# xuhaocuhk/TilinGNN

Measured on AMD Instinct MI355X. Metric: scored tile-nodes/sec (GNN forward), higher is better.
Workload: dtype f32; 1 GPU; TilinGNN.forward on a seeded banded super-graph: 100000 nodes / 1000000 adjacency edges / 1250000 collision edges per GPU, tile_count 2, T=13 edge types, width 32, depth 20, train-mode BatchNorm, graph prep included; n_nodes=100000, n_adj_edges=1000000, n_col_edges=1250000, parallelism=single GPU

## Files before the change

### include/tgnn.h

```cpp
#ifndef TGNN_H
#define TGNN_H

#include <stddef.h>
#include <stdint.h>

#ifdef __cplusplus
extern "C" {
#endif

#define TGNN_VERSION 100

#define TGNN_OK 0
#define TGNN_ERR_INVALID_ARG (-1)
#define TGNN_ERR_WORKSPACE (-2)
#define TGNN_ERR_LAUNCH (-3)
#define TGNN_ERR_UNSUPPORTED (-4)
#define TGNN_ERR_BAD_GRAPH (-5)
#define TGNN_ERR_UNVERIFIED (-7)
#define TGNN_ERR_STALE_RESULT (-6)

#define TGNN_ACT_NONE 0
#define TGNN_ACT_LEAKY_RELU 1
#define TGNN_ACT_SIGMOID 2

#define TGNN_BN_STAT_ROWS 4
#define TGNN_BN_MAX_PARTIALS 512

typedef void *tgnn_stream_t;

int tgnn_version(void);
const char *tgnn_last_error(void);


size_t tgnn_csr_workspace_bytes(int64_t n_nodes, int64_t n_edges);
int tgnn_csr_build(const int64_t *edge_index, int64_t n_edges, int64_t n_nodes, int64_t n_src_nodes,
                   int drop_self_loops, int32_t *rowptr, int32_t *col_src, int32_t *col_eid, int32_t *err_flag,
                   void *ws, size_t ws_bytes, tgnn_stream_t stream);

size_t tgnn_edge_dedup_workspace_bytes(int64_t n_edges, int32_t fe);
int tgnn_edge_type_dedup(const float *edge_attr, int64_t n_edges, int32_t fe, int32_t *edge_type,
                         int32_t *type_rep_edge, int32_t *n_types, void *ws, size_t ws_bytes,
                         tgnn_stream_t stream);

int tgnn_gather_i32(const int32_t *src, int64_t n_src, const int32_t *idx, int64_t n, int32_t *out,
                    tgnn_stream_t stream);


int tgnn_edge_weight_table(const float *edge_attr, const int32_t *type_rep_edge, int32_t n_types, int32_t fe,
                           const float *w1, const float *b1, const float *w2, const float *b2,
                           const float *w3, const float *b3, int32_t c, float *wtab, tgnn_stream_t stream);

int tgnn_nnconv_mean_fwd(const float *h, int64_t ldh, const int32_t *rowptr, const int32_t *col_src,
                         const int32_t *col_type, const float *wtab, int32_t n_types, const float *root,
                         const float *bias, int64_t n_nodes, int32_t c, int32_t act, float *out,
                         double *bn_partial, int32_t *n_partials_host, tgnn_stream_t stream);

int64_t tgnn_nnconv_cols_max_columns(int64_t n_nodes, int64_t n_edges);
size_t tgnn_nnconv_cols_workspace_bytes(int64_t n_nodes);
int tgnn_nnconv_cols_build(const int32_t *rowptr, const int32_t *col_src, const int32_t *col_type,
                           int64_t n_nodes, int32_t n_types, int32_t *tile_col_ptr, int32_t *col_meta,
                           int32_t *col_slot_src, void *ws, size_t ws_bytes, tgnn_stream_t stream);
int32_t tgnn_nnconv_cols_max_types(void);
size_t tgnn_nnconv_weight_image_floats(int32_t n_types);
int tgnn_nnconv_mean_cols_fwd(const float *h, int64_t ldh, const int32_t *tile_col_ptr, const int32_t *col_meta,
                              const int32_t *col_src, const float *wtab, int32_t n_types, const float *root,
                              const float *bias, int64_t n_nodes, int32_t c, int32_t act, float *out,
                              float *wimg_scratch, double *bn_partial, int32_t *n_partials_host,
                              tgnn_stream_t stream);
int tgnn_nnconv_mean_cols_f16_fwd(const float *h, int64_t ldh, int64_t n_src_rows, const int32_t *tile_col_ptr,
                                  const int32_t *col_meta, const int32_t *col_src, const float *wtab, int32_t n_types,
                                  const float *root, const float *bias, int64_t n_nodes, int32_t max_in_degree, int32_t act,
                                  float *out, float *wimg_scratch, uint32_t *bounds_scratch, double *bn_partial,
                                  int32_t *n_partials_host, tgnn_stream_t stream);

int64_t tgnn_nnconv_eg_max_groups(int64_t n_nodes, int64_t n_edges, int32_t n_types);
int tgnn_nnconv_eg_build(const int32_t *rowptr, const int32_t *col_src, const int32_t *col_type, int64_t n_nodes,
                         int32_t n_types, int32_t *tile_grp_ptr, int32_t *grp, void *ws, size_t ws_bytes, tgnn_stream_t stream);
int tgnn_nnconv_mean_eg_fwd(const float *h, int64_t ldh, int64_t n_src_rows, const int32_t *tile_grp_ptr,
                            const int32_t *grp, const float *wtab, int32_t n_types,
                            const float *root, const float *bias, int64_t n_nodes, int32_t act, float *out,
                            float *wimg_scratch, uint32_t *bounds_scratch, double *bn_partial, int32_t *n_partials_host,
                            tgnn_stream_t stream);

int32_t tgnn_nnconv64_eg_max_types(void);
size_t tgnn_nnconv64_eg_image_floats(int32_t n_types);
int tgnn_nnconv64_mean_eg_fwd(const float *h, int64_t ldh, int64_t n_src_rows, const int32_t *tile_grp_ptr,
                              const int32_t *grp, const float *wtab, int32_t n_types,
                              const float *root, const float *bias, int64_t n_nodes, int32_t act, float *out,
                              float *wimg_scratch, uint32_t *bounds_scratch, double *bn_partial, int32_t *n_partials_host,
                              tgnn_stream_t stream);

int tgnn_ubench_row_gather(int32_t shape, const float *table, int64_t n_rows, float *sink, int32_t iters, int32_t reps,
                           double *rows_per_s_out, tgnn_stream_t stream);

#define TGNN_MID_BATCH_WORDS 36
#define TGNN_MID_TILE_BATCHES 24
int64_t tgnn_mid_entries_words(int64_t n_nodes);
int tgnn_mid_entries_build(const int32_t *tile_col_ptr, const int32_t *col_meta, const int32_t *col_src, int64_t n_nodes,
                           const int32_t *cols_built_dev, int32_t *tile_nb, uint32_t *ent, int32_t *result, tgnn_stream_t stream);
void tgnn_forward_path_counts(int64_t *out3);
void tgnn_set_mid_layout_limit(int64_t n_nodes);
int64_t tgnn_get_mid_layout_limit(void);
int64_t tgnn_mid_layout_max_nodes(void);

int tgnn_gin_fwd(const float *a, int64_t lda, const float *in_stat, const int32_t *rowptr,
                 const int32_t *col_src, const float *eps, const float *w1, const float *b1,
                 const float *w2, const float *b2, const float *w3, const float *b3, int64_t n_nodes,
                 int32_t c, int32_t act, float *out, float *z_scratch, double *bn_partial,
                 int32_t *n_partials_host, tgnn_stream_t stream);
int tgnn_gin32_fwd(const float *a, int64_t lda, const float *in_stat, const int32_t *rowptr, const int32_t *col_src,
                   const float *eps, const float *w1, const float *b1, const float *w2, const float *b2, const float *w3,
                   const float *b3, int64_t n_nodes, int32_t c, int32_t act, int32_t variant, float *out, float *z_scratch,
                   double *bn_partial, int32_t *n_partials_host, tgnn_stream_t stream);
int tgnn_gin64_fwd(const float *a, int64_t lda, const float *in_stat, const int32_t *rowptr, const int32_t *col_src,
                   const float *eps, const float *w1, const float *b1, const float *w2, const float *b2, const float *w3,
                   const float *b3, int64_t n_nodes, int32_t act, float *out, float *z_scratch, double *bn_partial,
                   int32_t *n_partials_host, tgnn_stream_t stream);

int tgnn_dense_act_fwd(const float *a, int64_t lda, int64_t a_kblock_stride, const float *in_stat,
                       const float *w, const float *b, int64_t n_rows, int32_t in_dim, int32_t out_dim,
                       int32_t act, float *out, int64_t ldo, double *bn_partial, int32_t *n_partials_host,
                       tgnn_stream_t stream);
int tgnn_dense_act_slots_fwd(const float *a, int32_t slot_width, int64_t slot_stride, const float *in_stat,
                             const float *w, const float *b, int64_t n_rows, int32_t in_dim, int32_t out_dim,
                             int32_t act, float *out, int64_t ldo, double *bn_partial, int32_t *n_partials_host,
                             tgnn_stream_t stream);
int tgnn_dense_act_slots_f16_fwd(const float *a, int32_t slot_width, int64_t slot_stride, const float *w, const float *b,
                                 int64_t n_rows, int32_t in_dim, int32_t out_dim, int32_t act, float *out, int64_t ldo,
                                 uint32_t *bounds_scratch, void *wimg_scratch, double *bn_partial, int32_t *n_partials_host,
                                 tgnn_stream_t stream);

int tgnn_bn_finalize(int32_t mode, const double *partials, int32_t n_partials, double *sums, int32_t f,
                     int64_t n_rows_total, const float *gamma, const float *beta, float eps, float momentum,
                     float *running_mean, float *running_var, int64_t *num_batches_tracked, float *stat,
                     tgnn_stream_t stream);

int tgnn_bn_apply(const float *v, int64_t ldv, const float *stat, int64_t n_rows, int32_t f, float *out,
                  int64_t ldo, tgnn_stream_t stream);

int tgnn_merge_fwd(const float *a1, const float *stat1, const float *a2, const float *stat2,
                   const float *resid, int64_t n_nodes, int32_t c, float *out, float *h2_out,
                   tgnn_stream_t stream);

typedef struct tgnn_model_dims {
    int32_t node_features_dim;
    int32_t adj_edge_features_dim;
    int32_t network_width;
    int32_t network_depth;
    int32_t output_dim;
} tgnn_model_dims;

int32_t tgnn_param_count(const tgnn_model_dims *dims);
int tgnn_param_name(const tgnn_model_dims *dims, int32_t index, char *buf, size_t buf_len);

typedef struct tgnn_graph {
    int64_t n_nodes;
    int64_t n_adj_edges;
    int64_t n_col_edges;
    int32_t n_types;
    const int32_t *adj_rowptr;
    const int32_t *adj_src;
    const int32_t *adj_type;
    const int32_t *type_rep_edge;
    const int32_t *col_rowptr;
    const int32_t *col_src;
    const int32_t *nn_tile_col_ptr;
    const int32_t *nn_col_meta;
    const int32_t *nn_col_src;
    int32_t nn_max_in_degree;
    const int32_t *nn_mid_tile_nb;
    const uint32_t *nn_mid_ent;
    const int32_t *nn_tile_grp_ptr;
    const int32_t *nn_grp;
    const int32_t *nn_mid_verdict;
} tgnn_graph;

size_t tgnn_forward_workspace_bytes(const tgnn_model_dims *dims, int64_t n_nodes, int32_t n_types);

enum { TGNN_WS_MID = 0, TGNN_WS_A1, TGNN_WS_F1, TGNN_WS_F2, TGNN_WS_F3, TGNN_WS_BOUNDS, TGNN_WS_BOUNDS64, TGNN_WS_MAP_ENTRIES };
int tgnn_forward_workspace_map(const tgnn_model_dims *dims, int64_t n_nodes, int64_t n_rows, int32_t n_types, int64_t *byte_offsets,
                               int32_t n);

int tgnn_forward(const tgnn_model_dims *dims, const void *const *params_host, const float *x,
                 const float *adj_edge_attr, const tgnn_graph *graph, int32_t update_running,
                 int32_t use_running_stats, float *probs, void *ws, size_t ws_bytes,
                 tgnn_stream_t stream, tgnn_stream_t stream2);

int tgnn_forward_begin(const tgnn_model_dims *dims, const void *const *params_host, const float *x, int64_t n_nodes,
                       int32_t update_running, void *ws, size_t ws_bytes, tgnn_stream_t stream, tgnn_stream_t stream2);
int tgnn_forward_resume(const tgnn_model_dims *dims, const void *const *params_host, const float *x, const float *adj_edge_attr,
                        const tgnn_graph *graph, int32_t update_running, float *probs, void *ws, size_t ws_bytes,
                        tgnn_stream_t stream, tgnn_stream_t stream2);
int tgnn_forward_small_prepass(const tgnn_model_dims *dims, const void *const *params_host, const float *adj_edge_attr,
                               const int32_t *type_rep_edge, const int32_t *n_types_dev, int64_t n_nodes, void *ws, size_t ws_bytes,
                               tgnn_stream_t stream);

int tgnn_forward_begin_weights(const tgnn_model_dims *dims, const void *const *params_host, const float *adj_edge_attr,
                               const int32_t *type_rep_edge, const int32_t *n_types_dev, int64_t n_nodes, void *ws, size_t ws_bytes,
                               tgnn_stream_t stream);

typedef struct tgnn_train_save {
    float *init_a[2];
    float *init_stat[2];
    float *a1, *a2;
    float *u;
    float *stat1, *stat2;
    float *fin_a[4];
    float *fin_stat[4];
    float *skip;
    float *wtab;
} tgnn_train_save;
int tgnn_forward_train(const tgnn_model_dims *dims, const void *const *params_host, const float *x,
                       const float *adj_edge_attr, const tgnn_graph *graph, const tgnn_train_save *keep, float *probs,
                       void *ws, size_t ws_bytes, tgnn_stream_t stream, tgnn_stream_t stream2);

typedef struct tgnn_train_graph {
    const int32_t *adjT_rowptr, *adjT_src, *adjT_type;
    const int32_t *colT_rowptr, *colT_src;
    const float *deg, *inv_deg;
} tgnn_train_graph;
size_t tgnn_backward_workspace_bytes(const tgnn_model_dims *dims, int64_t n_nodes, int32_t n_types);
int tgnn_backward(const tgnn_model_dims *dims, const void *const *params_host, void *const *grads_host, const float *x,
                  const float *adj_edge_attr, const tgnn_graph *graph, const tgnn_train_graph *tgraph,
                  const tgnn_train_save *keep, const float *probs, const float *dprobs, void *ws, size_t ws_bytes,
                  tgnn_stream_t stream);
typedef struct tgnn_train_groups {
    const int32_t *fwd_tile_grp_ptr, *fwd_grp;
    const int32_t *bwd_tile_grp_ptr, *bwd_grp;
    const int32_t *type_major;
    int64_t n_list;
    int32_t max_in_degree, max_out_degree;
} tgnn_train_groups;
int tgnn_backward_groups(const tgnn_model_dims *dims, const void *const *params_host, void *const *grads_host, const float *x,
                         const float *adj_edge_attr, const tgnn_graph *graph, const tgnn_train_graph *tgraph,
                         const tgnn_train_groups *groups, const tgnn_train_save *keep, const float *probs, const float *dprobs,
                         void *ws, size_t ws_bytes, tgnn_stream_t stream);

typedef struct tgnn_shard {
    int64_t n_own, n_rows, n_total;
    const int32_t *send_idx;
    int64_t n_send;
    double *sum_buf;
    float *send_buf;
    float *recv_buf;
    int (*allreduce_f64)(void *ctx, double *buf, int64_t count, tgnn_stream_t stream);
    int (*alltoall_rows)(void *ctx, const float *send, float *recv, int32_t row_floats, int32_t extra_rows,
                         tgnn_stream_t stream);
    void *ctx;
    int32_t world, rank;
    const int32_t *send_idx_fused;
    const int32_t *recv_idx_fused;
    tgnn_stream_t side_stream;
    void *rccl_comm, *rccl_comm_side;
    const int64_t *send_counts, *recv_counts;
    const int32_t *send_row_ptr, *send_row_slot;
} tgnn_shard;

int32_t tgnn_rccl_available(void);
size_t tgnn_rccl_unique_id_bytes(void);
int tgnn_rccl_unique_id(void *id_out);
int tgnn_rccl_comm_create(const void *unique_id, int32_t rank, int32_t world, void **comm_out);
int tgnn_rccl_comm_destroy(void *comm);
void tgnn_rccl_counters(int64_t *out2);
size_t tgnn_forward_sharded_workspace_bytes(const tgnn_model_dims *dims, int64_t n_own, int64_t n_rows,
                                            int32_t n_types);
int tgnn_forward_sharded(const tgnn_model_dims *dims, const void *const *params_host, const float *x,
                         const float *adj_edge_attr, const tgnn_graph *graph, const tgnn_shard *shard,
                         int32_t update_running, float *probs, void *ws, size_t ws_bytes, tgnn_stream_t stream);

void tgnn_set_small_layout_limit(int64_t n_nodes);
int tgnn_spin_error_poll(tgnn_stream_t stream, uint32_t *code_out);
uint64_t tgnn_set_spin_budget_us(uint64_t us);
void tgnn_persist_fallback(int64_t n_forwards);
uint32_t tgnn_spin_error_peek(void);
int64_t tgnn_get_small_layout_limit(void);

int32_t tgnn_set_split_precision(int32_t mode);
int32_t tgnn_set_gin_fused(int32_t mode);
int32_t tgnn_set_gin_mlp_f16(int32_t on);
int32_t tgnn_set_mid_tail(int32_t on);
int32_t tgnn_set_nnconv_eg(int32_t on);
int32_t tgnn_set_nnconv64_eg(int32_t on);
int32_t tgnn_set_gin64_mfma(int32_t on);
int32_t tgnn_set_dense_rows_mode(int32_t mode);
int32_t tgnn_set_lean_head(int32_t bits);

int64_t tgnn_graph_prep_small_max_nodes(void);
int64_t tgnn_graph_prep_small_max_edges(void);
size_t tgnn_graph_prep_small_tmp_ints(int64_t n_nodes, int64_t n_adj_edges, int64_t n_col_edges);
int tgnn_graph_prep_small(const int64_t *adj_edge_index, int64_t n_adj_edges, const float *adj_edge_attr, int32_t fe,
                          const int64_t *col_edge_index, int64_t n_col_edges, int64_t n_nodes, int32_t *adj_rowptr,
                          int32_t *adj_src, int32_t *adj_eid, int32_t *adj_type, int32_t *edge_type, int32_t *type_rep_edge,
// ... 312 lines not shown
```

### tilingnn_amd/_lib.py

```python
from __future__ import annotations

import ctypes as C
import os

_HERE = os.path.dirname(os.path.abspath(__file__))
LIB_PATH = os.environ.get("TGNN_LIB_PATH") or os.path.join(_HERE, "libtgnn.so")

ACT_NONE, ACT_LEAKY_RELU, ACT_SIGMOID = 0, 1, 2
BN_MAX_PARTIALS = 512
BN_STAT_ROWS = 4


class TgnnError(RuntimeError):
    code = 0


class ModelDims(C.Structure):
    _fields_ = [("node_features_dim", C.c_int32), ("adj_edge_features_dim", C.c_int32),
                ("network_width", C.c_int32), ("network_depth", C.c_int32), ("output_dim", C.c_int32)]


class Graph(C.Structure):
    _fields_ = [("n_nodes", C.c_int64), ("n_adj_edges", C.c_int64), ("n_col_edges", C.c_int64),
                ("n_types", C.c_int32),
                ("adj_rowptr", C.c_void_p), ("adj_src", C.c_void_p), ("adj_type", C.c_void_p),
                ("type_rep_edge", C.c_void_p), ("col_rowptr", C.c_void_p), ("col_src", C.c_void_p),
                ("nn_tile_col_ptr", C.c_void_p), ("nn_col_meta", C.c_void_p), ("nn_col_src", C.c_void_p),
                ("nn_max_in_degree", C.c_int32),
                ("nn_mid_tile_nb", C.c_void_p), ("nn_mid_ent", C.c_void_p),
                ("nn_tile_grp_ptr", C.c_void_p), ("nn_grp", C.c_void_p), ("nn_mid_verdict", C.c_void_p)]


class SmallPrepLayout(C.Structure):
    _fields_ = [("adj_edge_index", C.c_void_p), ("adj_edge_attr", C.c_void_p), ("col_edge_index", C.c_void_p),
                ("n_adj_edges", C.c_int64), ("n_col_edges", C.c_int64), ("n_nodes", C.c_int64),
                ("adj_rowptr", C.c_void_p), ("adj_src", C.c_void_p), ("adj_eid", C.c_void_p), ("adj_type", C.c_void_p),
                ("edge_type", C.c_void_p), ("type_rep_edge", C.c_void_p),
                ("col_rowptr", C.c_void_p), ("col_src", C.c_void_p), ("col_eid", C.c_void_p),
                ("tile_col_ptr", C.c_void_p), ("col_meta", C.c_void_p), ("col_slot_src", C.c_void_p),
                ("tmp", C.c_void_p), ("fe", C.c_int32), ("reserved_", C.c_int32)]


class TrainSave(C.Structure):
    _fields_ = [("init_a", C.c_void_p * 2), ("init_stat", C.c_void_p * 2), ("a1", C.c_void_p), ("a2", C.c_void_p),
                ("u", C.c_void_p), ("stat1", C.c_void_p), ("stat2", C.c_void_p), ("fin_a", C.c_void_p * 4),
                ("fin_stat", C.c_void_p * 4), ("skip", C.c_void_p), ("wtab", C.c_void_p)]


class TrainGraphDesc(C.Structure):
    _fields_ = [("adjT_rowptr", C.c_void_p), ("adjT_src", C.c_void_p), ("adjT_type", C.c_void_p),
                ("colT_rowptr", C.c_void_p), ("colT_src", C.c_void_p), ("deg", C.c_void_p), ("inv_deg", C.c_void_p)]


class TrainGroupsDesc(C.Structure):
    _fields_ = [("fwd_tile_grp_ptr", C.c_void_p), ("fwd_grp", C.c_void_p), ("bwd_tile_grp_ptr", C.c_void_p), ("bwd_grp", C.c_void_p),
                ("type_major", C.c_void_p), ("n_list", C.c_int64), ("max_in_degree", C.c_int32), ("max_out_degree", C.c_int32)]


ALLREDUCE_CB = C.CFUNCTYPE(C.c_int, C.c_void_p, C.c_void_p, C.c_int64, C.c_void_p)
ALLTOALL_CB = C.CFUNCTYPE(C.c_int, C.c_void_p, C.c_void_p, C.c_void_p, C.c_int32, C.c_int32, C.c_void_p)


class ShardDesc(C.Structure):
    _fields_ = [("n_own", C.c_int64), ("n_rows", C.c_int64), ("n_total", C.c_int64),
                ("send_idx", C.c_void_p), ("n_send", C.c_int64),
                ("sum_buf", C.c_void_p), ("send_buf", C.c_void_p), ("recv_buf", C.c_void_p),
                ("allreduce_f64", ALLREDUCE_CB), ("alltoall_rows", ALLTOALL_CB), ("ctx", C.c_void_p),
                ("world", C.c_int32), ("rank", C.c_int32), ("send_idx_fused", C.c_void_p), ("recv_idx_fused", C.c_void_p),
                ("side_stream", C.c_void_p), ("rccl_comm", C.c_void_p), ("rccl_comm_side", C.c_void_p),
                ("send_counts", C.c_void_p), ("recv_counts", C.c_void_p),
                ("send_row_ptr", C.c_void_p), ("send_row_slot", C.c_void_p)]


def _load() -> C.CDLL:
    if not os.path.exists(LIB_PATH):
        raise ImportError(
            f"{LIB_PATH} is missing: the HIP extension has not been built. Build it with\n"
            f"    python -c 'import __graft_entry__ as g; g.build()'    (or: make -C tilingnn_amd/csrc)\n"
            "tilingnn_amd has no CPU fallback by design.")
    import torch
    lib = C.CDLL(LIB_PATH)
    p, i32, i64, f32, sz = C.c_void_p, C.c_int32, C.c_int64, C.c_float, C.c_size_t
    pi32 = C.POINTER(C.c_int32)
    sigs = {
        "tgnn_version": (C.c_int, []),
        "tgnn_last_error": (C.c_char_p, []),
        "tgnn_csr_workspace_bytes": (sz, [i64, i64]),
        "tgnn_csr_build": (C.c_int, [p, i64, i64, i64, C.c_int, p, p, p, p, p, sz, p]),
        "tgnn_edge_dedup_workspace_bytes": (sz, [i64, i32]),
        "tgnn_edge_type_dedup": (C.c_int, [p, i64, i32, p, p, p, p, sz, p]),
        "tgnn_gather_i32": (C.c_int, [p, i64, p, i64, p, p]),
        "tgnn_edge_weight_table": (C.c_int, [p, p, i32, i32, p, p, p, p, p, p, i32, p, p]),
        "tgnn_nnconv_mean_fwd": (C.c_int, [p, i64, p, p, p, p, i32, p, p, i64, i32, i32, p, p, pi32, p]),
        "tgnn_nnconv_cols_max_columns": (i64, [i64, i64]),
        "tgnn_nnconv_cols_workspace_bytes": (sz, [i64]),
        "tgnn_nnconv_cols_build": (C.c_int, [p, p, p, i64, i32, p, p, p, p, sz, p]),
        "tgnn_nnconv_cols_max_types": (i32, []),
        "tgnn_nnconv_weight_image_floats": (sz, [i32]),
        "tgnn_nnconv_mean_cols_fwd": (C.c_int, [p, i64, p, p, p, p, i32, p, p, i64, i32, i32, p, p, p, pi32, p]),
        "tgnn_nnconv_mean_cols_f16_fwd": (C.c_int, [p, i64, i64, p, p, p, p, i32, p, p, i64, i32, i32, p, p, p, p, pi32, p]),
        "tgnn_nnconv_eg_max_groups": (i64, [i64, i64, i32]),
        "tgnn_nnconv_eg_build": (C.c_int, [p, p, p, i64, i32, p, p, p, sz, p]),
        "tgnn_nnconv_mean_eg_fwd": (C.c_int, [p, i64, i64, p, p, p, i32, p, p, i64, i32, p, p, p, p, pi32, p]),
        "tgnn_nnconv64_eg_max_types": (i32, []),
        "tgnn_nnconv64_eg_image_floats": (sz, [i32]),
        "tgnn_nnconv64_mean_eg_fwd": (C.c_int, [p, i64, i64, p, p, p, i32, p, p, i64, i32, p, p, p, p, pi32, p]),
        "tgnn_ubench_row_gather": (C.c_int, [i32, p, i64, p, i32, i32, C.POINTER(C.c_double), p]),
        "tgnn_mid_entries_words": (i64, [i64]),
        "tgnn_mid_entries_build": (C.c_int, [p, p, p, i64, p, p, p, p, p]),
        "tgnn_forward_path_counts": (None, [p]),
        "tgnn_set_mid_layout_limit": (None, [i64]),
        "tgnn_get_mid_layout_limit": (i64, []),
        "tgnn_mid_layout_max_nodes": (i64, []),
        "tgnn_spin_error_poll": (C.c_int, [p, C.POINTER(C.c_uint32)]),
        "tgnn_set_spin_budget_us": (C.c_uint64, [C.c_uint64]),
        "tgnn_persist_fallback": (None, [i64]),
        "tgnn_spin_error_peek": (C.c_uint32, []),
        "tgnn_gin_fwd": (C.c_int, [p, i64, p, p, p, p, p, p, p, p, p, p, i64, i32, i32, p, p, p, pi32, p]),
        "tgnn_gin32_fwd": (C.c_int, [p, i64, p, p, p, p, p, p, p, p, p, p, i64, i32, i32, i32, p, p, p, pi32, p]),
        "tgnn_gin64_fwd": (C.c_int, [p, i64, p, p, p, p, p, p, p, p, p, p, i64, i32, p, p, p, pi32, p]),
        "tgnn_dense_act_fwd": (C.c_int, [p, i64, i64, p, p, p, i64, i32, i32, i32, p, i64, p, pi32, p]),
        "tgnn_dense_act_slots_fwd": (C.c_int, [p, i32, i64, p, p, p, i64, i32, i32, i32, p, i64, p, pi32, p]),
        "tgnn_dense_act_slots_f16_fwd": (C.c_int, [p, i32, i64, p, p, i64, i32, i32, i32, p, i64, p, p, p, pi32, p]),
        "tgnn_bn_finalize": (C.c_int, [i32, p, i32, p, i32, i64, p, p, f32, f32, p, p, p, p, p]),
        "tgnn_bn_apply": (C.c_int, [p, i64, p, i64, i32, p, i64, p]),
        "tgnn_merge_fwd": (C.c_int, [p, p, p, p, p, i64, i32, p, p, p]),
        "tgnn_param_count": (i32, [C.POINTER(ModelDims)]),
        "tgnn_param_name": (C.c_int, [C.POINTER(ModelDims), i32, C.c_char_p, sz]),
        "tgnn_forward_workspace_bytes": (sz, [C.POINTER(ModelDims), i64, i32]),
        "tgnn_forward_workspace_map": (C.c_int, [C.POINTER(ModelDims), i64, i64, i32, C.POINTER(C.c_int64), i32]),
        "tgnn_forward": (C.c_int, [C.POINTER(ModelDims), C.POINTER(C.c_void_p), p, p, C.POINTER(Graph), i32, i32,
                                   p, p, sz, p, p]),
        "tgnn_forward_begin": (C.c_int, [C.POINTER(ModelDims), C.POINTER(C.c_void_p), p, i64, i32, p, sz, p, p]),
        "tgnn_forward_resume": (C.c_int, [C.POINTER(ModelDims), C.POINTER(C.c_void_p), p, p, C.POINTER(Graph), i32, p, p, sz, p, p]),
        "tgnn_forward_begin_weights": (C.c_int, [C.POINTER(ModelDims), C.POINTER(C.c_void_p), p, p, p, i64, p, sz, p]),
        "tgnn_forward_small_prepass": (C.c_int, [C.POINTER(ModelDims), C.POINTER(C.c_void_p), p, p, p, i64, p, sz, p]),
        "tgnn_forward_sharded_workspace_bytes": (sz, [C.POINTER(ModelDims), i64, i64, i32]),
        "tgnn_forward_sharded": (C.c_int, [C.POINTER(ModelDims), C.POINTER(C.c_void_p), p, p, C.POINTER(Graph),
                                           C.POINTER(ShardDesc), i32, p, p, sz, p]),
        "tgnn_sublayout_workspace_bytes": (sz, [i64, i64, i64]),
        "tgnn_sublayout_compact": (C.c_int, [p, i64, p, i32, p, i64, p, i32, p, i64, p, p, p, p, p, p, p, p, sz, p]),
        "tgnn_shard_alive_rows": (C.c_int, [p, p, i64, i64, p, i64, p, i64, p, p, p]),
        "tgnn_tiles_in_region": (C.c_int, [p, p, p, p, p, i64, p, p, p, p, i64, i32, p, p, p]),
        "tgnn_region_edge_counts": (C.c_int, [p, i64, i64, p, i64, p, i64, p, p, p]),
        "tgnn_union_area_workspace_bytes": (sz, [i64, i64]),
        "tgnn_union_area": (C.c_int, [p, p, i64, p, p, p, i64, C.c_double, p, p, p, sz, p]),
        "tgnn_union_topology_workspace_bytes": (sz, [i64, i64]),
        "tgnn_union_topology": (C.c_int, [p, p, i64, p, p, p, p, p, i64, C.c_double, C.c_double, C.c_double, p, p, p, sz, p]),
        "tgnn_union_hole_delta_workspace_bytes": (sz, [i64, i64]),
        "tgnn_union_hole_delta": (C.c_int, [p, p, i64, p, p, p, p, p, i64, C.c_double, C.c_double, C.c_double, p, p, p, p, sz, p]),
        "tgnn_union_contour_workspace_bytes": (sz, [i64, i64, i64]),
        "tgnn_union_contour": (C.c_int, [p, p, i64, p, p, p, p, p, i64, C.c_double, i64, i64, p, p, p, p, p, p, p, p, sz, p]),
        "tgnn_batch_union": (C.c_int, [p] * 10 + [i32, i32, i32, p, p, i32, p, p, p, p, p]),
        "tgnn_greedy_round_workspace_bytes": (sz, [i64]),
        "tgnn_greedy_round": (C.c_int, [p, i64, p, i64, p, i64, i32, C.c_uint64, p, p, p, p, p, p, sz, p]),
        "tgnn_greedy_finish_max_nodes": (i64, []),
        "tgnn_greedy_finish": (C.c_int, [p, i64, p, i64, i32, i32, C.c_uint64, p, p, p, p, p, p, p]),
        "tgnn_sublayout_compact_many_workspace_bytes": (sz, [i32, i64, i64, i64]),
        "tgnn_sublayout_compact_many": (C.c_int, [i32, p, p, p, p, i64, i64, i64, p, p, i32, p, p, i32, p, p, p, p, p, p, p, p, p, sz, p]),
        "tgnn_greedy_round_many_workspace_bytes": (sz, [i32, i64]),
        "tgnn_greedy_round_many": (C.c_int, [i32, p, p, i64, p, p, i64, i64, p, p, p, i32, p, p, p, p, p, p, p, sz, p]),
        "tgnn_greedy_finish_many": (C.c_int, [i32, p, p, p, i64, i64, p, p, p, i32, i32, p, p, p, p, p, p, p, p]),
        "tgnn_solution_score_sums_many_workspace_bytes": (sz, [i32]),
        "tgnn_solution_score_sums_many": (C.c_int, [i32, p, p, p, i64, i64, p, p, i64, p, p, p, i64, p, p, sz, p]),
        "tgnn_unsupervised_loss_many_workspace_bytes": (sz, [i32, i32]),
        "tgnn_unsupervised_loss_many": (C.c_int, [i32, p, p, p, p, i64, i64, i64, p, p, i64, i32, p, i64, p, p, i64, p, f32, f32, f32,
                                                  p, p, p, p, sz, p]),
        "tgnn_unsupervised_loss_workspace_bytes": (sz, [i32]),
        "tgnn_unsupervised_loss": (C.c_int, [p, i64, i32, p, i64, i64, p, i64, p, i64, p, i64, f32, f32, f32, p, p, p, sz, p]),
        "tgnn_solution_score_sums": (C.c_int, [p, p, i64, p, i64, p, i64, p, i64, p, p, sz, p]),
        "tgnn_graph_prep_small_max_nodes": (i64, []),
        "tgnn_graph_prep_small_max_edges": (i64, []),
        "tgnn_graph_prep_small_tmp_ints": (sz, [i64, i64, i64]),
        "tgnn_graph_prep_small": (C.c_int, [p, i64, p, i32, p, i64, i64] + [p] * 16 + [p]),
        "tgnn_graph_prep_workspace_bytes": (sz, [i64, i64, i64, i32]),
        "tgnn_graph_prep": (C.c_int, [p, i64, p, i32, p, i64, i64, i64] + [p] * 17 + [sz, p, p, p]),
        "tgnn_graph_prep_wait": (C.c_int, [p]),
        "tgnn_graph_prep_small_many": (C.c_int, [C.POINTER(SmallPrepLayout), i32, p, p, p]),
        "tgnn_graph_prep_small_many_wait": (C.c_int, [p]),
        "tgnn_graph_prep_small_many_plan": (C.c_int, [p, p, p, i32, i32, p, p]),
        "tgnn_graph_prep_small_many_counts": (None, [p]),
        "tgnn_set_nnconv_eg": (i32, [i32]),
        "tgnn_set_nnconv64_eg": (i32, [i32]),
        "tgnn_set_gin64_mfma": (i32, [i32]),
        "tgnn_set_dense_rows_mode": (i32, [i32]),
        "tgnn_set_lean_head": (i32, [i32]),
        "tgnn_set_prep_words_poll": (i32, [i32]),
        "tgnn_set_small_layout_limit": (None, [i64]),
        "tgnn_get_small_layout_limit": (i64, []),
        "tgnn_set_split_precision": (i32, [i32]),
        "tgnn_set_gin_fused": (i32, [i32]),
        "tgnn_set_gin_mlp_f16": (i32, [i32]),
        "tgnn_set_mid_tail": (i32, [i32]),
        "tgnn_rccl_available": (i32, []),
        "tgnn_rccl_unique_id_bytes": (sz, []),
        "tgnn_rccl_unique_id": (C.c_int, [p]),
        "tgnn_rccl_comm_create": (C.c_int, [p, i32, i32, C.POINTER(C.c_void_p)]),
        "tgnn_rccl_comm_destroy": (C.c_int, [p]),
        "tgnn_rccl_counters": (None, [p]),
        "tgnn_forward_profiled": (C.c_int, [C.POINTER(ModelDims), C.POINTER(C.c_void_p), p, p, C.POINTER(Graph), i32,
                                            i32, p, p, sz, p, C.POINTER(C.c_float), pi32]),
        "tgnn_forward_many": (C.c_int, [C.POINTER(ModelDims), C.POINTER(C.c_void_p), i32, p, p, p, i32, i32, p, p, p, p, i32, p]),
        "tgnn_forward_union": (C.c_int, [C.POINTER(ModelDims), C.POINTER(C.c_void_p), i32, p, p, p, i32, p, p, p, p, p, i32, p]),
        "tgnn_forward_union_plan": (C.c_int, [p, i32, i32, p]),
        "tgnn_forward_union_counts": (None, [p]),
        "tgnn_forward_stamped": (C.c_int, [C.POINTER(ModelDims), C.POINTER(C.c_void_p), p, p, C.POINTER(Graph), i32, p, p, sz, p, p,
                                           C.POINTER(C.c_float)]),
        "tgnn_forward_profiled_two_stream": (C.c_int, [C.POINTER(ModelDims), C.POINTER(C.c_void_p), p, p, C.POINTER(Graph), i32,
                                                       p, p, sz, p, p, C.POINTER(C.c_float), pi32]),
        "tgnn_transpose": (C.c_int, [p, i32, i32, p, p]),
        "tgnn_swap_leading": (C.c_int, [p, i32, i32, i32, p, i32, p]),
        "tgnn_backward_workspace_bytes": (sz, [C.POINTER(ModelDims), i64, i32]),
        "tgnn_backward": (C.c_int, [C.POINTER(ModelDims), C.POINTER(C.c_void_p), C.POINTER(C.c_void_p), p, p,
                                    C.POINTER(Graph), C.POINTER(TrainGraphDesc), C.POINTER(TrainSave), p, p, p, sz, p]),
        "tgnn_backward_groups": (C.c_int, [C.POINTER(ModelDims), C.POINTER(C.c_void_p), C.POINTER(C.c_void_p), p, p,
                                           C.POINTER(Graph), C.POINTER(TrainGraphDesc), C.POINTER(TrainGroupsDesc),
                                           C.POINTER(TrainSave), p, p, p, sz, p]),
        "tgnn_nnconv_bwd_eg_ok": (i32, [i32, i64, i32, i32, i32, i32, i32]),
        "tgnn_nnconv_bwd_eg_workspace_bytes": (sz, [i64, i64, i32, i32]),
        "tgnn_nnconv_bwd_eg_list_ints": (sz, [i64]),
        "tgnn_nnconv_bwd_eg_dw_blocks": (i32, [i64]),
        "tgnn_nnconv_bwd_eg_build": (C.c_int, [p, p, i64, i32, p, p]),
        "tgnn_nnconv_bwd_eg": (C.c_int, [p, i64, p, p, p, p, p, p, p, i64, p, p, i64, i32, i32, i32, i32, p, p, p, sz, p]),
        "tgnn_set_nnconv_bwd_eg": (i32, [i32]),
        "tgnn_forward_train": (C.c_int, [C.POINTER(ModelDims), C.POINTER(C.c_void_p), p, p, C.POINTER(Graph),
                                         C.POINTER(TrainSave), p, p, sz, p, p]),
        "tgnn_gin_aggregate": (C.c_int, [p, i64, p, p, p, p, i64, i32, p, p]),
        "tgnn_sigmoid_bwd": (C.c_int, [p, i64, p, i64, i64, i32, p, i64, p]),
        "tgnn_add_into": (C.c_int, [p, i64, i64, i32, p, i64, p]),
        "tgnn_reduce_workspace_bytes": (sz, [i32]),
        "tgnn_colsum": (C.c_int, [p, i64, i64, i32, p, p, sz, p]),
        "tgnn_bn_bwd_reduce": (C.c_int, [p, i64, p, i64, p, i64, i32, f32, p, p, p, p, sz, p]),
        "tgnn_bn_bwd_apply": (C.c_int, [p, i64, p, i64, p, p, i64, i32, i32, p, i64, p, p, i64, p]),
        "tgnn_merge_bwd_reduce": (C.c_int, [p, i64, p, p, p, p, p, i64, i32, f32, f32, p, p, p, i64, p, p, p, p, p, p,
                                            p, sz, p]),
        "tgnn_wgrad_workspace_bytes": (sz, [i64, i32, i32]),
        "tgnn_wgrad": (C.c_int, [p, i64, p, i64, i64, i64, i32, i32, p, p, p, sz, p]),
        "tgnn_wgrad_slots": (C.c_int, [p, i64, p, i32, i64, i64, i32, i32, p, p, p, sz, p]),
        "tgnn_sigmoid_mlp_bwd_workspace_bytes": (sz, [i64, i32, i32, i32, i32]),
        "tgnn_sigmoid_mlp_bwd": (C.c_int, [p, i64, i32, i32, i32, i32, p, p, p, p, p, p, p, i64, p, p, p, p, p, p, p, p, sz,
                                           p]),
        "tgnn_sigmoid_mlp_bwd_fused_form": (i32, [i64, i32, i32, i32, i32, i32]),
        "tgnn_sigmoid_mlp_bwd_fused_workspace_bytes": (sz, [i64, i32, i32, i32, i32]),
        "tgnn_sigmoid_mlp_bwd_fused": (C.c_int, [p, i64, i32, i32, i32, i32, p, p, p, p, p, p, p, i64, p, p, p, p, p, p, p, p,
                                                 sz, p]),
        "tgnn_set_mlp_bwd_fused": (i32, [i32]),
        "tgnn_sigmoid_mlp_bwd_tall64_ok": (i32, [i64, i32, i32, i32, i32]),
        "tgnn_sigmoid_mlp_bwd_tall64_workspace_bytes": (sz, [i64, i32, i32, i32, i32]),
        "tgnn_sigmoid_mlp_bwd_tall64": (C.c_int, [p, i64, i32, i32, i32, i32, p, p, p, p, p, p, p, i64, p, p, p, p, p, p, p, p,
                                                  sz, p]),
        "tgnn_set_mlp_bwd_tall64": (i32, [i32]),
        "tgnn_nnconv_type_sum": (C.c_int, [p, i64, p, i64, p, p, p, p, i64, i32, i32, p, p]),
        "tgnn_csr_degree": (C.c_int, [p, i64, p, p, p]),
        "tgnn_unsupervised_loss_bwd": (C.c_int, [p, i64, p, i64, i64, p, i64, p, i64, p, i64, f32, f32, f32, p, p, p, i64,
                                                 p, sz, p]),
        "tgnn_f32_to_bf16": (C.c_int, [p, i64, p, p]),
        "tgnn_nnconv64_image_elems": (sz, [i32]),
        "tgnn_nnconv64_bf16_fwd": (C.c_int, [p, i64, p, p, p, p, i32, p, p, i64, i32, p, p, p, pi32, p]),
        "tgnn_nnconv64_bf16_eg_fwd": (C.c_int, [p, i64, p, p, p, i32, p, p, i64, i32, p, p, p, pi32, p]),
        "tgnn_gin64_bf16_fwd": (C.c_int, [p, p, p, p, p, p, p, p, p, p, p, i64, i32, p, p, p, pi32, p]),
        "tgnn_collconv64_bf16_fwd": (C.c_int, [p, p, p, p, p, p, p, p, p, p, p, p, p, p, p, i64, p, p, p, p, p, p]),
        "tgnn_merge_bf16_fwd": (C.c_int, [p, p, p, p, p, i64, i32, p, p]),
        "tgnn_dense_bf16_slots_fwd": (C.c_int, [p, i64, i32, p, p, i64, i32, i32, p, p, p, pi32, p]),
        "tgnn_forward_bf16_workspace_bytes": (sz, [C.POINTER(ModelDims), i64, i32]),
        "tgnn_forward_bf16": (C.c_int, [C.POINTER(ModelDims), C.POINTER(C.c_void_p), p, p, C.POINTER(Graph), i32, p, p, sz, p, p]),
        "tgnn_forward_bf16_begin": (C.c_int, [C.POINTER(ModelDims), C.POINTER(C.c_void_p), p, i64, i32, p, sz, p]),
        "tgnn_forward_bf16_drop": (C.c_int, [i32]),
        "tgnn_adam_chunk_elems": (i64, []),
        "tgnn_adam_chunk_count": (i64, [p, i32]),
        "tgnn_adam_table_bytes": (sz, [i32, i64]),
        "tgnn_adam_table_build": (C.c_int, [p, p, p, p, i32, i64, p, sz, C.POINTER(C.c_int64)]),
        "tgnn_adam_step": (C.c_int, [p, p, i32, i64, p, p, p, i64] + [C.c_double] * 6 + [p]),
        "tgnn_rows_gather": (C.c_int, [p, i64, p, i64, i32, p, i64, p]),
        "tgnn_rows_scatter": (C.c_int, [p, p, i64, i32, p, i64, p]),
    }
    for name, (res, args) in sigs.items():
        fn = getattr(lib, name)
        fn.restype, fn.argtypes = res, args
    for name, (res, args) in {"tgnn_debug_spin_fault": (None, [i32]), "tgnn_debug_set_csr_bucket_cap": (i32, [i32]),
                              "tgnn_debug_set_block_caps": (None, [i32, i32])}.items():
        try:
            fn = getattr(lib, name)
        except AttributeError:
            continue
        fn.restype, fn.argtypes = res, args
    return lib


DEBUG_LIB_PATH = os.path.join(_HERE, "libtgnn_debug.so")


def has_debug_hooks() -> bool:
    return hasattr(lib, "tgnn_debug_spin_fault")


lib = _load()
EXPORTED_SYMBOLS = (
    "tgnn_version", "tgnn_last_error", "tgnn_csr_workspace_bytes", "tgnn_csr_build",
    "tgnn_edge_dedup_workspace_bytes", "tgnn_edge_type_dedup", "tgnn_gather_i32", "tgnn_edge_weight_table",
    "tgnn_nnconv_mean_fwd", "tgnn_nnconv_cols_max_columns", "tgnn_nnconv_cols_workspace_bytes",
    "tgnn_nnconv_cols_build", "tgnn_nnconv_cols_max_types", "tgnn_nnconv_weight_image_floats", "tgnn_nnconv_mean_cols_fwd", "tgnn_nnconv_mean_cols_f16_fwd", "tgnn_nnconv_eg_max_groups", "tgnn_nnconv_eg_build", "tgnn_nnconv_mean_eg_fwd",
    "tgnn_nnconv64_eg_max_types", "tgnn_nnconv64_eg_image_floats", "tgnn_nnconv64_mean_eg_fwd", "tgnn_set_nnconv64_eg",
    "tgnn_gin64_fwd", "tgnn_set_gin64_mfma", "tgnn_gin32_fwd",
    "tgnn_ubench_row_gather", "tgnn_mid_entries_words", "tgnn_mid_entries_build", "tgnn_forward_path_counts", "tgnn_set_mid_layout_limit", "tgnn_get_mid_layout_limit", "tgnn_mid_layout_max_nodes",
    "tgnn_spin_error_poll", "tgnn_set_spin_budget_us", "tgnn_persist_fallback", "tgnn_spin_error_peek", "tgnn_gin_fwd", "tgnn_dense_act_fwd", "tgnn_dense_act_slots_fwd", "tgnn_dense_act_slots_f16_fwd", "tgnn_bn_finalize", "tgnn_bn_apply",
    "tgnn_merge_fwd", "tgnn_param_count", "tgnn_param_name", "tgnn_forward_workspace_bytes", "tgnn_forward_workspace_map", "tgnn_forward", "tgnn_forward_begin", "tgnn_forward_resume",
    "tgnn_forward_profiled", "tgnn_forward_profiled_two_stream", "tgnn_forward_stamped", "tgnn_forward_many", "tgnn_forward_union", "tgnn_forward_union_plan", "tgnn_forward_union_counts", "tgnn_graph_prep_small_max_nodes", "tgnn_graph_prep_small_max_edges", "tgnn_graph_prep_small_tmp_ints",
    "tgnn_graph_prep_small", "tgnn_graph_prep_workspace_bytes", "tgnn_graph_prep", "tgnn_graph_prep_wait", "tgnn_graph_prep_small_many", "tgnn_graph_prep_small_many_wait", "tgnn_graph_prep_small_many_plan", "tgnn_graph_prep_small_many_counts", "tgnn_set_small_layout_limit", "tgnn_get_small_layout_limit", "tgnn_set_split_precision", "tgnn_set_gin_fused", "tgnn_set_gin_mlp_f16", "tgnn_set_mid_tail", "tgnn_set_nnconv_eg", "tgnn_set_dense_rows_mode", "tgnn_set_lean_head", "tgnn_set_prep_words_poll", "tgnn_forward_begin_weights", "tgnn_forward_bf16_begin", "tgnn_forward_bf16_drop", "tgnn_forward_small_prepass", "tgnn_rccl_available", "tgnn_rccl_unique_id_bytes", "tgnn_rccl_unique_id", "tgnn_rccl_comm_create", "tgnn_rccl_comm_destroy", "tgnn_rccl_counters", "tgnn_forward_train", "tgnn_backward_workspace_bytes", "tgnn_backward", "tgnn_forward_sharded_workspace_bytes", "tgnn_forward_sharded",
    "tgnn_rows_gather", "tgnn_rows_scatter", "tgnn_unsupervised_loss_workspace_bytes", "tgnn_unsupervised_loss", "tgnn_solution_score_sums",
    "tgnn_sublayout_workspace_bytes", "tgnn_sublayout_compact", "tgnn_greedy_round_workspace_bytes", "tgnn_greedy_round", "tgnn_greedy_finish_max_nodes", "tgnn_greedy_finish", "tgnn_shard_alive_rows",
    "tgnn_sublayout_compact_many_workspace_bytes", "tgnn_sublayout_compact_many", "tgnn_greedy_round_many_workspace_bytes", "tgnn_greedy_round_many",
    "tgnn_greedy_finish_many", "tgnn_solution_score_sums_many_workspace_bytes", "tgnn_solution_score_sums_many",
    "tgnn_unsupervised_loss_many_workspace_bytes", "tgnn_unsupervised_loss_many",
    "tgnn_tiles_in_region", "tgnn_region_edge_counts", "tgnn_union_area_workspace_bytes", "tgnn_union_area", "tgnn_batch_union",
    "tgnn_union_topology_workspace_bytes", "tgnn_union_topology", "tgnn_union_contour_workspace_bytes", "tgnn_union_contour",
    "tgnn_union_hole_delta_workspace_bytes", "tgnn_union_hole_delta",
    "tgnn_transpose", "tgnn_swap_leading", "tgnn_gin_aggregate", "tgnn_sigmoid_bwd", "tgnn_add_into", "tgnn_reduce_workspace_bytes", "tgnn_colsum",
    "tgnn_bn_bwd_reduce", "tgnn_bn_bwd_apply", "tgnn_merge_bwd_reduce", "tgnn_wgrad_workspace_bytes", "tgnn_wgrad", "tgnn_wgrad_slots",
    "tgnn_sigmoid_mlp_bwd_workspace_bytes", "tgnn_sigmoid_mlp_bwd",
    "tgnn_sigmoid_mlp_bwd_fused_form", "tgnn_sigmoid_mlp_bwd_fused_workspace_bytes", "tgnn_sigmoid_mlp_bwd_fused", "tgnn_set_mlp_bwd_fused",
    "tgnn_sigmoid_mlp_bwd_tall64_ok", "tgnn_sigmoid_mlp_bwd_tall64_workspace_bytes", "tgnn_sigmoid_mlp_bwd_tall64", "tgnn_set_mlp_bwd_tall64",
    "tgnn_backward_groups", "tgnn_nnconv_bwd_eg_ok", "tgnn_nnconv_bwd_eg_workspace_bytes", "tgnn_nnconv_bwd_eg_list_ints",
    "tgnn_nnconv_bwd_eg_dw_blocks", "tgnn_nnconv_bwd_eg_build", "tgnn_nnconv_bwd_eg", "tgnn_set_nnconv_bwd_eg",
    "tgnn_nnconv_type_sum", "tgnn_csr_degree", "tgnn_unsupervised_loss_bwd",
    "tgnn_f32_to_bf16", "tgnn_nnconv64_image_elems", "tgnn_nnconv64_bf16_fwd", "tgnn_nnconv64_bf16_eg_fwd", "tgnn_gin64_bf16_fwd", "tgnn_collconv64_bf16_fwd", "tgnn_merge_bf16_fwd",
    "tgnn_dense_bf16_slots_fwd", "tgnn_forward_bf16_workspace_bytes", "tgnn_forward_bf16",
    "tgnn_adam_chunk_elems", "tgnn_adam_chunk_count", "tgnn_adam_table_bytes", "tgnn_adam_table_build", "tgnn_adam_step")


WS_MAP_PIECES = ("mid", "a1", "f1", "f2", "f3", "bounds", "bounds64")


def forward_workspace_map(dims, n_nodes, n_rows=None, n_types=0):
    out = (C.c_int64 * len(WS_MAP_PIECES))()
    check(lib.tgnn_forward_workspace_map(C.byref(dims), n_nodes, n_nodes if n_rows is None else n_rows, n_types, out, len(WS_MAP_PIECES)))
    return {name: int(v) for name, v in zip(WS_MAP_PIECES, out)}


def forward_path_counts():
    out = (C.c_int64 * 3)()
    lib.tgnn_forward_path_counts(out)
    return tuple(int(v) for v in out)


def forward_union_counts():
    out = (C.c_int64 * 2)()
    lib.tgnn_forward_union_counts(out)
    return tuple(int(v) for v in out)


def forward_union_plan(n_nodes, capacity_blocks):
    k = len(n_nodes)
    sizes = (C.c_int64 * max(k, 1))(*[int(v) for v in n_nodes])
    out = (C.c_int32 * max(k, 1))()
    n_groups = int(lib.tgnn_forward_union_plan(sizes, k, int(capacity_blocks), out))
    if n_groups < 0:
        raise ValueError("tgnn_forward_union_plan: invalid arguments")
    return [int(out[i]) for i in range(k)], n_groups


def graph_prep_small_many_counts():
    out = (C.c_int64 * 2)()
    lib.tgnn_graph_prep_small_many_counts(out)
    return tuple(int(v) for v in out)


def graph_prep_small_many_plan(n_adj_edges, n_col_edges, n_nodes, capacity_blocks):
    k = len(n_nodes)
    if not (len(n_adj_edges) == len(n_col_edges) == k):
        raise ValueError("tgnn_graph_prep_small_many_plan: one count of each kind per layout")
    arr = lambda vs: (C.c_int64 * max(k, 1))(*[int(v) for v in vs])
    blocks, groups = (C.c_int32 * max(k, 1))(), (C.c_int32 * max(k, 1))()
    n_groups = int(lib.tgnn_graph_prep_small_many_plan(arr(n_adj_edges), arr(n_col_edges), arr(n_nodes), k, int(capacity_blocks), blocks, groups))
    if n_groups < 0:
        raise ValueError("tgnn_graph_prep_small_many_plan: invalid arguments")
    return [int(blocks[i]) for i in range(k)], [int(groups[i]) for i in range(k)], n_groups


def check(rc: int) -> None:
    if rc != 0:
        msg = lib.tgnn_last_error()
        err = TgnnError(f"libtgnn error {rc}: {msg.decode() if msg else '?'}")
        err.code = int(rc)
        raise err


def ptr(t) -> C.c_void_p:
    return C.c_void_p(0) if t is None else C.c_void_p(t.data_ptr())


import threading

_pinned = threading.local()


def current_stream(device) -> C.c_void_p:
    import torch
    hit = getattr(_pinned, "value", None)
    if hit is not None:
        return hit[1]
    return C.c_void_p(torch.cuda.current_stream(device).cuda_stream)


class pinned_stream:

    def __init__(self, device):
        self.device = device

    def __enter__(self):
        import torch
        self.prev = getattr(_pinned, "value", None)
        dev = torch.device(self.device)
        _pinned.value = (dev.index, C.c_void_p(torch.cuda.current_stream(dev).cuda_stream))

    def __exit__(self, *exc):
        _pinned.value = self.prev


_side_streams = {}
_stream_lock = threading.Lock()
_stream_retry_at = {}
_stream_sets = {}


def _run_side_by_side(a, b, dev, cycles=400_000, reps=3) -> bool:
    import torch

    def span(with_b: bool) -> float:
        best = float("inf")
        for _ in range(reps):
            torch.cuda.synchronize(dev)
            e0, ea, eb = (torch.cuda.Event(enable_timing=True) for _ in range(3))
            e0.record(a)
            if with_b:
                b.wait_event(e0)
            with torch.cuda.stream(a):
                torch.cuda._sleep(cycles)
            ea.record(a)
            if with_b:
                with torch.cuda.stream(b):
                    torch.cuda._sleep(cycles)
                eb.record(b)
            torch.cuda.synchronize(dev)
            t = e0.elapsed_time(ea)
            if with_b:
                t = max(t, e0.elapsed_time(eb))
            best = min(best, t)
        return best
    span(False)
    with torch.cuda.stream(b):
        torch.cuda._sleep(1000)
    return span(True) < 1.5 * span(False)


# ... 75 lines not shown
```

### tilingnn_amd/csrc/bn_merge.hip

```cpp
#include "tgnn_common.h"

namespace tgnn {

__global__ __launch_bounds__(1024) void bn_finalize_kernel(BnJobs jobs, int mode, int f, int slices, int64_t n_total, float eps,
                                                           float momentum) {
    __shared__ double red[1024];
    __shared__ double tot[64];
    const BnJob jb = jobs.job[blockIdx.x / slices];
    const int slice = blockIdx.x % slices, f0 = slice * 32, fw = f - f0 < 32 ? f - f0 : 32;
    const int tid = threadIdx.x, two_f = 2 * f;
    float pre_gamma = 1.f, pre_beta = 0.f, pre_rm = 0.f, pre_rv = 1.f;
    if (tid < fw && mode != 1) {
        pre_gamma = jb.gamma[f0 + tid];
        pre_beta = jb.beta[f0 + tid];
        if (jb.running_mean) {
            pre_rm = jb.running_mean[f0 + tid];
            pre_rv = jb.running_var[f0 + tid];
        }
    }
    if (mode == 3) {
        if (tid < fw) {
            const double mean = (double)pre_rm;
            const double var = (double)pre_rv;
            const float mh = (float)mean;
            jb.stat[f0 + tid] = mh;
            jb.stat[f + f0 + tid] = (float)(mean - (double)mh);
            jb.stat[2 * f + f0 + tid] = (float)((double)pre_gamma / sqrt(var + (double)eps));
            jb.stat[3 * f + f0 + tid] = pre_beta;
        }
        return;
    }
    const int j = tid & 63, g = tid >> 6;
    const bool live = (j & 31) < fw;
    const int col = (j >> 5) * f + f0 + (j & 31);
    if (mode == 2) {
        if (tid < 64) tot[tid] = live ? jb.sums[col] : 0.0;
    } else {
        constexpr int groups = 16;
        double acc = 0.0;
        if (live) {
            const double *src = jb.partials + col;
            int p = g;
            for (; p + 31 * groups < jb.n_partials; p += 32 * groups) {
                double v[32];
#pragma unroll
                for (int u = 0; u < 32; ++u) v[u] = src[(int64_t)(p + u * groups) * two_f];
#pragma unroll
                for (int u = 0; u < 32; ++u) acc += v[u];
            }
            for (; p + 7 * groups < jb.n_partials; p += 8 * groups) {
                double v[8];
#pragma unroll
                for (int u = 0; u < 8; ++u) v[u] = src[(int64_t)(p + u * groups) * two_f];
#pragma unroll
                for (int u = 0; u < 8; ++u) acc += v[u];
            }
            for (; p < jb.n_partials; p += groups) acc += src[(int64_t)p * two_f];
        }
        red[tid] = acc;
        __syncthreads();
        if (tid < 64) {
            double t = 0.0;
            for (int gg = 0; gg < groups; ++gg) t += red[gg * 64 + tid];
            tot[tid] = t;
            if (mode == 1 && live) jb.sums[col] = t;
        }
        if (mode == 1) return;
    }
    __syncthreads();
    if (tid < fw) {
        const double inv_n = 1.0 / (double)n_total;
        const double mean = tot[tid] * inv_n;
        double var = tot[32 + tid] * inv_n - mean * mean;
        if (var < 0.0) var = 0.0;
        const float mh = (float)mean;
        jb.stat[f0 + tid] = mh;
        jb.stat[f + f0 + tid] = (float)(mean - (double)mh);
        jb.stat[2 * f + f0 + tid] = (float)((double)pre_gamma / sqrt(var + (double)eps));
        jb.stat[3 * f + f0 + tid] = pre_beta;
        if (jb.running_mean) {
            const double unbiased = n_total > 1 ? var * ((double)n_total / (double)(n_total - 1)) : var;
            jb.running_mean[f0 + tid] = (float)((1.0 - (double)momentum) * (double)pre_rm + (double)momentum * mean);
            jb.running_var[f0 + tid] = (float)((1.0 - (double)momentum) * (double)pre_rv + (double)momentum * unbiased);
        }
    }
    if (tid == 0 && slice == 0 && jb.num_batches_tracked) *jb.num_batches_tracked += 1;
}

__global__ void bn_apply_kernel(const float *__restrict__ v, int64_t ldv, const float *__restrict__ stat, int64_t n,
                                int f, float *__restrict__ out, int64_t ldo, unsigned *__restrict__ absmax_out) {
    const int64_t total = n * f;
    float am = 0.f;
    if (f == 32 && ldv == 32 && ldo == 32 && (((uintptr_t)v | (uintptr_t)out | (uintptr_t)stat) & 15) == 0) {
        const int q = threadIdx.x & 7;
        const float4 mh = reinterpret_cast<const float4 *>(stat)[q], ml = reinterpret_cast<const float4 *>(stat + 32)[q];
        const float4 gi = reinterpret_cast<const float4 *>(stat + 64)[q], be = reinterpret_cast<const float4 *>(stat + 96)[q];
        for (int64_t i = (int64_t)blockIdx.x * blockDim.x + threadIdx.x; i < total / 4; i += (int64_t)gridDim.x * blockDim.x) {
            const float4 x = reinterpret_cast<const float4 *>(v)[i];
            float4 o;
            o.x = bn_apply1(x.x, mh.x, ml.x, gi.x, be.x);
            o.y = bn_apply1(x.y, mh.y, ml.y, gi.y, be.y);
            o.z = bn_apply1(x.z, mh.z, ml.z, gi.z, be.z);
            o.w = bn_apply1(x.w, mh.w, ml.w, gi.w, be.w);
            reinterpret_cast<float4 *>(out)[i] = o;
            am = absmax4(am, o);
        }
        absmax_flush(am, absmax_out);
        return;
    }
    for (int64_t i = (int64_t)blockIdx.x * blockDim.x + threadIdx.x; i < total; i += (int64_t)gridDim.x * blockDim.x) {
        const int64_t r = i / f;
        const int c = (int)(i - r * f);
        const float o = bn_apply1(v[r * ldv + c], stat[c], stat[f + c], stat[2 * f + c], stat[3 * f + c]);
        out[r * ldo + c] = o;
        am = fmaxf(am, fabsf(o));
    }
    absmax_flush(am, absmax_out);
}

__global__ __launch_bounds__(256) void merge_kernel(const float *__restrict__ a1, const float *__restrict__ st1,
                                                    const float *__restrict__ a2, const float *__restrict__ st2,
                                                    const float *__restrict__ resid, int64_t n4, int c,
                                                    float *__restrict__ out, float *__restrict__ h2_out,
                                                    unsigned *__restrict__ absmax_out) {
    float am = 0.f;
    for (int64_t i = (int64_t)blockIdx.x * blockDim.x + threadIdx.x; i < n4; i += (int64_t)gridDim.x * blockDim.x) {
        const int col = (int)((i * 4) % c);
        const float4 x1 = reinterpret_cast<const float4 *>(a1)[i];
        const float4 x2 = reinterpret_cast<const float4 *>(a2)[i];
        const float4 m1h = *reinterpret_cast<const float4 *>(st1 + col), m1l = *reinterpret_cast<const float4 *>(st1 + c + col);
        const float4 g1 = *reinterpret_cast<const float4 *>(st1 + 2 * c + col), b1 = *reinterpret_cast<const float4 *>(st1 + 3 * c + col);
        const float4 m2h = *reinterpret_cast<const float4 *>(st2 + col), m2l = *reinterpret_cast<const float4 *>(st2 + c + col);
        const float4 g2 = *reinterpret_cast<const float4 *>(st2 + 2 * c + col), b2 = *reinterpret_cast<const float4 *>(st2 + 3 * c + col);
        float4 y2, o;
        y2.x = bn_apply1(x2.x, m2h.x, m2l.x, g2.x, b2.x);
        y2.y = bn_apply1(x2.y, m2h.y, m2l.y, g2.y, b2.y);
        y2.z = bn_apply1(x2.z, m2h.z, m2l.z, g2.z, b2.z);
        y2.w = bn_apply1(x2.w, m2h.w, m2l.w, g2.w, b2.w);
        o.x = bn_apply1(x1.x, m1h.x, m1l.x, g1.x, b1.x) * y2.x;
        o.y = bn_apply1(x1.y, m1h.y, m1l.y, g1.y, b1.y) * y2.y;
        o.z = bn_apply1(x1.z, m1h.z, m1l.z, g1.z, b1.z) * y2.z;
        o.w = bn_apply1(x1.w, m1h.w, m1l.w, g1.w, b1.w) * y2.w;
        if (resid) {
            const float4 r = reinterpret_cast<const float4 *>(resid)[i];
            o.x += r.x; o.y += r.y; o.z += r.z; o.w += r.w;
        }
        reinterpret_cast<float4 *>(out)[i] = o;
        am = absmax4(am, o);
        if (h2_out) reinterpret_cast<float4 *>(h2_out)[i] = y2;
    }
    absmax_flush(am, absmax_out);
}

__global__ __launch_bounds__(256) void merge_bn1_kernel(const float *__restrict__ a1, BnJob j1, int64_t n_total, float eps,
                                                        float momentum, const float *__restrict__ a2,
                                                        const float *__restrict__ st2, const float *__restrict__ resid,
                                                        int64_t n4, float *__restrict__ out, unsigned *__restrict__ absmax_out) {
    constexpr int c = 32, two_f = 64, groups = 16;
    __shared__ double red[groups * two_f];
    __shared__ double tot[two_f];
    __shared__ __attribute__((aligned(16))) float st1[4 * c];
    const int tid = threadIdx.x;
    float pre_gamma = 1.f, pre_beta = 0.f, pre_rm = 0.f, pre_rv = 1.f;
    if (tid < c) {
        pre_gamma = j1.gamma[tid];
        pre_beta = j1.beta[tid];
        if (blockIdx.x == 0 && j1.running_mean) {
            pre_rm = j1.running_mean[tid];
            pre_rv = j1.running_var[tid];
        }
    }
    {
        const int j = tid & 63, g0 = (tid >> 6) * 4;
        const double *src = j1.partials + j;
#pragma unroll
        for (int u = 0; u < 4; ++u) {
            const int g = g0 + u;
            double acc = 0.0;
            int p = g;
            for (; p + 31 * groups < j1.n_partials; p += 32 * groups) {
                double v[32];
#pragma unroll
                for (int q = 0; q < 32; ++q) v[q] = src[(int64_t)(p + q * groups) * two_f];
#pragma unroll
                for (int q = 0; q < 32; ++q) acc += v[q];
            }
            for (; p + 7 * groups < j1.n_partials; p += 8 * groups) {
                double v[8];
#pragma unroll
                for (int q = 0; q < 8; ++q) v[q] = src[(int64_t)(p + q * groups) * two_f];
#pragma unroll
                for (int q = 0; q < 8; ++q) acc += v[q];
            }
            for (; p < j1.n_partials; p += groups) acc += src[(int64_t)p * two_f];
            red[g * two_f + j] = acc;
        }
    }
    __syncthreads();
    if (tid < two_f) {
        double t = 0.0;
        for (int gg = 0; gg < groups; ++gg) t += red[gg * two_f + tid];
        tot[tid] = t;
    }
    __syncthreads();
    if (tid < c) {
        const double inv_n = 1.0 / (double)n_total;
        const double mean = tot[tid] * inv_n;
        double var = tot[c + tid] * inv_n - mean * mean;
        if (var < 0.0) var = 0.0;
        const float mh = (float)mean;
        st1[tid] = mh;
        st1[c + tid] = (float)(mean - (double)mh);
        st1[2 * c + tid] = (float)((double)pre_gamma / sqrt(var + (double)eps));
        st1[3 * c + tid] = pre_beta;
        if (blockIdx.x == 0) {
            if (j1.stat) {
                j1.stat[tid] = st1[tid]; j1.stat[c + tid] = st1[c + tid];
                j1.stat[2 * c + tid] = st1[2 * c + tid]; j1.stat[3 * c + tid] = st1[3 * c + tid];
            }
            if (j1.running_mean) {
                const double unbiased = n_total > 1 ? var * ((double)n_total / (double)(n_total - 1)) : var;
                j1.running_mean[tid] = (float)((1.0 - (double)momentum) * (double)pre_rm + (double)momentum * mean);
                j1.running_var[tid] = (float)((1.0 - (double)momentum) * (double)pre_rv + (double)momentum * unbiased);
            }
            if (tid == 0 && j1.num_batches_tracked) *j1.num_batches_tracked += 1;
        }
    }
    __syncthreads();
    float am = 0.f;
    for (int64_t i = (int64_t)blockIdx.x * blockDim.x + tid; i < n4; i += (int64_t)gridDim.x * blockDim.x) {
        const int col = (int)((i * 4) % c);
        const float4 x1 = reinterpret_cast<const float4 *>(a1)[i];
        const float4 x2 = reinterpret_cast<const float4 *>(a2)[i];
        const float4 m1h = *reinterpret_cast<const float4 *>(st1 + col), m1l = *reinterpret_cast<const float4 *>(st1 + c + col);
        const float4 g1 = *reinterpret_cast<const float4 *>(st1 + 2 * c + col), b1 = *reinterpret_cast<const float4 *>(st1 + 3 * c + col);
        const float4 m2h = *reinterpret_cast<const float4 *>(st2 + col), m2l = *reinterpret_cast<const float4 *>(st2 + c + col);
        const float4 g2 = *reinterpret_cast<const float4 *>(st2 + 2 * c + col), b2 = *reinterpret_cast<const float4 *>(st2 + 3 * c + col);
        float4 o;
        o.x = bn_apply1(x1.x, m1h.x, m1l.x, g1.x, b1.x) * bn_apply1(x2.x, m2h.x, m2l.x, g2.x, b2.x);
        o.y = bn_apply1(x1.y, m1h.y, m1l.y, g1.y, b1.y) * bn_apply1(x2.y, m2h.y, m2l.y, g2.y, b2.y);
        o.z = bn_apply1(x1.z, m1h.z, m1l.z, g1.z, b1.z) * bn_apply1(x2.z, m2h.z, m2l.z, g2.z, b2.z);
        o.w = bn_apply1(x1.w, m1h.w, m1l.w, g1.w, b1.w) * bn_apply1(x2.w, m2h.w, m2l.w, g2.w, b2.w);
        if (resid) {
            const float4 r = reinterpret_cast<const float4 *>(resid)[i];
            o.x += r.x; o.y += r.y; o.z += r.z; o.w += r.w;
        }
        reinterpret_cast<float4 *>(out)[i] = o;
        am = absmax4(am, o);
    }
    absmax_flush(am, absmax_out);
}

__global__ __launch_bounds__(1024) void merge_bn1_wide_kernel(const float *__restrict__ a1, BnJob j1, int64_t n_total, float eps,
                                                              float momentum, const float *__restrict__ a2,
                                                              const float *__restrict__ st2, const float *__restrict__ resid,
                                                              int64_t n4, float *__restrict__ out, unsigned *__restrict__ absmax_out) {
    constexpr int c = 32, two_f = 64, groups = 16;
    __shared__ double red[groups * two_f];
    __shared__ double tot[two_f];
    __shared__ __attribute__((aligned(16))) float st1[4 * c];
    __shared__ __attribute__((aligned(16))) float st2s[4 * c];
    const int tid = threadIdx.x;
    float pre_gamma = 1.f, pre_beta = 0.f, pre_rm = 0.f, pre_rv = 1.f;
    if (tid < c) {
        pre_gamma = j1.gamma[tid];
        pre_beta = j1.beta[tid];
        if (blockIdx.x == 0 && j1.running_mean) {
            pre_rm = j1.running_mean[tid];
            pre_rv = j1.running_var[tid];
        }
    }
    if (tid >= 1024 - 4 * c) st2s[tid - (1024 - 4 * c)] = st2[tid - (1024 - 4 * c)];
    constexpr int kPf = 3;
    const int64_t i_first = (int64_t)blockIdx.x * blockDim.x + tid, i_step = (int64_t)gridDim.x * blockDim.x;
    float4 px1[kPf], px2[kPf], pr[kPf];
    {
        using u32x2_ = __attribute__((ext_vector_type(2))) unsigned int;
        const int j = tid % two_f, g = tid / two_f;
        const __amdgpu_buffer_rsrc_t prs = __builtin_amdgcn_make_buffer_rsrc(
            const_cast<double *>(j1.partials), 0, (int)((uint32_t)j1.n_partials * (uint32_t)two_f * 8u), 0x00020000);
        static_assert(TGNN_BN_MAX_PARTIALS <= 32 * groups, "32 rows per thread cover every partial row");
        u32x2_ v[32];
#pragma unroll
        for (int q = 0; q < 32; ++q)
            v[q] = __builtin_amdgcn_raw_buffer_load_b64(prs, ((uint32_t)(g + q * groups) * (uint32_t)two_f + (uint32_t)j) * 8u, 0, 0);
#pragma unroll
        for (int k = 0; k < kPf; ++k) {
            const int64_t i = i_first + k * i_step;
            const int64_t ii = i < n4 ? i : n4 - 1;
            px1[k] = reinterpret_cast<const float4 *>(a1)[ii];
            px2[k] = reinterpret_cast<const float4 *>(a2)[ii];
            pr[k] = resid ? reinterpret_cast<const float4 *>(resid)[ii] : float4{0.f, 0.f, 0.f, 0.f};
        }
        double acc = 0.0;
#pragma unroll
        for (int q = 0; q < 32; ++q) acc += __builtin_bit_cast(double, v[q]);
        red[tid] = acc;
    }
    __syncthreads();
    if (tid < two_f) {
        double t = 0.0;
        for (int gg = 0; gg < groups; ++gg) t += red[gg * two_f + tid];
        tot[tid] = t;
    }
    __syncthreads();
    if (tid < c) {
        const double inv_n = 1.0 / (double)n_total;
        const double mean = tot[tid] * inv_n;
        double var = tot[c + tid] * inv_n - mean * mean;
        if (var < 0.0) var = 0.0;
        const float mh = (float)mean;
        st1[tid] = mh;
        st1[c + tid] = (float)(mean - (double)mh);
        st1[2 * c + tid] = (float)((double)pre_gamma / sqrt(var + (double)eps));
        st1[3 * c + tid] = pre_beta;
        if (blockIdx.x == 0) {
            if (j1.stat) {
                j1.stat[tid] = st1[tid]; j1.stat[c + tid] = st1[c + tid];
                j1.stat[2 * c + tid] = st1[2 * c + tid]; j1.stat[3 * c + tid] = st1[3 * c + tid];
            }
            if (j1.running_mean) {
                const double unbiased = n_total > 1 ? var * ((double)n_total / (double)(n_total - 1)) : var;
                j1.running_mean[tid] = (float)((1.0 - (double)momentum) * (double)pre_rm + (double)momentum * mean);
                j1.running_var[tid] = (float)((1.0 - (double)momentum) * (double)pre_rv + (double)momentum * unbiased);
            }
            if (tid == 0 && j1.num_batches_tracked) *j1.num_batches_tracked += 1;
        }
    }
    __syncthreads();
    const int col = (tid * 4) % c;
    const float4 m1h = *reinterpret_cast<const float4 *>(st1 + col), m1l = *reinterpret_cast<const float4 *>(st1 + c + col);
    const float4 g1 = *reinterpret_cast<const float4 *>(st1 + 2 * c + col), b1 = *reinterpret_cast<const float4 *>(st1 + 3 * c + col);
    const float4 m2h = *reinterpret_cast<const float4 *>(st2s + col), m2l = *reinterpret_cast<const float4 *>(st2s + c + col);
    const float4 g2 = *reinterpret_cast<const float4 *>(st2s + 2 * c + col), b2 = *reinterpret_cast<const float4 *>(st2s + 3 * c + col);
    float am = 0.f;
    auto item = [&](const float4 &x1, const float4 &x2, const float4 &r, int64_t i) {
#pragma clang fp contract(off)
        float4 o;
        o.x = bn_apply1(x1.x, m1h.x, m1l.x, g1.x, b1.x) * bn_apply1(x2.x, m2h.x, m2l.x, g2.x, b2.x);
        o.y = bn_apply1(x1.y, m1h.y, m1l.y, g1.y, b1.y) * bn_apply1(x2.y, m2h.y, m2l.y, g2.y, b2.y);
        o.z = bn_apply1(x1.z, m1h.z, m1l.z, g1.z, b1.z) * bn_apply1(x2.z, m2h.z, m2l.z, g2.z, b2.z);
        o.w = bn_apply1(x1.w, m1h.w, m1l.w, g1.w, b1.w) * bn_apply1(x2.w, m2h.w, m2l.w, g2.w, b2.w);
        if (resid) { o.x += r.x; o.y += r.y; o.z += r.z; o.w += r.w; }
        reinterpret_cast<float4 *>(out)[i] = o;
        am = absmax4(am, o);
    };
#pragma unroll
    for (int k = 0; k < kPf; ++k) {
        const int64_t i = i_first + k * i_step;
        if (i < n4) item(px1[k], px2[k], pr[k], i);
    }
    for (int64_t i = i_first + kPf * i_step; i < n4; i += i_step) {
        const float4 x1 = reinterpret_cast<const float4 *>(a1)[i];
        const float4 x2 = reinterpret_cast<const float4 *>(a2)[i];
        const float4 r = resid ? reinterpret_cast<const float4 *>(resid)[i] : float4{0.f, 0.f, 0.f, 0.f};
        item(x1, x2, r, i);
    }
    absmax_flush(am, absmax_out);
}

__global__ void rows_gather_kernel(const float *__restrict__ src, int64_t ld, const int *__restrict__ idx, int64_t n_idx,
                                   int c, float *__restrict__ out, int64_t ld_out) {
    const int64_t total = n_idx * c;
    for (int64_t i = (int64_t)blockIdx.x * blockDim.x + threadIdx.x; i < total; i += (int64_t)gridDim.x * blockDim.x) {
        const int64_t r = i / c;
        const int k = (int)(i - r * c);
        out[r * ld_out + k] = src[(int64_t)idx[r] * ld + k];
    }
}

__global__ void rows_scatter_kernel(const float *__restrict__ in, const int *__restrict__ idx, int64_t n_idx, int c,
                                    float *__restrict__ dst, int64_t ld) {
    const int64_t total = n_idx * c;
    for (int64_t i = (int64_t)blockIdx.x * blockDim.x + threadIdx.x; i < total; i += (int64_t)gridDim.x * blockDim.x) {
        const int64_t r = i / c;
        const int k = (int)(i - r * c);
        dst[(int64_t)idx[r] * ld + k] = in[i];
    }
}

static inline unsigned ew_grid(int64_t n, int cap = 256 * 8) {
    int64_t g = (n + 255) / 256;
    if (g < 1) g = 1;
    if (g > cap) g = cap;
    return (unsigned)g;
}

__global__ void shard_pack_kernel(const float *__restrict__ a1, const float *__restrict__ a2, const int *__restrict__ idx,
                                  int64_t n_rows, const float *__restrict__ sums_as_float, float *__restrict__ out) {
    const int64_t total = n_rows * 64;
    for (int64_t i = (int64_t)blockIdx.x * blockDim.x + threadIdx.x; i < total; i += (int64_t)gridDim.x * blockDim.x) {
        const int64_t r = i >> 6;
        const int k = (int)(i & 63), id = idx[r];
        float v;
        if (id >= 0) v = k < 32 ? a1[(int64_t)id * 32 + k] : a2[(int64_t)id * 32 + (k - 32)];
        else v = sums_as_float[(-1 - id) * 64 + k];
        out[i] = v;
    }
}
__global__ void shard_unpack_kernel(const float *__restrict__ in, const int *__restrict__ idx, int64_t n_rows,
                                    int64_t n_own, float *__restrict__ a1, float *__restrict__ a2,
                                    float *__restrict__ peer_sums_as_float) {
    const int64_t total = n_rows * 64;
    for (int64_t i = (int64_t)blockIdx.x * blockDim.x + threadIdx.x; i < total; i += (int64_t)gridDim.x * blockDim.x) {
        const int64_t r = i >> 6;
        const int k = (int)(i & 63), id = idx[r];
        const float v = in[i];
        if (id >= 0) {
            if (k < 32) a1[(n_own + id) * 32 + k] = v;
            else a2[(n_own + id) * 32 + (k - 32)] = v;
        } else {
            peer_sums_as_float[(int64_t)(-1 - id) * 64 + k] = v;
        }
    }
}
__global__ void shard_sum_peers_kernel(const double *__restrict__ peer_sums, const double *__restrict__ own, int world,
                                       int rank, double *__restrict__ total) {
    const int j = threadIdx.x;
    double t = 0.0;
    for (int p = 0; p < world; ++p) t += p == rank ? own[j] : peer_sums[(int64_t)p * 128 + j];
    total[j] = t;
}

__device__ __forceinline__ void bn_sums_from_partials_1024(const BnJob &jb, int two_f, double *red, double *tot) {
    const int tid = threadIdx.x;
    const int groups = 1024 / two_f;
    const int j = tid % two_f, g = tid / two_f;
    double acc = 0.0;
    if (g < groups) {
        const double *src = jb.partials + j;
        int p = g;
        for (; p + 31 * groups < jb.n_partials; p += 32 * groups) {
            double v[32];
#pragma unroll
            for (int u = 0; u < 32; ++u) v[u] = src[(int64_t)(p + u * groups) * two_f];
#pragma unroll
            for (int u = 0; u < 32; ++u) acc += v[u];
        }
        for (; p + 7 * groups < jb.n_partials; p += 8 * groups) {
            double v[8];
#pragma unroll
            for (int u = 0; u < 8; ++u) v[u] = src[(int64_t)(p + u * groups) * two_f];
#pragma unroll
            for (int u = 0; u < 8; ++u) acc += v[u];
        }
        for (; p < jb.n_partials; p += groups) acc += src[(int64_t)p * two_f];
    }
    red[tid] = acc;
    __syncthreads();
    if (tid < two_f) {
        double t = 0.0;
        for (int gg = 0; gg < groups; ++gg) t += red[gg * two_f + tid];
        tot[tid] = t;
    }
    __syncthreads();
}

__global__ __launch_bounds__(1024) void shard_pack_sums_kernel(const float *__restrict__ a1, const float *__restrict__ a2,
                                                               const int *__restrict__ idx, int64_t n_rows, BnJobs jobs,
                                                               float *__restrict__ out) {
    const int tid = threadIdx.x;
    if (blockIdx.x == 0) {
        __shared__ double red[1024];
        __shared__ double tot[128];
        bn_sums_from_partials_1024(jobs.job[0], 64, red, tot);
        bn_sums_from_partials_1024(jobs.job[1], 64, red, tot + 64);
        if (tid < 128) jobs.job[tid >> 6].sums[tid & 63] = tot[tid];
        const float *tf = reinterpret_cast<const float *>(tot);
        for (int64_t r = tid >> 6; r < n_rows; r += 16) {
            const int id = idx[r];
            if (id < 0) out[r * 64 + (tid & 63)] = tf[(-1 - id) * 64 + (tid & 63)];
        }
        return;
    }
    const int64_t total = n_rows * 64;
    for (int64_t i = (int64_t)(blockIdx.x - 1) * 1024 + tid; i < total; i += (int64_t)(gridDim.x - 1) * 1024) {
        const int64_t r = i >> 6;
        const int k = (int)(i & 63), id = idx[r];
        if (id >= 0) out[i] = k < 32 ? a1[(int64_t)id * 32 + k] : a2[(int64_t)id * 32 + (k - 32)];
    }
}

__global__ __launch_bounds__(1024) void shard_unpack_finalize_kernel(const float *__restrict__ in, const int *__restrict__ idx,
                                                                     int64_t n_rows, int64_t n_own, float *__restrict__ a1,
                                                                     float *__restrict__ a2, BnJobs jobs, int world, int rank,
                                                                     int64_t n_total, float eps, float momentum) {
    const int tid = threadIdx.x;
    if (blockIdx.x == 0) {
        __shared__ int pos[4 * 64];
        __shared__ double tot[128];
        for (int64_t r = tid; r < n_rows; r += 1024) {
            const int id = idx[r];
            if (id < 0 && -1 - id < 4 * 64) pos[-1 - id] = (int)r;
        }
        __syncthreads();
        if (tid < 128) {
            const int k = tid >> 5, jj = tid & 31;
            const double *own = jobs.job[0].sums;
            double t = 0.0;
            for (int p = 0; p < world; ++p)
                t += p == rank ? own[tid] : reinterpret_cast<const double *>(in + (int64_t)pos[4 * p + k] * 64)[jj];
            tot[tid] = t;
        }
        __syncthreads();
        bn_record_from_sums(jobs.job[0], tot, 32, n_total, eps, momentum);
        bn_record_from_sums(jobs.job[1], tot + 64, 32, n_total, eps, momentum);
        return;
    }
    const int64_t total = n_rows * 64;
// ... 53 lines not shown
        return;
    }
    const int64_t total = n_rows * 32;
    for (int64_t i = (int64_t)(blockIdx.x - 1) * 1024 + tid; i < total; i += (int64_t)(gridDim.x - 1) * 1024) {
        const int id = idx[i >> 5];
        if (id >= 0) a[(n_own + id) * 32 + (i & 31)] = in[i];
    }
}

__global__ __launch_bounds__(256) void shard_unpack1_merge_kernel(const float *__restrict__ in, const int *__restrict__ idx,
                                                                  int64_t n_in, int64_t n_own, const float *__restrict__ a1, BnJob job,
                                                                  int world, int rank, int64_t n_total, float eps, float momentum,
                                                                  const float *__restrict__ a2, const float *__restrict__ st2,
                                                                  const float *__restrict__ resid, int64_t n_rows,
                                                                  float *__restrict__ out, unsigned *__restrict__ absmax_out) {
    constexpr int c = 32;
    __shared__ int pos[4 * 64];
    __shared__ int hend[64];
    __shared__ double tot[64];
    __shared__ __attribute__((aligned(16))) float st1[4 * c];
    const int tid = threadIdx.x;
    for (int64_t r = tid; r < n_in; r += 256) {
        const int id = idx[r];
        if (id < 0 && -1 - id < 4 * 64) pos[-1 - id] = (int)r;
    }
    float pre_gamma = 1.f, pre_beta = 0.f, pre_rm = 0.f, pre_rv = 1.f;
    if (tid < c) {
        pre_gamma = job.gamma[tid];
        pre_beta = job.beta[tid];
        if (blockIdx.x == 0 && job.running_mean) {
            pre_rm = job.running_mean[tid];
            pre_rv = job.running_var[tid];
        }
    }
    __syncthreads();
    if (tid < 64) {
        const int k = tid >> 4, jj = tid & 15;
        double t = 0.0;
        for (int p = 0; p < world; ++p)
            t += p == rank ? job.sums[tid] : reinterpret_cast<const double *>(in + (int64_t)pos[4 * p + k] * 32)[jj];
        tot[tid] = t;
        if (tid < world) hend[tid] = pos[4 * tid] - 4 * tid;
    }
    __syncthreads();
    if (tid < c) {
        const double inv_n = 1.0 / (double)n_total;
        const double mean = tot[tid] * inv_n;
        double var = tot[c + tid] * inv_n - mean * mean;
        if (var < 0.0) var = 0.0;
        const float mh = (float)mean;
        st1[tid] = mh;
        st1[c + tid] = (float)(mean - (double)mh);
        st1[2 * c + tid] = (float)((double)pre_gamma / sqrt(var + (double)eps));
        st1[3 * c + tid] = pre_beta;
        if (blockIdx.x == 0) {
            job.stat[tid] = st1[tid]; job.stat[c + tid] = st1[c + tid];
            job.stat[2 * c + tid] = st1[2 * c + tid]; job.stat[3 * c + tid] = st1[3 * c + tid];
            if (job.running_mean) {
                const double unbiased = n_total > 1 ? var * ((double)n_total / (double)(n_total - 1)) : var;
                job.running_mean[tid] = (float)((1.0 - (double)momentum) * (double)pre_rm + (double)momentum * mean);
                job.running_var[tid] = (float)((1.0 - (double)momentum) * (double)pre_rv + (double)momentum * unbiased);
            }
            if (tid == 0 && job.num_batches_tracked) *job.num_batches_tracked += 1;
        }
    }
    __syncthreads();
    float am = 0.f;
    const int64_t n4 = n_rows * c / 4;
    for (int64_t i = (int64_t)blockIdx.x * blockDim.x + tid; i < n4; i += (int64_t)gridDim.x * blockDim.x) {
        const int col = (int)((i * 4) % c);
        const int64_t row = i >> 3;
        float4 x1;
        if (row < n_own) {
            x1 = reinterpret_cast<const float4 *>(a1)[i];
        } else {
            const int h = (int)(row - n_own);
            int p = 0;
            while (p + 1 < world && h >= hend[p]) ++p;
            x1 = reinterpret_cast<const float4 *>(in)[((int64_t)h + 4 * p) * 8 + (i & 7)];
        }
        const float4 x2 = reinterpret_cast<const float4 *>(a2)[i];
        const float4 m1h = *reinterpret_cast<const float4 *>(st1 + col), m1l = *reinterpret_cast<const float4 *>(st1 + c + col);
        const float4 g1 = *reinterpret_cast<const float4 *>(st1 + 2 * c + col), b1 = *reinterpret_cast<const float4 *>(st1 + 3 * c + col);
        const float4 m2h = *reinterpret_cast<const float4 *>(st2 + col), m2l = *reinterpret_cast<const float4 *>(st2 + c + col);
        const float4 g2 = *reinterpret_cast<const float4 *>(st2 + 2 * c + col), b2 = *reinterpret_cast<const float4 *>(st2 + 3 * c + col);
        float4 y2, o;
        y2.x = bn_apply1(x2.x, m2h.x, m2l.x, g2.x, b2.x);
        y2.y = bn_apply1(x2.y, m2h.y, m2l.y, g2.y, b2.y);
        y2.z = bn_apply1(x2.z, m2h.z, m2l.z, g2.z, b2.z);
        y2.w = bn_apply1(x2.w, m2h.w, m2l.w, g2.w, b2.w);
        o.x = bn_apply1(x1.x, m1h.x, m1l.x, g1.x, b1.x) * y2.x;
        o.y = bn_apply1(x1.y, m1h.y, m1l.y, g1.y, b1.y) * y2.y;
        o.z = bn_apply1(x1.z, m1h.z, m1l.z, g1.z, b1.z) * y2.z;
        o.w = bn_apply1(x1.w, m1h.w, m1l.w, g1.w, b1.w) * y2.w;
        if (resid) {
            const float4 r = reinterpret_cast<const float4 *>(resid)[i];
            o.x += r.x; o.y += r.y; o.z += r.z; o.w += r.w;
        }
        reinterpret_cast<float4 *>(out)[i] = o;
        am = absmax4(am, o);
    }
    absmax_flush(am, absmax_out);
}

static inline unsigned shard_copy_blocks(int64_t n_rows) {
    int64_t b = (n_rows * 64 + 1023) / 1024;
    if (b < 1) b = 1;
    if (b > 1024) b = 1024;
    return (unsigned)b;
}
void launch_shard_pack_sums(const float *a1, const float *a2, const int *idx, int64_t n_rows, const BnJobs &jobs, float *out,
                            hipStream_t s) {
    shard_pack_sums_kernel<<<1 + shard_copy_blocks(n_rows), 1024, 0, s>>>(a1, a2, idx, n_rows, jobs, out);
}
void launch_shard_unpack_finalize(const float *in, const int *idx, int64_t n_rows, int64_t n_own, float *a1, float *a2,
                                  const BnJobs &jobs, int world, int rank, int64_t n_total, float eps, float momentum,
                                  hipStream_t s) {
    shard_unpack_finalize_kernel<<<1 + shard_copy_blocks(n_rows), 1024, 0, s>>>(in, idx, n_rows, n_own, a1, a2, jobs, world,
                                                                                rank, n_total, eps, momentum);
}

void launch_shard_pack1(const float *a, const int *idx, int64_t n_rows, const BnJob &job, float *out, hipStream_t s) {
    shard_pack1_kernel<<<1 + shard_copy_blocks((n_rows + 1) / 2), 1024, 0, s>>>(a, idx, n_rows, job, out);
}
void launch_shard_unpack1(const float *in, const int *idx, int64_t n_rows, int64_t n_own, float *a, const BnJob &job, int world,
                          int rank, int64_t n_total, float eps, float momentum, hipStream_t s) {
    shard_unpack1_kernel<<<1 + shard_copy_blocks((n_rows + 1) / 2), 1024, 0, s>>>(in, idx, n_rows, n_own, a, job, world, rank,
                                                                                 n_total, eps, momentum);
}

void launch_shard_unpack1_merge(const float *in, const int *idx, int64_t n_in, int64_t n_own, const float *a1, const BnJob &job,
                                int world, int rank, int64_t n_total, float eps, float momentum, const float *a2, const float *stat2,
                                const float *resid, int64_t n_rows, float *out, unsigned *absmax_out, hipStream_t s) {
    const int64_t n4 = n_rows * 32 / 4;
    shard_unpack1_merge_kernel<<<ew_grid(n4, 512), 256, 0, s>>>(in, idx, n_in, n_own, a1, job, world, rank, n_total, eps, momentum, a2,
                                                               stat2, resid, n_rows, out, absmax_out);
}

void launch_shard_pack(const float *a1, const float *a2, const int *idx, int64_t n_rows, const double *sums, float *out,
                       hipStream_t s) {
    if (n_rows > 0)
        shard_pack_kernel<<<ew_grid(n_rows * 64), 256, 0, s>>>(a1, a2, idx, n_rows, reinterpret_cast<const float *>(sums), out);
}
void launch_shard_unpack(const float *in, const int *idx, int64_t n_rows, int64_t n_own, float *a1, float *a2,
                         double *peer_sums, hipStream_t s) {
    if (n_rows > 0)
        shard_unpack_kernel<<<ew_grid(n_rows * 64), 256, 0, s>>>(in, idx, n_rows, n_own, a1, a2,
                                                                 reinterpret_cast<float *>(peer_sums));
}
void launch_shard_sum_peers(const double *peer_sums, const double *own, int world, int rank, double *total, hipStream_t s) {
    shard_sum_peers_kernel<<<1, 128, 0, s>>>(peer_sums, own, world, rank, total);
}

void launch_merge_bn1(const float *a1, const BnJob &j1, int64_t n_total, float eps, float momentum, const float *a2,
                      const float *stat2, const float *resid, int64_t n_nodes, float *out, hipStream_t s, unsigned *absmax_out) {
    const int64_t n4 = n_nodes * 32 / 4;
    if (j1.n_partials > 128) {
        int64_t blocks = (n4 + 1023) / 1024;
        if (blocks > 256) blocks = 256;
        merge_bn1_wide_kernel<<<(unsigned)blocks, 1024, 0, s>>>(a1, j1, n_total, eps, momentum, a2, stat2, resid, n4, out, absmax_out);
        return;
    }
    int64_t blocks = (n4 + 255) / 256;
    if (blocks > 256) blocks = 256;
    merge_bn1_kernel<<<(unsigned)blocks, 256, 0, s>>>(a1, j1, n_total, eps, momentum, a2, stat2, resid, n4, out, absmax_out);
}

__global__ void absmax_kernel(const float *__restrict__ h, int64_t n4, unsigned *__restrict__ out_bits) {
    float m = 0.f;
    for (int64_t i = (int64_t)blockIdx.x * blockDim.x + threadIdx.x; i < n4; i += (int64_t)gridDim.x * blockDim.x) {
        const float4 v = reinterpret_cast<const float4 *>(h)[i];
        m = fmaxf(fmaxf(m, fmaxf(fabsf(v.x), fabsf(v.y))), fmaxf(fabsf(v.z), fabsf(v.w)));
    }
    absmax_flush(m, out_bits);
}
void launch_absmax(const float *h, int64_t n_floats, unsigned *max_bits, hipStream_t s) {
    const int64_t n4 = n_floats / 4;
    if (n4 <= 0) return;
    int64_t g = (n4 + 255) / 256;
    if (g > 512) g = 512;
    absmax_kernel<<<(unsigned)g, 256, 0, s>>>(h, n4, max_bits);
}

void launch_merge(const float *a1, const float *stat1, const float *a2, const float *stat2, const float *resid, int64_t n_nodes,
                  int c, float *out, float *h2_out, unsigned *absmax_out, hipStream_t s) {
    const int64_t n4 = n_nodes * c / 4;
    merge_kernel<<<ew_grid(n4, absmax_out ? 512 : 256 * 8), 256, 0, s>>>(a1, stat1, a2, stat2, resid, n4, c, out, h2_out, absmax_out);
}
void launch_bn_apply(const float *v, int64_t ldv, const float *stat, int64_t n_rows, int f, float *out, int64_t ldo,
                     unsigned *absmax_out, hipStream_t s) {
    bn_apply_kernel<<<ew_grid(n_rows * f, absmax_out ? 512 : 256 * 8), 256, 0, s>>>(v, ldv, stat, n_rows, f, out, ldo, absmax_out);
}

void launch_bn_finalize(const BnJobs &jobs, int n_jobs, int mode, int f, int64_t n_total, float eps, float momentum,
                        hipStream_t s) {
    const int slices = (f + 31) / 32;
    bn_finalize_kernel<<<n_jobs * slices, 1024, 0, s>>>(jobs, mode, f, slices, n_total, eps, momentum);
}

}

using namespace tgnn;

extern "C" int tgnn_bn_finalize(int32_t mode, const double *partials, int32_t n_partials, double *sums, int32_t f,
                                int64_t n_rows_total, const float *gamma, const float *beta, float eps, float momentum,
                                float *running_mean, float *running_var, int64_t *num_batches_tracked, float *stat,
                                tgnn_stream_t stream) {
    DeviceGuard guard__(stream);
    TGNN_CHECK_ARG(mode >= 0 && mode <= 3, "mode");
    TGNN_CHECK_ARG(f >= 1 && f <= 256, "feature count must be in [1,256]");
    TGNN_CHECK_ARG(mode == 3 || n_rows_total >= 1, "n_rows_total");
    TGNN_CHECK_ARG(mode == 1 || (gamma && beta && stat), "null pointer");
    TGNN_CHECK_ARG(!(mode == 0 || mode == 1) || (partials && n_partials >= 1 && n_partials <= TGNN_BN_MAX_PARTIALS), "partials");
    TGNN_CHECK_ARG(!(mode == 1 || mode == 2) || sums, "sums");
    TGNN_CHECK_ARG(mode != 3 || (running_mean && running_var), "running stats");
    TGNN_CHECK_ARG((running_mean == nullptr) == (running_var == nullptr), "running stats come in pairs");
    BnJobs jobs{};
    jobs.job[0] = BnJob{partials, n_partials, sums, gamma, beta, running_mean, running_var, num_batches_tracked, stat};
    const int slices = (f + 31) / 32;
    bn_finalize_kernel<<<slices, 1024, 0, static_cast<hipStream_t>(stream)>>>(jobs, mode, f, slices, n_rows_total, eps, momentum);
    TGNN_CHECK_LAUNCH();
    return TGNN_OK;
}

extern "C" int tgnn_bn_apply(const float *v, int64_t ldv, const float *stat, int64_t n_rows, int32_t f, float *out,
                             int64_t ldo, tgnn_stream_t stream) {
    DeviceGuard guard__(stream);
    if (n_rows <= 0) return TGNN_OK;
    TGNN_CHECK_ARG(v && stat && out && f >= 1 && ldv >= f && ldo >= f, "arguments");
    launch_bn_apply(v, ldv, stat, n_rows, f, out, ldo, nullptr, static_cast<hipStream_t>(stream));
    TGNN_CHECK_LAUNCH();
    return TGNN_OK;
}

extern "C" int tgnn_merge_fwd(const float *a1, const float *stat1, const float *a2, const float *stat2,
                              const float *resid, int64_t n_nodes, int32_t c, float *out, float *h2_out,
                              tgnn_stream_t stream) {
    DeviceGuard guard__(stream);
    if (n_nodes <= 0) return TGNN_OK;
    TGNN_CHECK_ARG(a1 && stat1 && a2 && stat2 && out, "null pointer");
    TGNN_CHECK_ARG(c >= 4 && c % 4 == 0, "width must be a multiple of 4");
    TGNN_CHECK_ARG(((uintptr_t)a1 | (uintptr_t)a2 | (uintptr_t)out | (uintptr_t)resid | (uintptr_t)h2_out |
                    (uintptr_t)stat1 | (uintptr_t)stat2) % 16 == 0, "pointers must be 16-byte aligned");
    launch_merge(a1, stat1, a2, stat2, resid, n_nodes, c, out, h2_out, nullptr, static_cast<hipStream_t>(stream));
    TGNN_CHECK_LAUNCH();
    return TGNN_OK;
}

extern "C" int tgnn_rows_gather(const float *src, int64_t ld_src, const int32_t *idx, int64_t n_idx, int32_t c,
                                float *out, int64_t ld_out, tgnn_stream_t stream) {
    DeviceGuard guard__(stream);
    if (n_idx <= 0) return TGNN_OK;
    TGNN_CHECK_ARG(src && idx && out && c >= 1 && ld_src >= c && ld_out >= c, "arguments");
    rows_gather_kernel<<<ew_grid(n_idx * c), 256, 0, static_cast<hipStream_t>(stream)>>>(src, ld_src, idx, n_idx, c, out,
                                                                                         ld_out);
    TGNN_CHECK_LAUNCH();
    return TGNN_OK;
}

extern "C" int tgnn_rows_scatter(const float *in, const int32_t *idx, int64_t n_idx, int32_t c, float *dst,
                                 int64_t ld_dst, tgnn_stream_t stream) {
    DeviceGuard guard__(stream);
    if (n_idx <= 0) return TGNN_OK;
    TGNN_CHECK_ARG(in && idx && dst && c >= 1 && ld_dst >= c, "arguments");
    rows_scatter_kernel<<<ew_grid(n_idx * c), 256, 0, static_cast<hipStream_t>(stream)>>>(in, idx, n_idx, c, dst, ld_dst);
    TGNN_CHECK_LAUNCH();
    return TGNN_OK;
}
```

### tilingnn_amd/csrc/gin.hip

```cpp
#include <stdlib.h>

#include "forward_persist.h"
#include "gin32_plan.h"

namespace tgnn {


template <int C>
__global__ __launch_bounds__(256) void gin_aggregate_kernel(
    const float *__restrict__ a, int64_t lda, const float *__restrict__ in_stat, const int *__restrict__ rowptr,
    const int *__restrict__ col_src, const float *__restrict__ eps_p, int64_t n, float *__restrict__ z) {
    constexpr int LPR = C / 4, RPB = 256 / LPR;
#ifdef TGNN_ABL_EMPTYGIN
    if (n > 0) return;
#endif
    const int tid = threadIdx.x, g = tid / LPR, q = tid % LPR;
    const int xcd = blockIdx.x & 7, chunk = blockIdx.x >> 3;
    const int64_t r_beg = n * xcd / 8, r_end = n * (xcd + 1) / 8;
    const int64_t v = r_beg + (int64_t)chunk * RPB + g;
    if (v >= r_end) return;
    const float one_eps = 1.0f + eps_p[0];
    float4 mhi = make_float4(0, 0, 0, 0), mlo = mhi, gv = make_float4(1, 1, 1, 1), bv = mhi;
    if (in_stat) {
        mhi = reinterpret_cast<const float4 *>(in_stat)[q];
        mlo = reinterpret_cast<const float4 *>(in_stat + C)[q];
        gv = reinterpret_cast<const float4 *>(in_stat + 2 * C)[q];
        bv = reinterpret_cast<const float4 *>(in_stat + 3 * C)[q];
    }
    const int beg = rowptr[v], end = rowptr[v + 1];
    const float4 self = *reinterpret_cast<const float4 *>(a + v * lda + 4 * q);
    float4 acc = make_float4(0, 0, 0, 0);
    int e = beg;
    for (; e + 4 <= end; e += 4) {
        const int s0 = col_src[e], s1 = col_src[e + 1], s2 = col_src[e + 2], s3 = col_src[e + 3];
        const float4 x0 = *reinterpret_cast<const float4 *>(a + (int64_t)s0 * lda + 4 * q);
        const float4 x1 = *reinterpret_cast<const float4 *>(a + (int64_t)s1 * lda + 4 * q);
        const float4 x2 = *reinterpret_cast<const float4 *>(a + (int64_t)s2 * lda + 4 * q);
        const float4 x3 = *reinterpret_cast<const float4 *>(a + (int64_t)s3 * lda + 4 * q);
#define TGNN_ACC(X)                          \
    acc.x += ((X).x - mhi.x) - mlo.x;        \
    acc.y += ((X).y - mhi.y) - mlo.y;        \
    acc.z += ((X).z - mhi.z) - mlo.z;        \
    acc.w += ((X).w - mhi.w) - mlo.w;
        TGNN_ACC(x0) TGNN_ACC(x1) TGNN_ACC(x2) TGNN_ACC(x3)
    }
    for (; e < end; ++e) {
        const float4 x0 = *reinterpret_cast<const float4 *>(a + (int64_t)col_src[e] * lda + 4 * q);
        TGNN_ACC(x0)
    }
#undef TGNN_ACC
    const float kb = one_eps + (float)(end - beg);
    float4 o;
    o.x = fmaf(gv.x, fmaf(one_eps, (self.x - mhi.x) - mlo.x, acc.x), kb * bv.x);
    o.y = fmaf(gv.y, fmaf(one_eps, (self.y - mhi.y) - mlo.y, acc.y), kb * bv.y);
    o.z = fmaf(gv.z, fmaf(one_eps, (self.z - mhi.z) - mlo.z, acc.z), kb * bv.z);
    o.w = fmaf(gv.w, fmaf(one_eps, (self.w - mhi.w) - mlo.w, acc.w), kb * bv.w);
    *reinterpret_cast<float4 *>(z + v * C + 4 * q) = o;
}

constexpr int kMlpWaves = 8, kMlpThreads = kMlpWaves * 64;
static_assert(kGin32BlockRows == kGin32TileRows * kMlpWaves && kGin32MaxPartials == TGNN_BN_MAX_PARTIALS &&
              kGin32ActLeakyRelu == TGNN_ACT_LEAKY_RELU, "gin32_plan.h restates these");
constexpr int kGinGroupRow0 = TGNN_BN_MAX_PARTIALS - 16;
using bf16x8 = __attribute__((ext_vector_type(8))) __bf16;
using f32x4 = __attribute__((ext_vector_type(4))) float;

__device__ __forceinline__ int gin_kf(int q, int e) { return e < 4 ? 4 * q + e : 16 + 4 * q + (e - 4); }

__device__ __forceinline__ void gin_split3(const float (&x)[8], bf16x8 &hi, bf16x8 &mid, bf16x8 &lo) {
    split3_trunc(x, hi, mid, lo);
}

__device__ __forceinline__ f32x4 gin_mma6(const bf16x8 *wpl, int plane_stride, const bf16x8 (&x)[3], f32x4 acc) {
    const bf16x8 w0 = wpl[0], w1 = wpl[plane_stride], w2 = wpl[2 * plane_stride];
    acc = __builtin_amdgcn_mfma_f32_16x16x32_bf16(w2, x[0], acc, 0, 0, 0);
    acc = __builtin_amdgcn_mfma_f32_16x16x32_bf16(w0, x[2], acc, 0, 0, 0);
    acc = __builtin_amdgcn_mfma_f32_16x16x32_bf16(w1, x[1], acc, 0, 0, 0);
    acc = __builtin_amdgcn_mfma_f32_16x16x32_bf16(w1, x[0], acc, 0, 0, 0);
    acc = __builtin_amdgcn_mfma_f32_16x16x32_bf16(w0, x[1], acc, 0, 0, 0);
    acc = __builtin_amdgcn_mfma_f32_16x16x32_bf16(w0, x[0], acc, 0, 0, 0);
    return acc;
}

__global__ __launch_bounds__(kMlpThreads, 2) void gin32_mlp_kernel(
    const float *__restrict__ z, const float *__restrict__ w1, const float *__restrict__ b1,
    const float *__restrict__ w2, const float *__restrict__ b2, const float *__restrict__ w3,
    const float *__restrict__ b3, int64_t n, int act, float *__restrict__ out, double *__restrict__ bn_partial, GinFin fin) {
    __shared__ bf16x8 W1s[3 * 2 * 64];
    __shared__ bf16x8 W2s[3 * 4 * 64];
    __shared__ bf16x8 W3s[3 * 2 * 2 * 64];
    __shared__ __attribute__((aligned(16))) float Bs[128];
    __shared__ double red[kMlpWaves * 64];
    const int tid = threadIdx.x, lane = tid & 63, wave = tid >> 6;
    const int fn = lane & 15, fq = lane >> 4;
#ifdef TGNN_ABL_EMPTYGIN
    if (n > 0) return;
#endif

    const Gin32Tiles share = gin32_wave_share(n, (int)gridDim.x, (int)blockIdx.x, wave);
    const int64_t t0 = share.t0, t1 = share.t1;

    auto load_z = [&](int64_t tile, float4 (&zin)[2]) {
        int64_t zr = tile * 16 + fn;
        zr = zr < n ? zr : n - 1;
        const float4 *pz = reinterpret_cast<const float4 *>(z + zr * 32 + 8 * fq);
        zin[0] = pz[0];
        zin[1] = pz[1];
    };
    float4 zin[2];
    load_z(t0 < t1 ? t0 : 0, zin);

#ifndef TGNN_ABL_GINNOPRO
    for (int i = tid; i < 2 * 64; i += kMlpThreads) {
        const int mb = i >> 6, ii = (i >> 2) & 15, q = i & 3;
        float x[8];
#pragma unroll
        for (int e = 0; e < 8; ++e) x[e] = w1[(16 * mb + ii) * 32 + 8 * q + e];
        gin_split3(x, W1s[(0 * 2 + mb) * 64 + ii * 4 + q], W1s[(1 * 2 + mb) * 64 + ii * 4 + q], W1s[(2 * 2 + mb) * 64 + ii * 4 + q]);
    }
    for (int i = tid; i < 4 * 64; i += kMlpThreads) {
        const int mb = i >> 6, ii = (i >> 2) & 15, q = i & 3;
        float x[8];
#pragma unroll
        for (int e = 0; e < 8; ++e) x[e] = w2[(16 * mb + ii) * 32 + gin_kf(q, e)];
        gin_split3(x, W2s[(0 * 4 + mb) * 64 + ii * 4 + q], W2s[(1 * 4 + mb) * 64 + ii * 4 + q], W2s[(2 * 4 + mb) * 64 + ii * 4 + q]);
    }
    for (int i = tid; i < 4 * 64; i += kMlpThreads) {
        const int mb = i >> 7, ks = (i >> 6) & 1, ii = (i >> 2) & 15, q = i & 3;
        float x[8];
#pragma unroll
        for (int e = 0; e < 8; ++e) x[e] = w3[(16 * mb + ii) * 64 + 32 * ks + gin_kf(q, e)];
        const int o = (mb * 2 + ks) * 64 + ii * 4 + q;
        gin_split3(x, W3s[0 * 256 + o], W3s[1 * 256 + o], W3s[2 * 256 + o]);
    }
#endif
    if (tid < 32) Bs[tid] = b1[tid];
    else if (tid < 96) Bs[tid] = b2[tid - 32];
    else if (tid < 128) Bs[tid] = b3[tid - 96];
    __syncthreads();

    auto bias4 = [&](int base, int mb) {
        const float4 t = *reinterpret_cast<const float4 *>(Bs + base + 16 * mb + 4 * fq);
        return f32x4{t.x, t.y, t.z, t.w};
    };
    const bf16x8 *w1p = W1s + fn * 4 + fq, *w2p = W2s + fn * 4 + fq, *w3p = W3s + fn * 4 + fq;
    double cs[8] = {0, 0, 0, 0, 0, 0, 0, 0}, cq[8] = {0, 0, 0, 0, 0, 0, 0, 0};

    for (int64_t tile = t0; tile < t1; ++tile) {
        bf16x8 xb[3];
        {
            const float x[8] = {zin[0].x, zin[0].y, zin[0].z, zin[0].w, zin[1].x, zin[1].y, zin[1].z, zin[1].w};
            gin_split3(x, xb[0], xb[1], xb[2]);
        }
        load_z(tile + 1 < t1 ? tile + 1 : tile, zin);
        f32x4 h1a = gin_mma6(w1p + 0 * 64, 2 * 64, xb, bias4(0, 0));
        f32x4 h1b = gin_mma6(w1p + 1 * 64, 2 * 64, xb, bias4(0, 1));
        {
            const float x[8] = {sigmoidf_(h1a[0]), sigmoidf_(h1a[1]), sigmoidf_(h1a[2]), sigmoidf_(h1a[3]),
                                sigmoidf_(h1b[0]), sigmoidf_(h1b[1]), sigmoidf_(h1b[2]), sigmoidf_(h1b[3])};
            gin_split3(x, xb[0], xb[1], xb[2]);
        }
        f32x4 h2[4];
#pragma unroll
        for (int mb = 0; mb < 4; ++mb) h2[mb] = gin_mma6(w2p + mb * 64, 4 * 64, xb, bias4(32, mb));
        f32x4 o0 = bias4(96, 0), o1 = bias4(96, 1);
#pragma unroll
        for (int ks = 0; ks < 2; ++ks) {
            const float x[8] = {sigmoidf_(h2[2 * ks][0]), sigmoidf_(h2[2 * ks][1]), sigmoidf_(h2[2 * ks][2]), sigmoidf_(h2[2 * ks][3]),
                                sigmoidf_(h2[2 * ks + 1][0]), sigmoidf_(h2[2 * ks + 1][1]), sigmoidf_(h2[2 * ks + 1][2]), sigmoidf_(h2[2 * ks + 1][3])};
            gin_split3(x, xb[0], xb[1], xb[2]);
            o0 = gin_mma6(w3p + (0 * 2 + ks) * 64, 256, xb, o0);
            o1 = gin_mma6(w3p + (1 * 2 + ks) * 64, 256, xb, o1);
        }
        float4 r0, r1;
        auto sig_out = [](float v) { return sigmoid_out_f32(v); };
        r0.x = sig_out(o0[0]); r0.y = sig_out(o0[1]); r0.z = sig_out(o0[2]); r0.w = sig_out(o0[3]);
        r1.x = sig_out(o1[0]); r1.y = sig_out(o1[1]); r1.z = sig_out(o1[2]); r1.w = sig_out(o1[3]);
        if (act == TGNN_ACT_LEAKY_RELU) {
            r0.x = leakyf_(r0.x); r0.y = leakyf_(r0.y); r0.z = leakyf_(r0.z); r0.w = leakyf_(r0.w);
            r1.x = leakyf_(r1.x); r1.y = leakyf_(r1.y); r1.z = leakyf_(r1.z); r1.w = leakyf_(r1.w);
        }
        const int64_t row = tile * 16 + fn;
        if (row < n) {
            *reinterpret_cast<float4 *>(out + row * 32 + 4 * fq) = r0;
            *reinterpret_cast<float4 *>(out + row * 32 + 16 + 4 * fq) = r1;
            const float v[8] = {r0.x, r0.y, r0.z, r0.w, r1.x, r1.y, r1.z, r1.w};
#pragma unroll
            for (int e = 0; e < 8; ++e) {
                cs[e] += (double)v[e];
                cq[e] += (double)v[e] * (double)v[e];
            }
        }
    }
    if (bn_partial) {
#pragma unroll
        for (int e = 0; e < 8; ++e)
#pragma unroll
            for (int d = 1; d <= 8; d <<= 1) {
                cs[e] += __shfl_xor(cs[e], d, 64);
                cq[e] += __shfl_xor(cq[e], d, 64);
            }
        if (fn == 0) {
#pragma unroll
            for (int e = 0; e < 8; ++e) {
                const int feat = (e < 4 ? 0 : 16) + 4 * fq + (e & 3);
                red[wave * 64 + feat] = cs[e];
                red[wave * 64 + 32 + feat] = cq[e];
            }
        }
        __syncthreads();
        using u32x2 = __attribute__((ext_vector_type(2))) unsigned int;
        const __amdgpu_buffer_rsrc_t prs = __builtin_amdgcn_make_buffer_rsrc(bn_partial, 0, (int)0x80000000u, 0x00020000);
        constexpr int kSc1 = 16;
        if (tid < 64) {
            double tot = 0.0;
            for (int w = 0; w < kMlpWaves; ++w) tot += red[w * 64 + tid];
            if (fin.counter)
                __builtin_amdgcn_raw_buffer_store_b64(__builtin_bit_cast(u32x2, tot), prs, ((uint32_t)blockIdx.x * 64u + (uint32_t)tid) * 8u, 0, kSc1);
            else
                bn_partial[(int64_t)blockIdx.x * 64 + tid] = tot;
        }
        if (fin.counter) {
            __shared__ unsigned ticket;
            __shared__ double ftot[64];
            const int g = (int)(blockIdx.x & 15u), np = (int)gridDim.x;
            asm volatile("s_waitcnt vmcnt(0)" ::: "memory");
            __syncthreads();
            if (tid == 0) ticket = __hip_atomic_fetch_add(fin.counter + 1 + g, 1u, __ATOMIC_RELAXED, __HIP_MEMORY_SCOPE_AGENT);
            __syncthreads();
            const unsigned group_size = (unsigned)((np - g + 15) / 16);
#ifdef TGNN_ABL_NOFOLDWORK
            if (ticket == group_size - 1 && tid == 0) __hip_atomic_store(fin.counter + 1 + g, 0u, __ATOMIC_RELAXED, __HIP_MEMORY_SCOPE_AGENT);
            if (false) {
#else
            if (ticket == group_size - 1) {
#endif
                if (tid < 64) {
                    double acc = 0.0;
                    for (int u0 = 0; g + u0 * 16 < np; u0 += 16) {
                        u32x2 v[16];
#pragma unroll
                        for (int u = 0; u < 16; ++u) {
                            const int pp = g + (u0 + u) * 16;
                            v[u] = __builtin_amdgcn_raw_buffer_load_b64(prs, pp < np ? ((uint32_t)pp * 64u + (uint32_t)tid) * 8u : 0x80000000u, 0, kSc1);
                        }
#pragma unroll
                        for (int u = 0; u < 16; ++u)
                            if (g + (u0 + u) * 16 < np) acc += __builtin_bit_cast(double, v[u]);
                    }
                    __builtin_amdgcn_raw_buffer_store_b64(__builtin_bit_cast(u32x2, acc), prs, ((uint32_t)(kGinGroupRow0 + g) * 64u + (uint32_t)tid) * 8u, 0, kSc1);
                }
                asm volatile("s_waitcnt vmcnt(0)" ::: "memory");
// ... 273 lines not shown
    if (tid >= 384 && tid < 384 + 8 * kFusedRing) flags[tid - 384] = 0;
    for (int i = tid; i < 4 * kMidTileFloats; i += kFusedThreads) tiles[i] = 0.f;
    __syncthreads();

    const int team = wave & 3, role = wave >> 2;
    const Gin32Tiles share = gin32_slot_share(n, (int)gridDim.x, (int)blockIdx.x, team);
    const int64_t t0 = share.t0, t1 = share.t1;
    const GinGraph G{rowptr, col_src, n};
    float *ring = rings + team * kFusedRing * kMidTileFloats;
    volatile int *ready = flags + 2 * kFusedRing * team, *taken = ready + kFusedRing;
    double bn = 0.0;
    if (role > 0) {
        for (int64_t i = role - 1; t0 + i < t1; i += kFusedGatherPerPair) {
            const int s = (int)(i % kFusedRing);
            while (i >= kFusedRing && taken[s] < (int)(i - kFusedRing) + 1) __builtin_amdgcn_s_sleep(1);
            gin_tile_gather<0>(G, t0 + i, in_stat != nullptr, a, spl, st2, ring + s * kMidTileFloats, lane);
            asm volatile("s_waitcnt lgkmcnt(0)" ::: "memory");
            __builtin_amdgcn_wave_barrier();
            if (lane == 0) ready[s] = (int)i + 1;
        }
    } else {
        float *tbuf = tiles + team * kMidTileFloats;
        for (int64_t i = 0; t0 + i < t1; ++i) {
            const int s = (int)(i % kFusedRing);
            while (ready[s] < (int)i + 1) __builtin_amdgcn_s_sleep(1);
            __builtin_amdgcn_fence(__ATOMIC_ACQUIRE, "workgroup");
            gin_tile_mlp<0>(G, t0 + i, out, gw, spl, ring + s * kMidTileFloats, tbuf, lane, bn, taken + s, (int)i + 1);
        }
    }

    if (bn_partial) {
        if (role == 0) red[team * 64 + lane] = bn;
        __syncthreads();
        using u32x2_ = __attribute__((ext_vector_type(2))) unsigned int;
        const __amdgpu_buffer_rsrc_t prs = __builtin_amdgcn_make_buffer_rsrc(bn_partial, 0, (int)0x80000000u, 0x00020000);
        if (tid < 64) {
            double tot = 0.0;
            for (int w = 0; w < 4; ++w) tot += red[w * 64 + tid];
            if (fin.counter)
                __builtin_amdgcn_raw_buffer_store_b64(__builtin_bit_cast(u32x2_, tot), prs, ((uint32_t)blockIdx.x * 64u + (uint32_t)tid) * 8u, 0, kCpSc1);
            else
                bn_partial[(int64_t)blockIdx.x * 64 + tid] = tot;
        }
        if (fin.counter) {
            __shared__ unsigned ticket;
            asm volatile("s_waitcnt vmcnt(0)" ::: "memory");
            __syncthreads();
            if (tid == 0) ticket = __hip_atomic_fetch_add(fin.counter, 1u, __ATOMIC_RELAXED, __HIP_MEMORY_SCOPE_AGENT);
            __syncthreads();
            if (ticket == gridDim.x - 1) {
                const int j = tid & 63, h = tid >> 6;
                if (tid < 512) {
#pragma unroll
                    for (int half = 0; half < 2; ++half) {
                        const int g = h + 8 * half;
                        double acc = 0.0;
                        const int np = (int)gridDim.x;
                        for (int p = g; p < np; p += 8 * 16) {
                            u32x2_ v[8];
#pragma unroll
                            for (int u = 0; u < 8; ++u) {
                                const int pp = p + u * 16;
                                v[u] = __builtin_amdgcn_raw_buffer_load_b64(prs, pp < np ? ((uint32_t)pp * 64u + (uint32_t)j) * 8u : 0x80000000u, 0, kCpSc1);
                            }
#pragma unroll
                            for (int u = 0; u < 8; ++u)
                                if (p + u * 16 < np) acc += __builtin_bit_cast(double, v[u]);
                        }
                        fred[g * 64 + j] = acc;
                    }
                }
                __syncthreads();
                if (tid < 64) {
                    double t = 0.0;
                    for (int gg = 0; gg < 16; ++gg) t += fred[gg * 64 + tid];
                    ftot[tid] = t;
                }
                __syncthreads();
                bn_record_from_sums(fin.job, ftot, 32, fin.n_total, fin.eps, fin.momentum);
                if (tid == 0) __hip_atomic_store(fin.counter, 0u, __ATOMIC_RELAXED, __HIP_MEMORY_SCOPE_AGENT);
            }
        }
    }
}

__global__ __launch_bounds__(256) void gin_generic_kernel(
    const float *__restrict__ a, int64_t lda, const float *__restrict__ in_stat, const int *__restrict__ rowptr,
    const int *__restrict__ col_src, const float *__restrict__ eps_p, const float *__restrict__ w1,
    const float *__restrict__ b1, const float *__restrict__ w2, const float *__restrict__ b2,
    const float *__restrict__ w3, const float *__restrict__ b3, int64_t n, int c, int act, float *__restrict__ out,
    double *__restrict__ bn_partial, float *__restrict__ z_keep) {
    __shared__ float zs[4][256];
    __shared__ float h1s[4][32];
    __shared__ float h2s[4][64];
    __shared__ double red[4][512];
    const int lane = threadIdx.x & 63, wave = threadIdx.x >> 6;
    const float one_eps = 1.0f + eps_p[0];
    for (int k = lane; k < 2 * c; k += 64) red[wave][k] = 0.0;
    for (int64_t v = (int64_t)blockIdx.x * 4 + wave; v < n; v += (int64_t)gridDim.x * 4) {
        const int beg = rowptr[v], end = rowptr[v + 1];
        for (int k = lane; k < c; k += 64) {
            float mh = 0.f, ml = 0.f, gg = 1.f, bb = 0.f;
            if (in_stat) { mh = in_stat[k]; ml = in_stat[c + k]; gg = in_stat[2 * c + k]; bb = in_stat[3 * c + k]; }
            float acc = 0.f;
            for (int e = beg; e < end; ++e) acc += (a[(int64_t)col_src[e] * lda + k] - mh) - ml;
            const float self = (a[v * lda + k] - mh) - ml;
            zs[wave][k] = fmaf(gg, fmaf(one_eps, self, acc), (one_eps + (float)(end - beg)) * bb);
            if (z_keep) z_keep[v * c + k] = zs[wave][k];
        }
        __builtin_amdgcn_wave_barrier();
        if (lane < 32) {
            float acc = b1[lane];
            for (int i = 0; i < c; ++i) acc = fmaf(zs[wave][i], w1[lane * c + i], acc);
            h1s[wave][lane] = sigmoidf_(acc);
        }
        __builtin_amdgcn_wave_barrier();
        {
            float acc = b2[lane];
            for (int i = 0; i < 32; ++i) acc = fmaf(h1s[wave][i], w2[lane * 32 + i], acc);
            h2s[wave][lane] = sigmoidf_(acc);
        }
        __builtin_amdgcn_wave_barrier();
        for (int o = lane; o < c; o += 64) {
            float acc = b3[o];
            for (int i = 0; i < 64; ++i) acc = fmaf(h2s[wave][i], w3[o * 64 + i], acc);
            acc = sigmoidf_(acc);
            if (act == TGNN_ACT_LEAKY_RELU) acc = leakyf_(acc);
            out[v * c + o] = acc;
            red[wave][o] += (double)acc;
            red[wave][c + o] += (double)acc * (double)acc;
        }
        __builtin_amdgcn_wave_barrier();
    }
    __syncthreads();
    if (bn_partial)
        for (int k = threadIdx.x; k < 2 * c; k += 256)
            bn_partial[(int64_t)blockIdx.x * 2 * c + k] = red[0][k] + red[1][k] + red[2][k] + red[3][k];
}

}

using namespace tgnn;
namespace tgnn { std::atomic<int> g_debug_block_cap[2]; static std::atomic<int> g_gin_fused{1}; std::atomic<int> g_gin_mlp16{0}; }
extern "C" int32_t tgnn_set_gin_mlp_f16(int32_t on) { return tgnn::g_gin_mlp16.exchange(on ? 1 : 0); }
extern "C" int32_t tgnn_set_gin_fused(int32_t mode) { return tgnn::g_gin_fused.exchange(mode < 0 ? 0 : (mode > 2 ? 2 : mode)); }
#ifdef TGNN_DEBUG
extern "C" void tgnn_debug_set_block_caps(int32_t nnconv_blocks, int32_t gin_mlp_blocks) {
    g_debug_block_cap[0].store(nnconv_blocks);
    g_debug_block_cap[1].store(gin_mlp_blocks);
}
#endif

namespace tgnn {
static int gin32_grid(int64_t n_nodes) {
    constexpr int reserve = 32;
    int cap = cus_minus(reserve);
    if (const int dbg = g_debug_block_cap[1].load(); dbg > 0) cap = dbg < device_cus() ? dbg : device_cus();
    return gin32_blocks(n_nodes, cap);
}

static void launch_gin32_aggregate(const float *a, int64_t lda, const float *in_stat, const int32_t *rowptr, const int32_t *col_src,
                                   const float *eps, int64_t n_nodes, float *z, hipStream_t s) {
    const int64_t rows_per_xcd = (n_nodes + 7) / 8;
    const unsigned agg_blocks = (unsigned)(8 * ((rows_per_xcd + 31) / 32));
    gin_aggregate_kernel<32><<<agg_blocks, 256, 0, s>>>(a, lda, in_stat, rowptr, col_src, eps, n_nodes, z);
}

static int launch_gin32_mlp_variant(Gin32Variant variant, const float *z, const float *w1, const float *b1, const float *w2, const float *b2,
                                    const float *w3, const float *b3, int64_t n_nodes, int32_t act, float *out, double *bn_partial,
                                    int32_t *n_partials_host, hipStream_t s, const GinFin *fin) {
    const int blocks = gin32_grid(n_nodes);
    GinFin f{};
    if (variant == kGin32F16) {
        if (fin && bn_partial) f = *fin;
        gin32_mlp16_kernel<<<blocks, kMlp16Threads, 0, s>>>(z, w1, b1, w2, b2, w3, b3, n_nodes, out, bn_partial, f);
    } else {
        if (fin && bn_partial) {
            f = *fin;
            f.job.partials = bn_partial;
            f.job.n_partials = blocks;
        }
        gin32_mlp_kernel<<<blocks, kMlpThreads, 0, s>>>(z, w1, b1, w2, b2, w3, b3, n_nodes, act, out, bn_partial, f);
    }
    if (n_partials_host) *n_partials_host = blocks;
    TGNN_CHECK_LAUNCH();
    return TGNN_OK;
}

static int launch_gin32_variant(Gin32Variant variant, const float *a, int64_t lda, const float *in_stat, const int32_t *rowptr,
                                const int32_t *col_src, const float *eps, const float *w1, const float *b1, const float *w2, const float *b2,
                                const float *w3, const float *b3, int64_t n_nodes, int32_t act, float *out, float *z_scratch,
                                double *bn_partial, int32_t *n_partials_host, const GinFin *fin, hipStream_t s) {
    if (variant == kGin32Fused) {
        const int blocks = gin32_grid(n_nodes);
        GinFin f{};
        if (fin && bn_partial) f = *fin;
        f.job.partials = bn_partial;
        f.job.n_partials = blocks;
        static LdsOptIn site;
        TGNN_CHECK_HIP(opt_in_dynamic_lds(gin32_fused_kernel, (int)kFusedLdsBytes, site));
        gin32_fused_kernel<<<blocks, kFusedThreads, kFusedLdsBytes, s>>>(a, in_stat, rowptr, col_src, eps, w1, b1, w2, b2, w3, b3, n_nodes, out, bn_partial, f);
        if (n_partials_host) *n_partials_host = blocks;
        TGNN_CHECK_LAUNCH();
        return TGNN_OK;
    }
    launch_gin32_aggregate(a, lda, in_stat, rowptr, col_src, eps, n_nodes, z_scratch, s);
    return launch_gin32_mlp_variant(variant, z_scratch, w1, b1, w2, b2, w3, b3, n_nodes, act, out, bn_partial, n_partials_host, s, fin);
}

int gin32_fwd_folded(const float *a, int64_t lda, const float *in_stat, const int32_t *rowptr, const int32_t *col_src, const float *eps,
                     const float *w1, const float *b1, const float *w2, const float *b2, const float *w3, const float *b3,
                     int64_t n_nodes, int32_t act, float *out, float *z_scratch, double *bn_partial, int32_t *n_partials_host,
                     const GinFin &fin, hipStream_t s, bool need_z) {
    if (!(n_nodes >= 1 && lda % 4 == 0 && ((uintptr_t)a % 16) == 0 && ((uintptr_t)out % 16) == 0 && z_scratch &&
          ((uintptr_t)z_scratch % 16) == 0 && bn_partial))
        return TGNN_ERR_UNSUPPORTED;
    const Gin32Variant variant = gin32_variant(need_z, lda, act, n_nodes, g_gin_fused.load(std::memory_order_relaxed),
                                               g_gin_mlp16.load(std::memory_order_relaxed));
    return launch_gin32_variant(variant, a, lda, in_stat, rowptr, col_src, eps, w1, b1, w2, b2, w3, b3, n_nodes, act, out, z_scratch, bn_partial,
                                n_partials_host, &fin, s);
}
}

extern "C" int tgnn_gin32_fwd(const float *a, int64_t lda, const float *in_stat, const int32_t *rowptr, const int32_t *col_src,
                              const float *eps, const float *w1, const float *b1, const float *w2, const float *b2, const float *w3,
                              const float *b3, int64_t n_nodes, int32_t c, int32_t act, int32_t variant, float *out, float *z_scratch,
                              double *bn_partial, int32_t *n_partials_host, tgnn_stream_t stream) {
    DeviceGuard guard__(stream);
    TGNN_CHECK_ARG(n_nodes >= 0 && c >= 1, "shape");
    TGNN_CHECK_ARG(act == TGNN_ACT_NONE || act == TGNN_ACT_LEAKY_RELU, "activation");
    TGNN_CHECK_ARG(variant == kGin32Bf16x3 || variant == kGin32F16 || variant == kGin32Fused, "variant");
    if (c != 32) {
        set_error("tgnn_gin32_fwd: width 32 only (c = %d)", (int)c);
        return TGNN_ERR_UNSUPPORTED;
    }
    if (n_nodes == 0) {
        if (n_partials_host) *n_partials_host = 0;
        return TGNN_OK;
    }
    TGNN_CHECK_ARG(a && rowptr && eps && w1 && b1 && w2 && b2 && w3 && b3 && out && (z_scratch || variant == kGin32Fused), "null pointer");
    TGNN_CHECK_ARG(lda >= 32, "lda");
    if (lda % 4 != 0 || ((uintptr_t)a % 16) != 0 || ((uintptr_t)out % 16) != 0 || (variant != kGin32Fused && ((uintptr_t)z_scratch % 16) != 0)) {
        set_error("tgnn_gin32_fwd: lda a multiple of 4, a / out / z_scratch 16-byte aligned (lda %lld)", (long long)lda);
        return TGNN_ERR_UNSUPPORTED;
    }
    if (!gin32_rows_addressable(n_nodes)) {
        set_error("tgnn_gin32_fwd: %lld rows of 128 bytes are past 2 GB", (long long)n_nodes);
        return TGNN_ERR_UNSUPPORTED;
    }
    if (variant != kGin32Bf16x3 && act != TGNN_ACT_LEAKY_RELU) {
        set_error("tgnn_gin32_fwd: variant %d runs with LeakyReLU only", (int)variant);
        return TGNN_ERR_UNSUPPORTED;
    }
    if (variant != kGin32Bf16x3 && lda != 32) {
        set_error("tgnn_gin32_fwd: variant %d reads packed rows only (lda %lld, not 32)", (int)variant, (long long)lda);
        return TGNN_ERR_UNSUPPORTED;
    }
    return launch_gin32_variant(static_cast<Gin32Variant>(variant), a, lda, in_stat, rowptr, col_src, eps, w1, b1, w2, b2, w3, b3, n_nodes, act,
                                out, z_scratch, bn_partial, n_partials_host, nullptr, static_cast<hipStream_t>(stream));
}

extern "C" int tgnn_gin_fwd(const float *a, int64_t lda, const float *in_stat, const int32_t *rowptr,
                            const int32_t *col_src, const float *eps, const float *w1, const float *b1,
                            const float *w2, const float *b2, const float *w3, const float *b3, int64_t n_nodes,
                            int32_t c, int32_t act, float *out, float *z_scratch, double *bn_partial,
                            int32_t *n_partials_host, tgnn_stream_t stream) {
    DeviceGuard guard__(stream);
    TGNN_CHECK_ARG(n_nodes >= 0 && c >= 1 && c <= 256, "shape");
    TGNN_CHECK_ARG(act == TGNN_ACT_NONE || act == TGNN_ACT_LEAKY_RELU, "activation");
    if (n_nodes == 0) {
        if (n_partials_host) *n_partials_host = 0;
        return TGNN_OK;
    }
    TGNN_CHECK_ARG(a && rowptr && eps && w1 && b1 && w2 && b2 && w3 && b3 && out, "null pointer");
    TGNN_CHECK_ARG(lda >= c, "lda");
    hipStream_t s = static_cast<hipStream_t>(stream);
    int blocks;
    if (c == 32 && lda % 4 == 0 && ((uintptr_t)a % 16) == 0 && ((uintptr_t)out % 16) == 0 && z_scratch &&
        ((uintptr_t)z_scratch % 16) == 0) {
        launch_gin32_aggregate(a, lda, in_stat, rowptr, col_src, eps, n_nodes, z_scratch, s);
        blocks = gin32_blocks(n_nodes, cus_minus(32));
        gin32_mlp_kernel<<<blocks, kMlpThreads, 0, s>>>(z_scratch, w1, b1, w2, b2, w3, b3, n_nodes, act, out,
                                                        bn_partial, GinFin{});
    } else {
        blocks = producer_blocks(n_nodes, 4);
        gin_generic_kernel<<<blocks, 256, 0, s>>>(a, lda, in_stat, rowptr, col_src, eps, w1, b1, w2, b2, w3, b3,
                                                  n_nodes, c, act, out, bn_partial, nullptr);
    }
    if (n_partials_host) *n_partials_host = blocks;
    TGNN_CHECK_LAUNCH();
    return TGNN_OK;
}

namespace tgnn {
int launch_gin32_mlp(const float *z, const float *w1, const float *b1, const float *w2, const float *b2, const float *w3,
                     const float *b3, int64_t n_nodes, int32_t act, float *out, double *bn_partial, int32_t *n_partials_host,
                     hipStream_t s, const GinFin *fin, bool inference) {
    const Gin32Variant variant = gin32_variant(!inference, 32, act, n_nodes, 0, g_gin_mlp16.load(std::memory_order_relaxed));
    return launch_gin32_mlp_variant(variant, z, w1, b1, w2, b2, w3, b3, n_nodes, act, out, bn_partial, n_partials_host, s, fin);
}
}

extern "C" int tgnn_gin_aggregate(const float *a, int64_t lda, const float *in_stat, const int32_t *rowptr,
                                  const int32_t *col_src, const float *eps, int64_t n_nodes, int32_t c, float *z,
                                  tgnn_stream_t stream) {
    DeviceGuard guard__(stream);
    TGNN_CHECK_ARG(n_nodes >= 0, "shape");
    if (c != 32 && c != 64) {
        set_error("tgnn_gin_aggregate: width 32 or 64 only");
        return TGNN_ERR_UNSUPPORTED;
    }
    if (n_nodes == 0) return TGNN_OK;
    TGNN_CHECK_ARG(a && rowptr && eps && z, "null pointer");
    TGNN_CHECK_ARG(lda >= c && lda % 4 == 0 && ((uintptr_t)a % 16) == 0 && ((uintptr_t)z % 16) == 0, "alignment");
    const int rows_per_block = 256 / (c / 4);
    const int64_t rows_per_xcd = (n_nodes + 7) / 8;
    const unsigned agg_blocks = (unsigned)(8 * ((rows_per_xcd + rows_per_block - 1) / rows_per_block));
    hipStream_t s = static_cast<hipStream_t>(stream);
    if (c == 32)
        gin_aggregate_kernel<32><<<agg_blocks, 256, 0, s>>>(a, lda, in_stat, rowptr, col_src, eps, n_nodes, z);
    else
        gin_aggregate_kernel<64><<<agg_blocks, 256, 0, s>>>(a, lda, in_stat, rowptr, col_src, eps, n_nodes, z);
    TGNN_CHECK_LAUNCH();
    return TGNN_OK;
}

namespace tgnn {
int gin_generic_fwd_keep(const float *a, int64_t lda, const float *in_stat, const int32_t *rowptr, const int32_t *col_src,
                         const float *eps, const float *w1, const float *b1, const float *w2, const float *b2, const float *w3,
                         const float *b3, int64_t n_nodes, int32_t c, int32_t act, float *out, float *z_keep, double *bn_partial,
                         int32_t *n_partials_host, hipStream_t s) {
    TGNN_CHECK_ARG(n_nodes >= 1 && c >= 1 && c <= 256 && lda >= c, "shape");
    TGNN_CHECK_ARG(a && rowptr && eps && w1 && b1 && w2 && b2 && w3 && b3 && out && z_keep, "null pointer");
    const int blocks = producer_blocks(n_nodes, 4);
    gin_generic_kernel<<<blocks, 256, 0, s>>>(a, lda, in_stat, rowptr, col_src, eps, w1, b1, w2, b2, w3, b3, n_nodes, c, act, out,
                                              bn_partial, z_keep);
    if (n_partials_host) *n_partials_host = blocks;
    TGNN_CHECK_LAUNCH();
    return TGNN_OK;
}
}
```

### tilingnn_amd/csrc/nnconv_eg.hip

```cpp
#include <atomic>
#include <type_traits>

#include "tgnn_common.h"
#include "split_pair_f16.h"

namespace tgnn {

using f32x4 = __attribute__((ext_vector_type(4))) float;
using f16x8 = tgnn_f16x8;
using f16x4 = __attribute__((ext_vector_type(4))) _Float16;

constexpr int kEgRootBit = 1 << 8;
constexpr int kEgExtraLog2 = 5;

using u32x4 = __attribute__((ext_vector_type(4))) unsigned;
using u32x2 = __attribute__((ext_vector_type(2))) unsigned;

struct EgShard {
    const int *send_row_ptr, *send_row_slot;
    float *msg;
    const int *msg_idx;
    int64_t n_msg;
    double *sums;
    unsigned *counter;
    double *group_rows;
};

template <int WAVES, int OCC, int ACT, bool SHARD = false, bool SUM = false>
__global__ __launch_bounds__(WAVES * 64, OCC) void nnconv32_eg_kernel(
    const float *__restrict__ h, const int *__restrict__ tile_grp_ptr, const int2 *__restrict__ grp,
    const float *__restrict__ wimg, int n_types, const float *__restrict__ bias, int64_t n,
    int act, float *__restrict__ out, double *__restrict__ bn_partial, const unsigned *__restrict__ h_max,
    const unsigned *__restrict__ root_max, unsigned long long *__restrict__ stamp, EgShard sh = EgShard{}) {
    extern __shared__ __attribute__((aligned(16))) float lds[];
    if (stamp && threadIdx.x == 0) atomicMin(stamp, wall_clock64());
    constexpr int kTy = kWtTypeF16;
    float *wl = lds;
    f16x4 *lut = reinterpret_cast<f16x4 *>(lds + (n_types + 1) * kTy);
    const unsigned hm_bits = *h_max, hm_exp = (hm_bits >> 23) & 0xffu;
#ifdef TGNN_ABL_EGNOUNIT
    const bool unit = hm_exp > 300;
#else
    const bool unit = hm_exp >= 130 && hm_exp <= 136;
#endif
    const float sx = unit ? 1.0f : pow2_scale_for(hm_bits, kEgExtraLog2);
    const float unscale = 1.0f / (sx * nnconv_weight_scale(*root_max) * kEgImageScale);
    const int tid = threadIdx.x, lane = tid & 63, wave = tid >> 6;
    const int fj = lane & 15, fq = lane >> 4;
    constexpr int kThreads = WAVES * 64;
    static_assert(WAVES % 4 == 0, "whole SIMD quads");
    const uint32_t n_tiles = (uint32_t)((n + 15) / 16);
    const uint32_t nblk = gridDim.x;
    uint32_t blk = blockIdx.x;
    if (nblk >= 8 && (nblk & 7) == 0) blk = (blockIdx.x & 7) * (nblk >> 3) + (blockIdx.x >> 3);
    const uint32_t slot = blk * 4 + (wave & 3), n_slots = nblk * 4;
    const uint32_t tq = n_tiles / n_slots, tr = n_tiles % n_slots;
    const uint32_t q0 = tq * slot + tr * slot / n_slots, q1 = tq * (slot + 1) + tr * (slot + 1) / n_slots;
    constexpr uint32_t kSubs = WAVES / 4;
    const uint32_t sub = wave >> 2;
    const int64_t t0 = q0 + (q1 - q0) * sub / kSubs, t1 = q0 + (q1 - q0) * (sub + 1) / kSubs;
    const int cbeg = __builtin_amdgcn_readfirstlane(tile_grp_ptr[t0]);
    const int cend = __builtin_amdgcn_readfirstlane(tile_grp_ptr[t1]);

    const float bias0 = SUM ? 0.f : bias[fj], bias1 = SUM ? 0.f : bias[16 + fj];
    double bs[2] = {0, 0}, bq[2] = {0, 0};

    const __amdgpu_buffer_rsrc_t h_rsrc =
        __builtin_amdgcn_make_buffer_rsrc(const_cast<float *>(h), 0, (int)0x80000000u, 0x00020000);
    const __amdgpu_buffer_rsrc_t own_rsrc =
        SUM ? __builtin_amdgcn_make_buffer_rsrc(const_cast<float *>(bias), 0, (int)0x80000000u, 0x00020000) : h_rsrc;
    const uint32_t fq_bytes = (uint32_t)fq * 32u;
    auto load_four = [&](int p, int &s4, int &m4) {
        const int pc = p < cend ? p : cbeg;
        const int2 v = grp[(int64_t)pc * 16 + lane];
        s4 = v.x;
        m4 = v.y;
    };
    auto unpack = [&](auto steady, int p, int u, int s4, int m4, int &s, int &m, int &meta) {
        s = __shfl(s4, u * 16 + fj, 64);
        m = __shfl(m4, u * 16 + fj, 64);
        meta = __builtin_amdgcn_readlane(m4, u * 16) >> 16;
        if constexpr (!decltype(steady)::value)
            if (p + u >= cend) {
                s = -1;
                m = 0;
                meta = 0;
            }
    };
    int64_t gtile = t0;
    auto own_off_of = [&](int64_t tile) -> uint32_t {
        const int64_t r = tile * 16 + fj;
        return r < n ? (uint32_t)r * 128u + fq_bytes : 0x80000000u;
    };
    uint32_t own_off = own_off_of(gtile);
    auto issue_gather = [&](int s, int meta, float4 (&x)[2]) {
        const bool root = (meta & kEgRootBit) != 0;
#ifdef TGNN_ABL_EGNOGATHER
        const uint32_t off = 0x80000000u + (((uint32_t)s + own_off) & 0);
#else
        const uint32_t off = root ? own_off : ((uint32_t)s << 7) + fq_bytes;
#endif
        if (SUM && root) {
            x[0] = __builtin_bit_cast(float4, __builtin_amdgcn_raw_buffer_load_b128(own_rsrc, off, 0, 0));
            x[1] = __builtin_bit_cast(float4, __builtin_amdgcn_raw_buffer_load_b128(own_rsrc, off + 16u, 0, 0));
        } else {
            x[0] = __builtin_bit_cast(float4, __builtin_amdgcn_raw_buffer_load_b128(h_rsrc, off, 0, 0));
            x[1] = __builtin_bit_cast(float4, __builtin_amdgcn_raw_buffer_load_b128(h_rsrc, off + 16u, 0, 0));
        }
        if (root) {
            ++gtile;
            own_off = own_off_of(gtile);
        }
    };

    f32x4 d0 = {0.f, 0.f, 0.f, 0.f}, d1 = d0;
    int64_t ctile = t0;
    const f32x4 zero4 = {0.f, 0.f, 0.f, 0.f};
    struct Msg {
        u32x2 a0, b0, a1, b1;
        f16x4 sel;
    };
    auto stage1 = [&](int s, int m, int meta, const float4 (&x)[2]) -> Msg {
        const int t = meta & 0xff;
        constexpr int kPl = kWtPlane / 4;
        const f16x8 *wp = reinterpret_cast<const f16x8 *>(wl + t * kTy) + lane;
        const f16x8 h0 = wp[0], h1 = wp[64], l0 = wp[kPl], l1 = wp[kPl + 64];
        f16x4 sel0 = lut[(m >> (4 * fq)) & 15];
#ifndef TGNN_ABL_EGLATE
        asm volatile("" : "+v"(sel0) :: "memory");
#endif
        unsigned xh0, xh1, xh2, xh3, xl0, xl1, xl2, xl3;
#ifdef TGNN_ABL_EGNOSPLIT
        xh0 = __float_as_uint(x[0].x); xl0 = __float_as_uint(x[0].y); xh1 = __float_as_uint(x[0].z); xl1 = __float_as_uint(x[0].w);
        xh2 = __float_as_uint(x[1].x); xl2 = __float_as_uint(x[1].y); xh3 = __float_as_uint(x[1].z); xl3 = __float_as_uint(x[1].w);
        if (false) {
#else
        if (unit) {
#endif
            split_pair_f16(x[0].x, x[0].y, xh0, xl0);
            split_pair_f16(x[0].z, x[0].w, xh1, xl1);
            split_pair_f16(x[1].x, x[1].y, xh2, xl2);
            split_pair_f16(x[1].z, x[1].w, xh3, xl3);
        } else {
            split_pair_f16(x[0].x, x[0].y, sx, xh0, xl0);
            split_pair_f16(x[0].z, x[0].w, sx, xh1, xl1);
            split_pair_f16(x[1].x, x[1].y, sx, xh2, xl2);
            split_pair_f16(x[1].z, x[1].w, sx, xh3, xl3);
        }
        const f16x8 gh = __builtin_bit_cast(f16x8, u32x4{xh0, xh1, xh2, xh3}), gl = __builtin_bit_cast(f16x8, u32x4{xl0, xl1, xl2, xl3});
        f32x4 m0 = __builtin_amdgcn_mfma_f32_16x16x32_f16(gh, l0, zero4, 0, 0, 0);
        f32x4 m1 = __builtin_amdgcn_mfma_f32_16x16x32_f16(gh, l1, zero4, 0, 0, 0);
        m0 = __builtin_amdgcn_mfma_f32_16x16x32_f16(gl, h0, m0, 0, 0, 0);
        m1 = __builtin_amdgcn_mfma_f32_16x16x32_f16(gl, h1, m1, 0, 0, 0);
        m0 = __builtin_amdgcn_mfma_f32_16x16x32_f16(gh, h0, m0, 0, 0, 0);
        m1 = __builtin_amdgcn_mfma_f32_16x16x32_f16(gh, h1, m1, 0, 0, 0);
        unsigned a00, a01, b00, b01, a10, a11, b10, b11;
#ifdef TGNN_ABL_EGNOMSGSPLIT
        a00 = __float_as_uint(m0[0]); b00 = __float_as_uint(m0[1]); a01 = __float_as_uint(m0[2]); b01 = __float_as_uint(m0[3]);
        a10 = __float_as_uint(m1[0]); b10 = __float_as_uint(m1[1]); a11 = __float_as_uint(m1[2]); b11 = __float_as_uint(m1[3]);
#else
        split_pair_f16(m0[0], m0[1], a00, b00);
        split_pair_f16(m0[2], m0[3], a01, b01);
        split_pair_f16(m1[0], m1[1], a10, b10);
        split_pair_f16(m1[2], m1[3], a11, b11);
#endif
        Msg r;
        r.a0 = u32x2{a00, a01}; r.b0 = u32x2{b00, b01}; r.a1 = u32x2{a10, a11}; r.b1 = u32x2{b10, b11};
        r.sel = sel0;
        if (!SUM && (meta & kEgRootBit)) {
            asm volatile("" ::: "memory");
            const _Float16 dg = (_Float16)__int_as_float(s);
            r.sel = r.sel * dg;
        }
        return r;
    };
    auto fold16 = [&](const Msg &g) {
        d0 = __builtin_amdgcn_mfma_f32_16x16x16f16(g.sel, __builtin_bit_cast(f16x4, g.b0), d0, 0, 0, 0);
        d1 = __builtin_amdgcn_mfma_f32_16x16x16f16(g.sel, __builtin_bit_cast(f16x4, g.b1), d1, 0, 0, 0);
        d0 = __builtin_amdgcn_mfma_f32_16x16x16f16(g.sel, __builtin_bit_cast(f16x4, g.a0), d0, 0, 0, 0);
        d1 = __builtin_amdgcn_mfma_f32_16x16x16f16(g.sel, __builtin_bit_cast(f16x4, g.a1), d1, 0, 0, 0);
    };
    auto fold32 = [&](const Msg &g, const Msg &k) {
        using f16x8v = f16x8;
        const f16x4 sg = g.sel, sk = k.sel;
        const f16x8v sel = {sg[0], sg[1], sg[2], sg[3], sk[0], sk[1], sk[2], sk[3]};
        auto cat = [](u32x2 p, u32x2 q) { return __builtin_bit_cast(f16x8v, u32x4{p[0], p[1], q[0], q[1]}); };
        d0 = __builtin_amdgcn_mfma_f32_16x16x32_f16(sel, cat(g.b0, k.b0), d0, 0, 0, 0);
        d1 = __builtin_amdgcn_mfma_f32_16x16x32_f16(sel, cat(g.b1, k.b1), d1, 0, 0, 0);
        d0 = __builtin_amdgcn_mfma_f32_16x16x32_f16(sel, cat(g.a0, k.a0), d0, 0, 0, 0);
        d1 = __builtin_amdgcn_mfma_f32_16x16x32_f16(sel, cat(g.a1, k.a1), d1, 0, 0, 0);
    };
    auto finish_tile = [&](int s) {
        double s0 = 0, s1 = 0, z0 = 0, z1 = 0;
#pragma unroll
        for (int r = 0; r < 4; ++r) {
            const int dg = __shfl(s, 4 * fq + r, 64);
            const bool valid = dg >= 0;
            const float inv = SUM ? unscale : unscale * __builtin_amdgcn_rcpf(__int_as_float(dg));
            float o0 = SUM ? d0[r] * inv : fmaf(d0[r], inv, bias0);
            float o1 = SUM ? d1[r] * inv : fmaf(d1[r], inv, bias1);
            if constexpr (ACT == TGNN_ACT_LEAKY_RELU) {
                o0 = leakyf_(o0);
                o1 = leakyf_(o1);
            }
            const int64_t v = ctile * 16 + 4 * fq + r;
            if (valid) {
                out[v * 32 + fj] = o0;
                out[v * 32 + 16 + fj] = o1;
                if constexpr (SHARD) {
                    const int p0 = sh.send_row_ptr[v], p1 = sh.send_row_ptr[v + 1];
                    for (int pp = p0; pp < p1; ++pp) {
                        float *dst = sh.msg + (int64_t)sh.send_row_slot[pp] * 32;
                        dst[fj] = o0;
// ... 33 lines not shown
    {
        int s4, m4;
        load_four(cbeg, s4, m4);
        load_four(cbeg + 4, s4n, m4n);
#pragma unroll
        for (int u = 0; u < 4; ++u) {
            unpack(std::false_type{}, cbeg, u, s4, m4, xs[u], xm[u], xt[u]);
            issue_gather(xs[u], xt[u], x[u]);
        }
    }
    {
        const int n4 = (n_types + 1) * kTy / 4;
        for (int i = tid; i < n4; i += 4 * kThreads) {
            float4 v[4];
#pragma unroll
            for (int u = 0; u < 4; ++u) {
                const int ii = i + u * kThreads < n4 ? i + u * kThreads : n4 - 1;
                v[u] = reinterpret_cast<const float4 *>(wimg)[ii];
            }
#pragma unroll
            for (int u = 0; u < 4; ++u)
                if (i + u * kThreads < n4) reinterpret_cast<float4 *>(wl)[i + u * kThreads] = v[u];
        }
        if (tid < 16) {
            f16x4 e;
#pragma unroll
            for (int b = 0; b < 4; ++b) e[b] = (tid >> b & 1) ? (_Float16)1.0f : (_Float16)0.0f;
            lut[tid] = e;
        }
    }

    __syncthreads();
    int base = cbeg;
#ifdef TGNN_ABL_EGNOLOOP
    base = cend;
#endif
    for (; base + 8 <= cend; base += 4) {
        int s4c, m4c;
        load_four(base + 8, s4c, m4c);
#pragma unroll
        for (int u = 0; u < 4; u += 2) {
            consume_pair(xs[u], xm[u], xt[u], x[u], xs[u + 1], xm[u + 1], xt[u + 1], x[u + 1]);
#pragma unroll
            for (int v = u; v < u + 2; ++v) {
                unpack(std::true_type{}, base + 4, v, s4n, m4n, xs[v], xm[v], xt[v]);
                issue_gather(xs[v], xt[v], x[v]);
            }
        }
        s4n = s4c;
        m4n = m4c;
    }
    for (; base < cend; base += 4) {
        int s4c, m4c;
        load_four(base + 8, s4c, m4c);
#pragma unroll
        for (int u = 0; u < 4; u += 2) {
            consume_pair(xs[u], xm[u], xt[u], x[u], xs[u + 1], xm[u + 1], xt[u + 1], x[u + 1]);
#pragma unroll
            for (int v = u; v < u + 2; ++v) {
                unpack(std::false_type{}, base + 4, v, s4n, m4n, xs[v], xm[v], xt[v]);
                issue_gather(xs[v], xt[v], x[v]);
            }
        }
        s4n = s4c;
        m4n = m4c;
    }

    if (bn_partial) {
        __syncthreads();
        double *red = reinterpret_cast<double *>(lds);
        double *mine = red + ((int64_t)wave * 64 + lane) * 4;
        mine[0] = bs[0]; mine[1] = bs[1]; mine[2] = bq[0]; mine[3] = bq[1];
        __syncthreads();
        if (tid < 64) {
            const int which = tid >> 5, ch = tid & 31, m2 = ch >> 4, j = ch & 15;
            double acc = 0;
            for (int w = 0; w < WAVES; ++w)
#pragma unroll
                for (int q = 0; q < 4; ++q) acc += red[((int64_t)w * 64 + q * 16 + j) * 4 + which * 2 + m2];
            if constexpr (SHARD) st_partial_sc1(bn_partial, (int64_t)blockIdx.x * 64 + tid, acc);
            else bn_partial[(int64_t)blockIdx.x * 64 + tid] = acc;
        }
        if constexpr (SHARD) {
            using u32x2_ = __attribute__((ext_vector_type(2))) unsigned int;
            constexpr int kSc1 = 16;
            double *ftot = red + WAVES * 64 * 4;
            unsigned *ticket = reinterpret_cast<unsigned *>(ftot + 64);
            const int np = (int)gridDim.x, g = (int)(blockIdx.x & 15u);
            const __amdgpu_buffer_rsrc_t prs = __builtin_amdgcn_make_buffer_rsrc(bn_partial, 0, (int)0x80000000u, 0x00020000);
            const __amdgpu_buffer_rsrc_t grs = __builtin_amdgcn_make_buffer_rsrc(sh.group_rows, 0, (int)0x80000000u, 0x00020000);
            asm volatile("s_waitcnt vmcnt(0)" ::: "memory");
            __syncthreads();
            if (tid == 0) *ticket = __hip_atomic_fetch_add(sh.counter + 1 + g, 1u, __ATOMIC_RELAXED, __HIP_MEMORY_SCOPE_AGENT);
            __syncthreads();
            if (*ticket == (unsigned)((np - g + 15) / 16) - 1u) {
                if (tid < 64) {
                    double acc = 0.0;
                    for (int u0 = 0; g + u0 * 16 < np; u0 += 16) {
                        u32x2_ v[16];
#pragma unroll
                        for (int u = 0; u < 16; ++u) {
                            const int pp = g + (u0 + u) * 16;
                            v[u] = __builtin_amdgcn_raw_buffer_load_b64(prs, pp < np ? ((uint32_t)pp * 64u + (uint32_t)tid) * 8u : 0x80000000u, 0, kSc1);
                        }
#pragma unroll
                        for (int u = 0; u < 16; ++u)
                            if (g + (u0 + u) * 16 < np) acc += __builtin_bit_cast(double, v[u]);
                    }
                    __builtin_amdgcn_raw_buffer_store_b64(__builtin_bit_cast(u32x2_, acc), grs, ((uint32_t)g * 64u + (uint32_t)tid) * 8u, 0, kSc1);
                }
                asm volatile("s_waitcnt vmcnt(0)" ::: "memory");
                __syncthreads();
                if (tid == 0) {
                    __hip_atomic_store(sh.counter + 1 + g, 0u, __ATOMIC_RELAXED, __HIP_MEMORY_SCOPE_AGENT);
                    *ticket = __hip_atomic_fetch_add(sh.counter, 1u, __ATOMIC_RELAXED, __HIP_MEMORY_SCOPE_AGENT);
                }
                __syncthreads();
                const int n_groups = np < 16 ? np : 16;
                if (*ticket == (unsigned)n_groups - 1u) {
                    if (tid < 64) {
                        u32x2_ v[16];
#pragma unroll
                        for (int gg = 0; gg < 16; ++gg)
                            v[gg] = __builtin_amdgcn_raw_buffer_load_b64(grs, gg < n_groups ? ((uint32_t)gg * 64u + (uint32_t)tid) * 8u : 0x80000000u, 0, kSc1);
                        double t = 0.0;
#pragma unroll
                        for (int gg = 0; gg < 16; ++gg)
                            if (gg < n_groups) t += __builtin_bit_cast(double, v[gg]);
                        ftot[tid] = t;
                        sh.sums[tid] = t;
                    }
                    __syncthreads();
                    const float *tf = reinterpret_cast<const float *>(ftot);
                    for (int64_t r = tid >> 5; r < sh.n_msg; r += kThreads / 32) {
                        const int id = sh.msg_idx[r];
                        if (id < 0) sh.msg[r * 32 + (tid & 31)] = tf[(-1 - id) * 32 + (tid & 31)];
                    }
                    if (tid == 0) __hip_atomic_store(sh.counter, 0u, __ATOMIC_RELAXED, __HIP_MEMORY_SCOPE_AGENT);
                }
            }
        }
    }
    if (stamp && tid == 0) atomicMax(stamp + 1, wall_clock64());
}

static size_t eg_lds_bytes(int n_types, int waves) {
    const size_t a = (size_t)(n_types + 1) * kWtTypeF16 * sizeof(float) + 16 * 8;
    const size_t b = (size_t)waves * 64 * 4 * sizeof(double) + 64 * sizeof(double) + 16;
    return a > b ? a : b;
}

constexpr size_t kEgMaxLds = 160 * 1024 - 256;

int launch_nnconv_eg(const float *h, const int32_t *tile_grp_ptr, const int32_t *grp, const float *wimg, int32_t n_types, const float *bias, int64_t n_nodes, int32_t act, float *out,
                     double *bn_partial, int32_t *n_partials_host, hipStream_t s, const unsigned *h_max, const unsigned *root_max,
                     unsigned long long *stamp, const EgShardPack *pack, const float *sum_root_rows) {
#ifdef TGNN_ABL_EGW8
    constexpr int WAVES = 8, kBlocksPerCu = 2;
#else
    constexpr int WAVES = 16, kBlocksPerCu = 1;
#endif
    const bool leaky = act == TGNN_ACT_LEAKY_RELU;
    const bool shard = pack && pack->counter && bn_partial && leaky;
    const bool sum = sum_root_rows != nullptr;
    auto kern = sum     ? nnconv32_eg_kernel<WAVES, 4, TGNN_ACT_NONE, false, true>
                : shard ? nnconv32_eg_kernel<WAVES, 4, TGNN_ACT_LEAKY_RELU, true>
                        : leaky ? nnconv32_eg_kernel<WAVES, 4, TGNN_ACT_LEAKY_RELU> : nnconv32_eg_kernel<WAVES, 4, TGNN_ACT_NONE>;
    static LdsOptIn site[4];
    TGNN_CHECK_HIP(opt_in_dynamic_lds(kern, (int)kEgMaxLds, site[sum ? 3 : shard ? 2 : leaky]));
    if (sum) {
        bias = sum_root_rows;
        bn_partial = nullptr;
    }
    EgShard sh{};
    if (shard) sh = EgShard{pack->send_row_ptr, pack->send_row_slot, pack->msg, pack->msg_idx, pack->n_msg, pack->sums, pack->counter, pack->group_rows};
    const int64_t n_tiles = (n_nodes + 15) / 16;
    constexpr int tiles_per_block = 4;
    int64_t blocks = (n_tiles + tiles_per_block - 1) / tiles_per_block;
    constexpr int reserve = 32;
    int64_t cap = (int64_t)cus_minus(reserve) * kBlocksPerCu;
    if (const int dbg = g_debug_block_cap[0].load(); dbg > 0) cap = dbg < device_cus() ? dbg : device_cus();
    if (blocks > cap) blocks = cap;
    if (blocks >= 8) blocks &= ~7;
    if (blocks < 1) blocks = 1;
    kern<<<(unsigned)blocks, WAVES * 64, eg_lds_bytes(n_types, WAVES), s>>>(h, tile_grp_ptr, reinterpret_cast<const int2 *>(grp), wimg,
                                                                            n_types, bias, n_nodes, act, out, bn_partial, h_max, root_max,
                                                                            stamp, sh);
    if (n_partials_host) *n_partials_host = (int32_t)blocks;
    TGNN_CHECK_LAUNCH();
    return TGNN_OK;
}

}

using namespace tgnn;

extern "C" int tgnn_nnconv_mean_eg_fwd(const float *h, int64_t ldh, int64_t n_src_rows, const int32_t *tile_grp_ptr,
                                       const int32_t *grp, const float *wtab, int32_t n_types,
                                       const float *root, const float *bias, int64_t n_nodes, int32_t act, float *out,
                                       float *wimg_scratch, uint32_t *bounds_scratch, double *bn_partial,
                                       int32_t *n_partials_host, tgnn_stream_t stream) {
    DeviceGuard guard__(stream);
    TGNN_CHECK_ARG(n_nodes >= 1 && n_src_rows >= n_nodes, "shape");
    TGNN_CHECK_ARG(act == TGNN_ACT_NONE || act == TGNN_ACT_LEAKY_RELU, "activation");
    TGNN_CHECK_ARG(h && tile_grp_ptr && grp && root && bias && out && wimg_scratch && bounds_scratch, "null pointer");
    TGNN_CHECK_ARG(n_types == 0 || wtab, "null weight table");
    TGNN_CHECK_ARG(ldh == 32 && ((uintptr_t)h % 16) == 0 && ((uintptr_t)wimg_scratch % 16) == 0 && ((uintptr_t)root % 16) == 0,
                   "alignment / packed rows");
    TGNN_CHECK_ARG(n_src_rows * 128 < ((int64_t)1 << 31), "source rows must lie within 2 GB of h");
    if ((size_t)(n_types + 1) * kWtTypeF16 * sizeof(float) + 16 * 8 > kEgMaxLds) {
        set_error("tgnn_nnconv_mean_eg_fwd: %d edge types do not fit the LDS weight image", n_types);
        return TGNN_ERR_UNSUPPORTED;
    }
    hipStream_t s = static_cast<hipStream_t>(stream);
    launch_forward_scales(bounds_scratch, 2, &root, 1, bounds_scratch + 1, nullptr, 0, nullptr, s);
    launch_absmax(h, n_src_rows * 32, bounds_scratch, s);
    launch_nnconv_weight_image(wtab, &root, n_types, 1, wimg_scratch, s, bounds_scratch + 1, kEgImageScale);
    return launch_nnconv_eg(h, tile_grp_ptr, grp, wimg_scratch, n_types, bias, n_nodes, act, out, bn_partial,
                            n_partials_host, s, bounds_scratch, bounds_scratch + 1, nullptr, nullptr, nullptr);
}
```

### tilingnn_amd/csrc/tgnn_common.h

```cpp
#pragma once
#include <hip/hip_runtime.h>
#include <stdint.h>
#include <stdio.h>

#include <atomic>

#include "../../include/tgnn.h"

namespace tgnn {

constexpr int kWave = 64;
constexpr float kLeakySlope = 0.01f;

void set_error(const char *fmt, ...);

#define TGNN_CHECK_ARG(cond, msg)                                                     \
    do {                                                                              \
        if (!(cond)) {                                                                \
            ::tgnn::set_error("%s: invalid argument: %s (%s)", __func__, msg, #cond); \
            return TGNN_ERR_INVALID_ARG;                                              \
        }                                                                             \
    } while (0)

#define TGNN_CHECK_LAUNCH()                                                                 \
// ... 259 lines not shown
        double acc = 0.0;
        for (int p = g; p < np; p += 8 * 16) {
            u32x2_ v[8];
#pragma unroll
            for (int u = 0; u < 8; ++u) {
                const int pp = p + u * 16;
                v[u] = __builtin_amdgcn_raw_buffer_load_b64(prs, pp < np ? ((uint32_t)pp * (uint32_t)kRow + (uint32_t)j) * 8u : 0x80000000u, 0, 16);
            }
#pragma unroll
            for (int u = 0; u < 8; ++u)
                if (p + u * 16 < np) acc += __builtin_bit_cast(double, v[u]);
        }
        fred[g * kRow + j] = acc;
    }
    __syncthreads();
    for (int j = tid; j < kRow; j += nthr) {
        double t = 0.0;
        for (int gg = 0; gg < 16; ++gg) t += fred[gg * kRow + j];
        ftot[j] = t;
    }
    __syncthreads();
    bn_record_from_sums(fin.job, ftot, F, fin.n_total, fin.eps, fin.momentum);
    if (tid == 0) __hip_atomic_store(fin.counter, 0u, __ATOMIC_RELAXED, __HIP_MEMORY_SCOPE_AGENT);
}
template <int F>
__device__ __forceinline__ void bn_fold_two_level(const GinFin &fin, double *bn_partial, double *group_rows, double *ftot,
                                                  unsigned *ticket) {
    using u32x2_ = __attribute__((ext_vector_type(2))) unsigned int;
    constexpr int kRow = 2 * F, kSc1 = 16;
    const int tid = threadIdx.x, nthr = blockDim.x, np = (int)gridDim.x, g = (int)(blockIdx.x & 15u);
    const __amdgpu_buffer_rsrc_t prs = __builtin_amdgcn_make_buffer_rsrc(bn_partial, 0, (int)0x80000000u, 0x00020000);
    const __amdgpu_buffer_rsrc_t grs = __builtin_amdgcn_make_buffer_rsrc(group_rows, 0, (int)0x80000000u, 0x00020000);
    asm volatile("s_waitcnt vmcnt(0)" ::: "memory");
    __syncthreads();
    if (tid == 0) *ticket = __hip_atomic_fetch_add(fin.counter + 1 + g, 1u, __ATOMIC_RELAXED, __HIP_MEMORY_SCOPE_AGENT);
    __syncthreads();
    if (*ticket != (unsigned)((np - g + 15) / 16) - 1u) return;
    for (int j = tid; j < kRow; j += nthr) {
        double acc = 0.0;
        for (int u0 = 0; g + u0 * 16 < np; u0 += 16) {
            u32x2_ v[16];
#pragma unroll
            for (int u = 0; u < 16; ++u) {
                const int pp = g + (u0 + u) * 16;
                v[u] = __builtin_amdgcn_raw_buffer_load_b64(prs, pp < np ? ((uint32_t)pp * (uint32_t)kRow + (uint32_t)j) * 8u : 0x80000000u, 0, kSc1);
            }
#pragma unroll
            for (int u = 0; u < 16; ++u)
                if (g + (u0 + u) * 16 < np) acc += __builtin_bit_cast(double, v[u]);
        }
        __builtin_amdgcn_raw_buffer_store_b64(__builtin_bit_cast(u32x2_, acc), grs, ((uint32_t)g * (uint32_t)kRow + (uint32_t)j) * 8u, 0, kSc1);
    }
    asm volatile("s_waitcnt vmcnt(0)" ::: "memory");
    __syncthreads();
    if (tid == 0) {
        __hip_atomic_store(fin.counter + 1 + g, 0u, __ATOMIC_RELAXED, __HIP_MEMORY_SCOPE_AGENT);
        *ticket = __hip_atomic_fetch_add(fin.counter, 1u, __ATOMIC_RELAXED, __HIP_MEMORY_SCOPE_AGENT);
    }
    __syncthreads();
    const int n_groups = np < 16 ? np : 16;
    if (*ticket != (unsigned)n_groups - 1u) return;
    for (int j = tid; j < kRow; j += nthr) {
        u32x2_ v[16];
#pragma unroll
        for (int gg = 0; gg < 16; ++gg)
            v[gg] = __builtin_amdgcn_raw_buffer_load_b64(grs, gg < n_groups ? ((uint32_t)gg * (uint32_t)kRow + (uint32_t)j) * 8u : 0x80000000u, 0, kSc1);
        double t = 0.0;
#pragma unroll
        for (int gg = 0; gg < 16; ++gg)
            if (gg < n_groups) t += __builtin_bit_cast(double, v[gg]);
        ftot[j] = t;
    }
    __syncthreads();
    bn_record_from_sums(fin.job, ftot, F, fin.n_total, fin.eps, fin.momentum);
    if (tid == 0) __hip_atomic_store(fin.counter, 0u, __ATOMIC_RELAXED, __HIP_MEMORY_SCOPE_AGENT);
}
void launch_bn_finalize(const BnJobs &jobs, int n_jobs, int mode, int f, int64_t n_total, float eps, float momentum,
                        hipStream_t s);
void launch_merge_bn1(const float *a1, const BnJob &j1, int64_t n_total, float eps, float momentum, const float *a2,
                      const float *stat2, const float *resid, int64_t n_nodes, float *out, hipStream_t s,
                      unsigned *absmax_out = nullptr);
void launch_merge(const float *a1, const float *stat1, const float *a2, const float *stat2, const float *resid, int64_t n_nodes,
                  int c, float *out, float *h2_out, unsigned *absmax_out, hipStream_t s);
void launch_bn_apply(const float *v, int64_t ldv, const float *stat, int64_t n_rows, int f, float *out, int64_t ldo,
                     unsigned *absmax_out, hipStream_t s);
void launch_shard_pack(const float *a1, const float *a2, const int *idx, int64_t n_rows, const double *sums, float *out,
                       hipStream_t s);
void launch_shard_unpack(const float *in, const int *idx, int64_t n_rows, int64_t n_own, float *a1, float *a2,
                         double *peer_sums, hipStream_t s);
void launch_shard_sum_peers(const double *peer_sums, const double *own, int world, int rank, double *total, hipStream_t s);
void launch_shard_pack_sums(const float *a1, const float *a2, const int *idx, int64_t n_rows, const BnJobs &jobs, float *out,
                            hipStream_t s);
int rccl_alltoall_rows(void *comm, const float *send, float *recv, const int64_t *send_counts, const int64_t *recv_counts,
                       int world, int32_t row_floats, int32_t extra_rows, hipStream_t s);
int rccl_allreduce_f64(void *comm, double *buf, int64_t count, hipStream_t s);
void launch_shard_pack1(const float *a, const int *idx, int64_t n_rows, const BnJob &job, float *out, hipStream_t s);
void launch_shard_unpack1(const float *in, const int *idx, int64_t n_rows, int64_t n_own, float *a, const BnJob &job, int world,
                          int rank, int64_t n_total, float eps, float momentum, hipStream_t s);
void launch_shard_unpack1_merge(const float *in, const int *idx, int64_t n_in, int64_t n_own, const float *a1, const BnJob &job,
                                int world, int rank, int64_t n_total, float eps, float momentum, const float *a2, const float *stat2,
                                const float *resid, int64_t n_rows, float *out, unsigned *absmax_out, hipStream_t s);
void launch_shard_unpack_finalize(const float *in, const int *idx, int64_t n_rows, int64_t n_own, float *a1, float *a2,
                                  const BnJobs &jobs, int world, int rank, int64_t n_total, float eps, float momentum,
                                  hipStream_t s);

struct EdgeMlpLayer {
    const float *w1, *b1, *w2, *b2, *w3, *b3;
};
constexpr int kMaxDepth = 64;
struct EdgeMlpLayers {
    EdgeMlpLayer l[kMaxDepth];
};
unsigned edge_weight_table_blocks(int n_types, int fe, int depth, int c, bool image);
void launch_edge_weight_table_batched(const float *edge_attr, const int *type_rep_edge, int n_types, int fe,
                                      const EdgeMlpLayers &layers, int depth, int c, float *wtab, const float *const *roots,
                                      float *wimg_all, hipStream_t s, unsigned *done_ctr = nullptr,
                                      const unsigned *root_max = nullptr, float img_scale = 1.0f, const int *n_types_dev = nullptr,
                                      int max_types_dev = 0);
struct EdgeWeightUnionEntry {
    const float *edge_attr;
    const int *type_rep_edge;
    float *wtab, *wimg;
    int n_types, pad_;
};
void launch_edge_weight_table_union(const EdgeWeightUnionEntry *tab_dev, int n_layouts, int max_types, int fe, const EdgeMlpLayers &layers,
                                    int depth, const float *const *roots, hipStream_t s);
bool edge_weight_table_device_count_ok(int fe, int c);
int init_mlp_fused_blocks(int64_t n);
int launch_init_mlp_fused(const float *x, int64_t ldx, int fx, const float *w0, const float *b0, const float *w1, const float *b1,
                          BnJob job0, BnJob job1, int64_t n, float eps, float momentum, float *out, unsigned *absmax_out,
                          hipStream_t s);
void launch_forward_scales(unsigned *words, int n_zero, const float *const *roots, int depth, unsigned *root_max,
                           const float *dense_w, int64_t dense_n, unsigned *dense_max, hipStream_t s);
void launch_nnconv_weight_image(const float *wtab_all, const float *const *roots, int n_types, int depth,
                                float *wimg_all, hipStream_t s, const unsigned *root_max = nullptr, float img_scale = 1.0f);
constexpr float kEgImageScale = 1.0f / 32768.0f;
int launch_nnconv_cols(const float *h, int64_t ldh, const int32_t *tile_col_ptr, const int32_t *col_meta,
                       const int32_t *col_src, const float *wimg, int32_t n_types, const float *bias,
                       int64_t n_nodes, int32_t act, float *out, double *bn_partial, int32_t *n_partials_host,
                       hipStream_t s, const unsigned *h_max = nullptr, const unsigned *root_max = nullptr,
                       int max_in_degree = 0, unsigned long long *stamp = nullptr);
struct EgShardPack {
    const int *send_row_ptr, *send_row_slot;
    float *msg;
    const int *msg_idx;
    int64_t n_msg;
    double *sums;
    unsigned *counter;
    double *group_rows;
};
int launch_nnconv_eg(const float *h, const int32_t *tile_grp_ptr, const int32_t *grp, const float *wimg, int32_t n_types, const float *bias, int64_t n_nodes, int32_t act, float *out,
                     double *bn_partial, int32_t *n_partials_host, hipStream_t s, const unsigned *h_max, const unsigned *root_max,
                     unsigned long long *stamp = nullptr, const EgShardPack *pack = nullptr, const float *sum_root_rows = nullptr);
void launch_absmax(const float *h, int64_t n_floats, unsigned *max_bits, hipStream_t s);
void launch_dense_bounds(int n_jobs, const float *const *w, const int64_t *w_n, const float *const *gamma, const float *const *beta,
                         const int *f, unsigned *const *w_max, unsigned *const *a_max, int64_t n_total, hipStream_t s);
int dense_act_bounded(const float *a, int64_t lda, int64_t a_kblock_stride, const float *in_stat, const float *w, const float *b,
                      int64_t n_rows, int32_t in_dim, int32_t out_dim, int32_t act, float *out, int64_t ldo, double *bn_partial,
                      int32_t *n_partials_host, const unsigned *a_max, int n_a_max, const unsigned *w_max, hipStream_t s,
                      const void *wimg = nullptr, const GinFin *fold = nullptr, double *fold_group_rows = nullptr, bool *folded = nullptr);
constexpr int64_t kDenseRowsKernelMin = 49152;
size_t dense_f16_image_size(int in_dim, int out_dim);
int dense_f16_image_build(const float *w, int in_dim, int out_dim, const unsigned *w_max, void *wimg, hipStream_t s);
int dense_f16_images_build(int n_jobs, const float *const *w, const int *in_dim, const int *out_dim, const unsigned *const *w_max,
                           void *const *wimg, hipStream_t s);
int dense_act_slots_bounded(const float *a, int32_t slot_width, int64_t slot_stride, const float *w, const float *b,
                            int64_t n_rows, int32_t in_dim, int32_t out_dim, int32_t act, float *out, int64_t ldo,
                            double *bn_partial, int32_t *n_partials_host, const unsigned *a_max, int n_a_max,
                            const unsigned *w_max, hipStream_t s, const void *wimg = nullptr, const GinFin *fold = nullptr,
                            double *fold_group_rows = nullptr, bool *folded = nullptr);
extern std::atomic<int> g_debug_block_cap[2];
int launch_gin32_mlp(const float *z, const float *w1, const float *b1, const float *w2, const float *b2, const float *w3,
                     const float *b3, int64_t n_nodes, int32_t act, float *out, double *bn_partial, int32_t *n_partials_host,
                     hipStream_t s, const GinFin *fin = nullptr, bool inference = false);
int gin32_fwd_folded(const float *a, int64_t lda, const float *in_stat, const int32_t *rowptr, const int32_t *col_src, const float *eps,
                     const float *w1, const float *b1, const float *w2, const float *b2, const float *w3, const float *b3,
                     int64_t n_nodes, int32_t act, float *out, float *z_scratch, double *bn_partial, int32_t *n_partials_host,
                     const GinFin &fin, hipStream_t s, bool need_z = true);
int gin_generic_fwd_keep(const float *a, int64_t lda, const float *in_stat, const int32_t *rowptr, const int32_t *col_src,
                         const float *eps, const float *w1, const float *b1, const float *w2, const float *b2, const float *w3,
                         const float *b3, int64_t n_nodes, int32_t c, int32_t act, float *out, float *z_keep, double *bn_partial,
                         int32_t *n_partials_host, hipStream_t s);
int spin_kernel_chain(hipStream_t s, void (*launch)(void *ctx, hipStream_t s), void *ctx, int cus_needed);
int small_layout_teams(const tgnn_model_dims *d, int64_t n_nodes, int n_types, int max_in_degree);
size_t small_pack_floats(int depth);
void launch_small_pack(const Params &P, int depth, float *pack, unsigned *barrier_ctr, hipStream_t s, bool dense_images = true,
                       void *zero = nullptr, size_t zero_bytes = 0, const unsigned *fin0_f16_max = nullptr,
                       hipStream_t final_images_stream = nullptr);
int launch_forward_small(const tgnn_model_dims *d, const Params &P, const float *x, float *probs, float *mid, float *a2_0,
                         float *a2_1, const float *wimg, float *pack, const tgnn_graph *graph, double *part, double *part_wide,
                         double *runstat, unsigned *ctr, const unsigned *weights_done, unsigned weights_target, int64_t n,
                         int update_running, float eps, float momentum, hipStream_t s);
struct SmallUnionLayout {
    const float *x, *edge_attr;
    const tgnn_graph *graph;
    float *probs, *mid, *a2_0, *a2_1, *wtab, *wimg;
    double *part, *part_wide;
};
int small_union_tiles(const tgnn_model_dims *d, int64_t n_nodes, int n_types, int max_in_degree);
int small_union_capacity();
int small_union_plan(const int *teams, int k, int capacity, int32_t *group_out);
int launch_forward_small_union(const tgnn_model_dims *d, const Params &P, const SmallUnionLayout *L, int k, const int32_t *group,
                               int n_groups, float eps, float momentum, hipStream_t s);
int mid_layout_tiles_per_block(const tgnn_model_dims *d, const tgnn_graph *g, int64_t n_nodes, int *blocks_out);
size_t mid_part_doubles();
int launch_forward_mid(const tgnn_model_dims *d, const Params &P, float *mid, float *a1, float *a2_0, float *a2_1, const float *wimg,
                       const float *pack, const tgnn_graph *graph, double *part, double *runstat, unsigned *ctr, unsigned *bounds,
                       int64_t n, int tiles_per_block, int blocks, int update_running, float eps, float momentum, hipStream_t s,
                       const unsigned *weights_done = nullptr, unsigned weights_target = 0, double *const *tail_zero = nullptr,
                       size_t tail_zero_doubles = 0, const float *x_init = nullptr);
int mid_tail_tiles_per_block(const tgnn_model_dims *d, int64_t n_nodes, int *blocks_out);
bool mid_init_in_kernel();
size_t mid_tail_part_doubles();
const float *small_dense_image(const float *pack, int depth, int k);
int launch_forward_tail(const tgnn_model_dims *d, const Params &P, const float *mid, const float *pack, float *probs, double *part,
                        double *gpart, const unsigned *slot_max, const unsigned *w0_max, int64_t n, int tiles_per_block, int blocks,
                        int update_running, float eps, float momentum, hipStream_t s, const int *verdict = nullptr);
constexpr int kWtPlane = 2 * 64 * 4;
constexpr int kWtType = 3 * kWtPlane;
constexpr int kWtTypeF16 = 2 * kWtPlane;
__device__ __host__ __forceinline__ float nnconv_weight_scale(unsigned root_max_bits) {
    float m;
    __builtin_memcpy(&m, &root_max_bits, 4);
    m = m > 1.0f ? m : 1.0f;
    unsigned b;
    __builtin_memcpy(&b, &m, 4);
    return pow2_scale_for(b, 0);
}
}
```

Measured before the change: 52.85 million nodes/s.

## Reshape merge and GIN MLP blocks to smaller waves for co-residency

The wide BN1 merge kernel drops from 1024 to 512 threads with an occupancy hint, handles two partial-row groups per thread, and batches its streaming loop with prefetch. The GIN MLP gains a four-wave variant, and a shared plan header fixes per-kernel footprints (waves, VGPR caps) and the NNConv tile split so the merge and GIN MLP kernels can share CUs. It also adds footprint query and standalone merge entry points. The goal is better occupancy and overlap between layer kernels, at the cost of more per-thread partial-reduction work and a changed block shape.

```diff
diff --git a/include/tgnn.h b/include/tgnn.h
--- a/include/tgnn.h
+++ b/include/tgnn.h
@@ -74,6 +74,8 @@
                                   int32_t *n_partials_host, tgnn_stream_t stream);
 
 int64_t tgnn_nnconv_eg_max_groups(int64_t n_nodes, int64_t n_edges, int32_t n_types);
+int tgnn_kernel_footprint(int32_t kernel, int32_t n_types, int32_t *out);
+int32_t tgnn_set_gin_mlp_half_blocks(int32_t mode);
 int tgnn_nnconv_eg_build(const int32_t *rowptr, const int32_t *col_src, const int32_t *col_type, int64_t n_nodes,
                          int32_t n_types, int32_t *tile_grp_ptr, int32_t *grp, void *ws, size_t ws_bytes, tgnn_stream_t stream);
 int tgnn_nnconv_mean_eg_fwd(const float *h, int64_t ldh, int64_t n_src_rows, const int32_t *tile_grp_ptr,
@@ -138,6 +140,9 @@
 int tgnn_bn_apply(const float *v, int64_t ldv, const float *stat, int64_t n_rows, int32_t f, float *out,
                   int64_t ldo, tgnn_stream_t stream);
 
+int tgnn_merge_bn1_fwd(const float *a1, const double *partials, int32_t n_partials, const float *gamma, const float *beta,
+                       int64_t n_rows_total, float eps, const float *a2, const float *stat2, const float *resid,
+                       int64_t n_nodes, float *out, float *stat1_out, tgnn_stream_t stream);
 int tgnn_merge_fwd(const float *a1, const float *stat1, const float *a2, const float *stat2,
                    const float *resid, int64_t n_nodes, int32_t c, float *out, float *h2_out,
                    tgnn_stream_t stream);
diff --git a/tilingnn_amd/_lib.py b/tilingnn_amd/_lib.py
--- a/tilingnn_amd/_lib.py
+++ b/tilingnn_amd/_lib.py
@@ -101,6 +101,9 @@
         "tgnn_nnconv_mean_cols_f16_fwd": (C.c_int, [p, i64, i64, p, p, p, p, i32, p, p, i64, i32, i32, p, p, p, p, pi32, p]),
         "tgnn_nnconv_eg_max_groups": (i64, [i64, i64, i32]),
         "tgnn_nnconv_eg_build": (C.c_int, [p, p, p, i64, i32, p, p, p, sz, p]),
+        "tgnn_kernel_footprint": (C.c_int, [i32, i32, pi32]),
+        "tgnn_set_gin_mlp_half_blocks": (i32, [i32]),
+        "tgnn_merge_bn1_fwd": (C.c_int, [p, p, i32, p, p, i64, C.c_float, p, p, p, i64, p, p, p]),
         "tgnn_nnconv_mean_eg_fwd": (C.c_int, [p, i64, i64, p, p, p, i32, p, p, i64, i32, p, p, p, p, pi32, p]),
         "tgnn_nnconv64_eg_max_types": (i32, []),
         "tgnn_nnconv64_eg_image_floats": (sz, [i32]),
@@ -299,7 +302,7 @@
     "tgnn_version", "tgnn_last_error", "tgnn_csr_workspace_bytes", "tgnn_csr_build",
     "tgnn_edge_dedup_workspace_bytes", "tgnn_edge_type_dedup", "tgnn_gather_i32", "tgnn_edge_weight_table",
     "tgnn_nnconv_mean_fwd", "tgnn_nnconv_cols_max_columns", "tgnn_nnconv_cols_workspace_bytes",
-    "tgnn_nnconv_cols_build", "tgnn_nnconv_cols_max_types", "tgnn_nnconv_weight_image_floats", "tgnn_nnconv_mean_cols_fwd", "tgnn_nnconv_mean_cols_f16_fwd", "tgnn_nnconv_eg_max_groups", "tgnn_nnconv_eg_build", "tgnn_nnconv_mean_eg_fwd",
+    "tgnn_nnconv_cols_build", "tgnn_nnconv_cols_max_types", "tgnn_nnconv_weight_image_floats", "tgnn_nnconv_mean_cols_fwd", "tgnn_nnconv_mean_cols_f16_fwd", "tgnn_nnconv_eg_max_groups", "tgnn_nnconv_eg_build", "tgnn_kernel_footprint", "tgnn_set_gin_mlp_half_blocks", "tgnn_merge_bn1_fwd", "tgnn_nnconv_mean_eg_fwd",
     "tgnn_nnconv64_eg_max_types", "tgnn_nnconv64_eg_image_floats", "tgnn_nnconv64_mean_eg_fwd", "tgnn_set_nnconv64_eg",
     "tgnn_gin64_fwd", "tgnn_set_gin64_mfma", "tgnn_gin32_fwd",
     "tgnn_ubench_row_gather", "tgnn_mid_entries_words", "tgnn_mid_entries_build", "tgnn_forward_path_counts", "tgnn_set_mid_layout_limit", "tgnn_get_mid_layout_limit", "tgnn_mid_layout_max_nodes",
diff --git a/tilingnn_amd/csrc/bn_merge.hip b/tilingnn_amd/csrc/bn_merge.hip
--- a/tilingnn_amd/csrc/bn_merge.hip
+++ b/tilingnn_amd/csrc/bn_merge.hip
@@ -1,4 +1,5 @@
 #include "tgnn_common.h"
+#include "nnconv_eg_plan.h"
 
 namespace tgnn {
 
@@ -251,11 +252,14 @@
     absmax_flush(am, absmax_out);
 }
 
-__global__ __launch_bounds__(1024) void merge_bn1_wide_kernel(const float *__restrict__ a1, BnJob j1, int64_t n_total, float eps,
-                                                              float momentum, const float *__restrict__ a2,
-                                                              const float *__restrict__ st2, const float *__restrict__ resid,
-                                                              int64_t n4, float *__restrict__ out, unsigned *__restrict__ absmax_out) {
+template <int THREADS>
+__global__ __launch_bounds__(THREADS, 4) void merge_bn1_wide_kernel(const float *__restrict__ a1, BnJob j1, int64_t n_total, float eps,
+                                                                    float momentum, const float *__restrict__ a2,
+                                                                    const float *__restrict__ st2, const float *__restrict__ resid,
+                                                                    int64_t n4, float *__restrict__ out, unsigned *__restrict__ absmax_out) {
     constexpr int c = 32, two_f = 64, groups = 16;
+    static_assert(THREADS == 1024 || THREADS == 512, "one or two row groups per thread");
+    constexpr int kGpt = groups * two_f / THREADS, kBatch = 32 / kGpt;
     __shared__ double red[groups * two_f];
     __shared__ double tot[two_f];
     __shared__ __attribute__((aligned(16))) float st1[4 * c];
@@ -270,7 +274,7 @@
             pre_rv = j1.running_var[tid];
         }
     }
-    if (tid >= 1024 - 4 * c) st2s[tid - (1024 - 4 * c)] = st2[tid - (1024 - 4 * c)];
+    if (tid >= THREADS - 4 * c) st2s[tid - (THREADS - 4 * c)] = st2[tid - (THREADS - 4 * c)];
     constexpr int kPf = 3;
     const int64_t i_first = (int64_t)blockIdx.x * blockDim.x + tid, i_step = (int64_t)gridDim.x * blockDim.x;
     float4 px1[kPf], px2[kPf], pr[kPf];
@@ -280,22 +284,36 @@
         const __amdgpu_buffer_rsrc_t prs = __builtin_amdgcn_make_buffer_rsrc(
             const_cast<double *>(j1.partials), 0, (int)((uint32_t)j1.n_partials * (uint32_t)two_f * 8u), 0x00020000);
         static_assert(TGNN_BN_MAX_PARTIALS <= 32 * groups, "32 rows per thread cover every partial row");
-        u32x2_ v[32];
-#pragma unroll
-        for (int q = 0; q < 32; ++q)
-            v[q] = __builtin_amdgcn_raw_buffer_load_b64(prs, ((uint32_t)(g + q * groups) * (uint32_t)two_f + (uint32_t)j) * 8u, 0, 0);
-#pragma unroll
-        for (int k = 0; k < kPf; ++k) {
-            const int64_t i = i_first + k * i_step;
-            const int64_t ii = i < n4 ? i : n4 - 1;
-            px1[k] = reinterpret_cast<const float4 *>(a1)[ii];
-            px2[k] = reinterpret_cast<const float4 *>(a2)[ii];
-            pr[k] = resid ? reinterpret_cast<const float4 *>(resid)[ii] : float4{0.f, 0.f, 0.f, 0.f};
-        }
-        double acc = 0.0;
-#pragma unroll
-        for (int q = 0; q < 32; ++q) acc += __builtin_bit_cast(double, v[q]);
-        red[tid] = acc;
+        double acc[kGpt];
+#pragma unroll
+        for (int u = 0; u < kGpt; ++u) acc[u] = 0.0;
+#pragma unroll
+        for (int q0 = 0; q0 < 32; q0 += kBatch) {
+            if (q0 > 0 && j1.n_partials <= q0 * groups) break;
+            u32x2_ v[kGpt][kBatch];
+#pragma unroll
+            for (int u = 0; u < kGpt; ++u)
+#pragma unroll
+                for (int q = 0; q < kBatch; ++q)
+                    v[u][q] = __builtin_amdgcn_raw_buffer_load_b64(
+                        prs, ((uint32_t)(g + u * (THREADS / two_f) + (q0 + q) * groups) * (uint32_t)two_f + (uint32_t)j) * 8u, 0, 0);
+            if (q0 == 0) {
+#pragma unroll
+                for (int k = 0; k < kPf; ++k) {
+                    const int64_t i = i_first + k * i_step;
+                    const int64_t ii = i < n4 ? i : n4 - 1;
+                    px1[k] = reinterpret_cast<const float4 *>(a1)[ii];
+                    px2[k] = reinterpret_cast<const float4 *>(a2)[ii];
+                    pr[k] = resid ? reinterpret_cast<const float4 *>(resid)[ii] : float4{0.f, 0.f, 0.f, 0.f};
+                }
+            }
+#pragma unroll
+            for (int u = 0; u < kGpt; ++u)
+#pragma unroll
+                for (int q = 0; q < kBatch; ++q) acc[u] += __builtin_bit_cast(double, v[u][q]);
+        }
+#pragma unroll
+        for (int u = 0; u < kGpt; ++u) red[tid + u * THREADS] = acc[u];
     }
     __syncthreads();
     if (tid < two_f) {
@@ -350,11 +368,29 @@
         const int64_t i = i_first + k * i_step;
         if (i < n4) item(px1[k], px2[k], pr[k], i);
     }
-    for (int64_t i = i_first + kPf * i_step; i < n4; i += i_step) {
-        const float4 x1 = reinterpret_cast<const float4 *>(a1)[i];
-        const float4 x2 = reinterpret_cast<const float4 *>(a2)[i];
-        const float4 r = resid ? reinterpret_cast<const float4 *>(resid)[i] : float4{0.f, 0.f, 0.f, 0.f};
-        item(x1, x2, r, i);
+    if constexpr (THREADS == 512) {
+        for (int64_t i0 = i_first + kPf * i_step; i0 < n4; i0 += kPf * i_step) {
+#pragma unroll
+            for (int k = 0; k < kPf; ++k) {
+                const int64_t i = i0 + k * i_step;
+                const int64_t ii = i < n4 ? i : n4 - 1;
+                px1[k] = reinterpret_cast<const float4 *>(a1)[ii];
+                px2[k] = reinterpret_cast<const float4 *>(a2)[ii];
+                pr[k] = resid ? reinterpret_cast<const float4 *>(resid)[ii] : float4{0.f, 0.f, 0.f, 0.f};
+            }
+#pragma unroll
+            for (int k = 0; k < kPf; ++k) {
+                const int64_t i = i0 + k * i_step;
+                if (i < n4) item(px1[k], px2[k], pr[k], i);
+            }
+        }
+    } else {
+        for (int64_t i = i_first + kPf * i_step; i < n4; i += i_step) {
+            const float4 x1 = reinterpret_cast<const float4 *>(a1)[i];
+            const float4 x2 = reinterpret_cast<const float4 *>(a2)[i];
+            const float4 r = resid ? reinterpret_cast<const float4 *>(resid)[i] : float4{0.f, 0.f, 0.f, 0.f};
+            item(x1, x2, r, i);
+        }
     }
     absmax_flush(am, absmax_out);
 }
@@ -714,13 +750,25 @@
     shard_sum_peers_kernel<<<1, 128, 0, s>>>(peer_sums, own, world, rank, total);
 }
 
+#ifdef TGNN_ABL_MERGEW16
+constexpr int kWideThreads = 1024;
+#else
+constexpr int kWideThreads = 512;
+#endif
+static_assert(kWideThreads == 1024 || kLayerFootprints[kLayerMerge].waves_per_block * 64 == kWideThreads, "nnconv_eg_plan.h states the shape");
+
+int merge_wide_func_attributes(hipFuncAttributes *attr, int *waves) {
+    *waves = kWideThreads / 64;
+    return (int)hipFuncGetAttributes(attr, reinterpret_cast<const void *>(merge_bn1_wide_kernel<kWideThreads>));
+}
+
 void launch_merge_bn1(const float *a1, const BnJob &j1, int64_t n_total, float eps, float momentum, const float *a2,
                       const float *stat2, const float *resid, int64_t n_nodes, float *out, hipStream_t s, unsigned *absmax_out) {
     const int64_t n4 = n_nodes * 32 / 4;
     if (j1.n_partials > 128) {
-        int64_t blocks = (n4 + 1023) / 1024;
+        int64_t blocks = (n4 + kWideThreads - 1) / kWideThreads;
         if (blocks > 256) blocks = 256;
-        merge_bn1_wide_kernel<<<(unsigned)blocks, 1024, 0, s>>>(a1, j1, n_total, eps, momentum, a2, stat2, resid, n4, out, absmax_out);
+        merge_bn1_wide_kernel<kWideThreads><<<(unsigned)blocks, kWideThreads, 0, s>>>(a1, j1, n_total, eps, momentum, a2, stat2, resid, n4, out, absmax_out);
         return;
     }
     int64_t blocks = (n4 + 255) / 256;
@@ -795,6 +843,21 @@
     return TGNN_OK;
 }
 
+extern "C" int tgnn_merge_bn1_fwd(const float *a1, const double *partials, int32_t n_partials, const float *gamma, const float *beta,
+                                  int64_t n_rows_total, float eps, const float *a2, const float *stat2, const float *resid,
+                                  int64_t n_nodes, float *out, float *stat1_out, tgnn_stream_t stream) {
+    DeviceGuard guard__(stream);
+    if (n_nodes <= 0) return TGNN_OK;
+    TGNN_CHECK_ARG(a1 && partials && gamma && beta && a2 && stat2 && out, "null pointer");
+    TGNN_CHECK_ARG(n_partials >= 1 && n_partials <= TGNN_BN_MAX_PARTIALS && n_rows_total >= 1, "partial rows / row count");
+    TGNN_CHECK_ARG(((uintptr_t)a1 | (uintptr_t)a2 | (uintptr_t)out | (uintptr_t)resid | (uintptr_t)stat2 | (uintptr_t)partials) % 16 == 0,
+                   "pointers must be 16-byte aligned");
+    launch_merge_bn1(a1, BnJob{partials, n_partials, nullptr, gamma, beta, nullptr, nullptr, nullptr, stat1_out}, n_rows_total, eps, 0.f,
+                     a2, stat2, resid, n_nodes, out, static_cast<hipStream_t>(stream), nullptr);
+    TGNN_CHECK_LAUNCH();
+    return TGNN_OK;
+}
+
 extern "C" int tgnn_merge_fwd(const float *a1, const float *stat1, const float *a2, const float *stat2,
                               const float *resid, int64_t n_nodes, int32_t c, float *out, float *h2_out,
                               tgnn_stream_t stream) {
diff --git a/tilingnn_amd/csrc/gin.hip b/tilingnn_amd/csrc/gin.hip
--- a/tilingnn_amd/csrc/gin.hip
+++ b/tilingnn_amd/csrc/gin.hip
@@ -2,12 +2,18 @@
 
 #include "forward_persist.h"
 #include "gin32_plan.h"
+#include "nnconv_eg_plan.h"
 
 namespace tgnn {
 
 
+#ifdef TGNN_ABL_AGG8
+#define TGNN_AGG_BOUNDS __launch_bounds__(256, 8)
+#else
+#define TGNN_AGG_BOUNDS __launch_bounds__(256)
+#endif
 template <int C>
-__global__ __launch_bounds__(256) void gin_aggregate_kernel(
+__global__ TGNN_AGG_BOUNDS void gin_aggregate_kernel(
     const float *__restrict__ a, int64_t lda, const float *__restrict__ in_stat, const int *__restrict__ rowptr,
     const int *__restrict__ col_src, const float *__restrict__ eps_p, int64_t n, float *__restrict__ z) {
     constexpr int LPR = C / 4, RPB = 256 / LPR;
@@ -31,17 +37,29 @@
     const float4 self = *reinterpret_cast<const float4 *>(a + v * lda + 4 * q);
     float4 acc = make_float4(0, 0, 0, 0);
     int e = beg;
+#define TGNN_ACC(X)                          \
+    acc.x += ((X).x - mhi.x) - mlo.x;        \
+    acc.y += ((X).y - mhi.y) - mlo.y;        \
+    acc.z += ((X).z - mhi.z) - mlo.z;        \
+    acc.w += ((X).w - mhi.w) - mlo.w;
+#ifdef TGNN_ABL_AGG8
+    for (; e + 8 <= end; e += 8) {
+        int sidx[8];
+#pragma unroll
+        for (int u = 0; u < 8; ++u) sidx[u] = col_src[e + u];
+        float4 xx[8];
+#pragma unroll
+        for (int u = 0; u < 8; ++u) xx[u] = *reinterpret_cast<const float4 *>(a + (int64_t)sidx[u] * lda + 4 * q);
+#pragma unroll
+        for (int u = 0; u < 8; ++u) { TGNN_ACC(xx[u]) }
+    }
+#endif
     for (; e + 4 <= end; e += 4) {
         const int s0 = col_src[e], s1 = col_src[e + 1], s2 = col_src[e + 2], s3 = col_src[e + 3];
         const float4 x0 = *reinterpret_cast<const float4 *>(a + (int64_t)s0 * lda + 4 * q);
         const float4 x1 = *reinterpret_cast<const float4 *>(a + (int64_t)s1 * lda + 4 * q);
         const float4 x2 = *reinterpret_cast<const float4 *>(a + (int64_t)s2 * lda + 4 * q);
         const float4 x3 = *reinterpret_cast<const float4 *>(a + (int64_t)s3 * lda + 4 * q);
-#define TGNN_ACC(X)                          \
-    acc.x += ((X).x - mhi.x) - mlo.x;        \
-    acc.y += ((X).y - mhi.y) - mlo.y;        \
-    acc.z += ((X).z - mhi.z) - mlo.z;        \
-    acc.w += ((X).w - mhi.w) - mlo.w;
         TGNN_ACC(x0) TGNN_ACC(x1) TGNN_ACC(x2) TGNN_ACC(x3)
     }
     for (; e < end; ++e) {
@@ -58,9 +76,10 @@
     *reinterpret_cast<float4 *>(z + v * C + 4 * q) = o;
 }
 
-constexpr int kMlpWaves = 8, kMlpThreads = kMlpWaves * 64;
-static_assert(kGin32BlockRows == kGin32TileRows * kMlpWaves && kGin32MaxPartials == TGNN_BN_MAX_PARTIALS &&
-              kGin32ActLeakyRelu == TGNN_ACT_LEAKY_RELU, "gin32_plan.h restates these");
+constexpr int kMlpWaves = 8, kMlpThreads = kMlpWaves * 64, kMlpHalfWaves = 4;
+static_assert(kGin32BlockRows == kGin32TileRows * kMlpWaves, "gin32_plan.h restates this");
+static_assert(kLayerFootprints[kLayerGinMlp].waves_per_block == kMlpHalfWaves, "nnconv_eg_plan.h states the forward's shape");
+static_assert(kGin32MaxPartials == TGNN_BN_MAX_PARTIALS && kGin32ActLeakyRelu == TGNN_ACT_LEAKY_RELU, "gin32_plan.h restates these");
 constexpr int kGinGroupRow0 = TGNN_BN_MAX_PARTIALS - 16;
 using bf16x8 = __attribute__((ext_vector_type(8))) __bf16;
 using f32x4 = __attribute__((ext_vector_type(4))) float;
@@ -82,7 +101,8 @@
     return acc;
 }
 
-__global__ __launch_bounds__(kMlpThreads, 2) void gin32_mlp_kernel(
+template <int WAVES>
+__global__ __launch_bounds__(WAVES * 64, 2) void gin32_mlp_kernel(
     const float *__restrict__ z, const float *__restrict__ w1, const float *__restrict__ b1,
     const float *__restrict__ w2, const float *__restrict__ b2, const float *__restrict__ w3,
     const float *__restrict__ b3, int64_t n, int act, float *__restrict__ out, double *__restrict__ bn_partial, GinFin fin) {
@@ -90,14 +110,17 @@
     __shared__ bf16x8 W2s[3 * 4 * 64];
     __shared__ bf16x8 W3s[3 * 2 * 2 * 64];
     __shared__ __attribute__((aligned(16))) float Bs[128];
-    __shared__ double red[kMlpWaves * 64];
+    __shared__ double red[WAVES * 64];
+    static_assert(WAVES == kMlpWaves || WAVES == kMlpHalfWaves, "two waves of a SIMD split its slot's run, or one walks it");
+    constexpr int kMlpThreads = WAVES * 64, kMlpWaves = WAVES;
     const int tid = threadIdx.x, lane = tid & 63, wave = tid >> 6;
     const int fn = lane & 15, fq = lane >> 4;
 #ifdef TGNN_ABL_EMPTYGIN
     if (n > 0) return;
 #endif
 
-    const Gin32Tiles share = gin32_wave_share(n, (int)gridDim.x, (int)blockIdx.x, wave);
+    const Gin32Tiles share = WAVES == 8 ? gin32_wave_share(n, (int)gridDim.x, (int)blockIdx.x, wave)
+                                        : gin32_slot_share(n, (int)gridDim.x, (int)blockIdx.x, wave);
     const int64_t t0 = share.t0, t1 = share.t1;
 
     auto load_z = [&](int64_t tile, float4 (&zin)[2]) {
@@ -677,11 +700,41 @@
 #endif
 
 namespace tgnn {
-static int gin32_grid(int64_t n_nodes) {
+static int gin32_cap() {
     constexpr int reserve = 32;
     int cap = cus_minus(reserve);
     if (const int dbg = g_debug_block_cap[1].load(); dbg > 0) cap = dbg < device_cus() ? dbg : device_cus();
-    return gin32_blocks(n_nodes, cap);
+    return cap;
+}
+static int gin32_grid(int64_t n_nodes) { return gin32_blocks(n_nodes, gin32_cap()); }
+
+int gin32_func_attributes(int which, hipFuncAttributes *attr, int *waves) {
+    *waves = which == kLayerGinMlp ? kMlpHalfWaves : 4;
+    return (int)hipFuncGetAttributes(attr, which == kLayerGinMlp ? reinterpret_cast<const void *>(gin32_mlp_kernel<kMlpHalfWaves>)
+                                                                 : reinterpret_cast<const void *>(gin_aggregate_kernel<32>));
+}
+
+static std::atomic<int> g_gin_mlp_half{1};
+static bool gin32_half_blocks(bool forward) {
+#ifdef TGNN_ABL_GINMLPW8
+    return false;
+#else
+    const int mode = g_gin_mlp_half.load(std::memory_order_relaxed);
+    return mode == 2 || (mode == 1 && forward);
+#endif
+}
+
+}
+extern "C" int32_t tgnn_set_gin_mlp_half_blocks(int32_t mode) { return tgnn::g_gin_mlp_half.exchange(mode < 0 ? 0 : (mode > 2 ? 2 : mode)); }
+namespace tgnn {
+
+static int gin32_mlp_grid(int64_t n_nodes, int cap, bool half) {
+    if (!half) return gin32_blocks(n_nodes, cap);
+    int64_t nb = (n_nodes + kGin32TileRows * kMlpHalfWaves - 1) / (kGin32TileRows * kMlpHalfWaves);
+    if (nb > 2 * (int64_t)cap) nb = 2 * (int64_t)cap;
+    if (nb > kGinGroupRow0) nb = kGinGroupRow0;
+    if (nb >= 8) nb &= ~int64_t(7);
+    return nb < 1 ? 1 : (int)nb;
 }
 
 static void launch_gin32_aggregate(const float *a, int64_t lda, const float *in_stat, const int32_t *rowptr, const int32_t *col_src,
@@ -693,9 +746,11 @@
 
 static int launch_gin32_mlp_variant(Gin32Variant variant, const float *z, const float *w1, const float *b1, const float *w2, const float *b2,
                                     const float *w3, const float *b3, int64_t n_nodes, int32_t act, float *out, double *bn_partial,
-                                    int32_t *n_partials_host, hipStream_t s, const GinFin *fin) {
-    const int blocks = gin32_grid(n_nodes);
+                                    int32_t *n_partials_host, hipStream_t s, const GinFin *fin, bool forward = false) {
+    int blocks = gin32_grid(n_nodes);
     GinFin f{};
+    const bool half = gin32_half_blocks(forward);
+    if (variant != kGin32F16) blocks = gin32_mlp_grid(n_nodes, gin32_cap(), half);
     if (variant == kGin32F16) {
         if (fin && bn_partial) f = *fin;
         gin32_mlp16_kernel<<<blocks, kMlp16Threads, 0, s>>>(z, w1, b1, w2, b2, w3, b3, n_nodes, out, bn_partial, f);
@@ -705,7 +760,8 @@
             f.job.partials = bn_partial;
             f.job.n_partials = blocks;
         }
-        gin32_mlp_kernel<<<blocks, kMlpThreads, 0, s>>>(z, w1, b1, w2, b2, w3, b3, n_nodes, act, out, bn_partial, f);
+        if (half) gin32_mlp_kernel<kMlpHalfWaves><<<blocks, kMlpHalfWaves * 64, 0, s>>>(z, w1, b1, w2, b2, w3, b3, n_nodes, act, out, bn_partial, f);
+        else gin32_mlp_kernel<kMlpWaves><<<blocks, kMlpThreads, 0, s>>>(z, w1, b1, w2, b2, w3, b3, n_nodes, act, out, bn_partial, f);
     }
     if (n_partials_host) *n_partials_host = blocks;
     TGNN_CHECK_LAUNCH();
@@ -715,7 +771,7 @@
 static int launch_gin32_variant(Gin32Variant variant, const float *a, int64_t lda, const float *in_stat, const int32_t *rowptr,
                                 const int32_t *col_src, const float *eps, const float *w1, const float *b1, const float *w2, const float *b2,
                                 const float *w3, const float *b3, int64_t n_nodes, int32_t act, float *out, float *z_scratch,
-                                double *bn_partial, int32_t *n_partials_host, const GinFin *fin, hipStream_t s) {
+                                double *bn_partial, int32_t *n_partials_host, const GinFin *fin, hipStream_t s, bool forward = false) {
     if (variant == kGin32Fused) {
         const int blocks = gin32_grid(n_nodes);
         GinFin f{};
@@ -730,7 +786,7 @@
         return TGNN_OK;
     }
     launch_gin32_aggregate(a, lda, in_stat, rowptr, col_src, eps, n_nodes, z_scratch, s);
-    return launch_gin32_mlp_variant(variant, z_scratch, w1, b1, w2, b2, w3, b3, n_nodes, act, out, bn_partial, n_partials_host, s, fin);
+    return launch_gin32_mlp_variant(variant, z_scratch, w1, b1, w2, b2, w3, b3, n_nodes, act, out, bn_partial, n_partials_host, s, fin, forward);
 }
 
 int gin32_fwd_folded(const float *a, int64_t lda, const float *in_stat, const int32_t *rowptr, const int32_t *col_src, const float *eps,
@@ -743,7 +799,7 @@
     const Gin32Variant variant = gin32_variant(need_z, lda, act, n_nodes, g_gin_fused.load(std::memory_order_relaxed),
                                                g_gin_mlp16.load(std::memory_order_relaxed));
     return launch_gin32_variant(variant, a, lda, in_stat, rowptr, col_src, eps, w1, b1, w2, b2, w3, b3, n_nodes, act, out, z_scratch, bn_partial,
-                                n_partials_host, &fin, s);
+                                n_partials_host, &fin, s, !need_z);
 }
 }
 
@@ -805,7 +861,7 @@
         ((uintptr_t)z_scratch % 16) == 0) {
         launch_gin32_aggregate(a, lda, in_stat, rowptr, col_src, eps, n_nodes, z_scratch, s);
         blocks = gin32_blocks(n_nodes, cus_minus(32));
-        gin32_mlp_kernel<<<blocks, kMlpThreads, 0, s>>>(z_scratch, w1, b1, w2, b2, w3, b3, n_nodes, act, out,
+        gin32_mlp_kernel<kMlpWaves><<<blocks, kMlpThreads, 0, s>>>(z_scratch, w1, b1, w2, b2, w3, b3, n_nodes, act, out,
                                                         bn_partial, GinFin{});
     } else {
         blocks = producer_blocks(n_nodes, 4);
diff --git a/tilingnn_amd/csrc/nnconv_eg.hip b/tilingnn_amd/csrc/nnconv_eg.hip
--- a/tilingnn_amd/csrc/nnconv_eg.hip
+++ b/tilingnn_amd/csrc/nnconv_eg.hip
@@ -2,6 +2,7 @@
 #include <type_traits>
 
 #include "tgnn_common.h"
+#include "nnconv_eg_plan.h"
 #include "split_pair_f16.h"
 
 namespace tgnn {
@@ -48,17 +49,9 @@
     const int tid = threadIdx.x, lane = tid & 63, wave = tid >> 6;
     const int fj = lane & 15, fq = lane >> 4;
     constexpr int kThreads = WAVES * 64;
-    static_assert(WAVES % 4 == 0, "whole SIMD quads");
-    const uint32_t n_tiles = (uint32_t)((n + 15) / 16);
-    const uint32_t nblk = gridDim.x;
-    uint32_t blk = blockIdx.x;
-    if (nblk >= 8 && (nblk & 7) == 0) blk = (blockIdx.x & 7) * (nblk >> 3) + (blockIdx.x >> 3);
-    const uint32_t slot = blk * 4 + (wave & 3), n_slots = nblk * 4;
-    const uint32_t tq = n_tiles / n_slots, tr = n_tiles % n_slots;
-    const uint32_t q0 = tq * slot + tr * slot / n_slots, q1 = tq * (slot + 1) + tr * (slot + 1) / n_slots;
-    constexpr uint32_t kSubs = WAVES / 4;
-    const uint32_t sub = wave >> 2;
-    const int64_t t0 = q0 + (q1 - q0) * sub / kSubs, t1 = q0 + (q1 - q0) * (sub + 1) / kSubs;
+    static_assert(WAVES % kEgSimds == 0, "whole SIMD quads");
+    const EgTiles share = nnconv_eg_wave_share(nnconv_eg_n_tiles(n), gridDim.x, blockIdx.x, (uint32_t)wave, WAVES);
+    const int64_t t0 = share.t0, t1 = share.t1;
     const int cbeg = __builtin_amdgcn_readfirstlane(tile_grp_ptr[t0]);
     const int cend = __builtin_amdgcn_readfirstlane(tile_grp_ptr[t1]);
 
@@ -398,20 +391,32 @@
 
 constexpr size_t kEgMaxLds = 160 * 1024 - 256;
 
+#if defined(TGNN_ABL_EGW8)
+constexpr int kEgWaves = 8, kEgOcc = 4, kEgBlocksPerCu = 2;
+#elif defined(TGNN_ABL_EGW12)
+constexpr int kEgWaves = 12, kEgOcc = 4, kEgBlocksPerCu = 1;
+#elif defined(TGNN_ABL_EGW16C96)
+constexpr int kEgWaves = 16, kEgOcc = 5, kEgBlocksPerCu = 1;
+#else
+constexpr int kEgWaves = kLayerFootprints[kLayerNnconvEg].waves_per_block, kEgOcc = kSimdVgprs / kLayerFootprints[kLayerNnconvEg].vgpr_cap;
+constexpr int kEgBlocksPerCu = 1;
+#endif
+
+int nnconv_eg_func_attributes(hipFuncAttributes *attr, int *waves) {
+    *waves = kEgWaves;
+    return (int)hipFuncGetAttributes(attr, reinterpret_cast<const void *>(nnconv32_eg_kernel<kEgWaves, kEgOcc, TGNN_ACT_LEAKY_RELU>));
+}
+
 int launch_nnconv_eg(const float *h, const int32_t *tile_grp_ptr, const int32_t *grp, const float *wimg, int32_t n_types, const float *bias, int64_t n_nodes, int32_t act, float *out,
                      double *bn_partial, int32_t *n_partials_host, hipStream_t s, const unsigned *h_max, const unsigned *root_max,
                      unsigned long long *stamp, const EgShardPack *pack, const float *sum_root_rows) {
-#ifdef TGNN_ABL_EGW8
-    constexpr int WAVES = 8, kBlocksPerCu = 2;
-#else
-    constexpr int WAVES = 16, kBlocksPerCu = 1;
-#endif
+    constexpr int WAVES = kEgWaves, OCC = kEgOcc, kBlocksPerCu = kEgBlocksPerCu;
     const bool leaky = act == TGNN_ACT_LEAKY_RELU;
     const bool shard = pack && pack->counter && bn_partial && leaky;
     const bool sum = sum_root_rows != nullptr;
-    auto kern = sum     ? nnconv32_eg_kernel<WAVES, 4, TGNN_ACT_NONE, false, true>
-                : shard ? nnconv32_eg_kernel<WAVES, 4, TGNN_ACT_LEAKY_RELU, true>
-                        : leaky ? nnconv32_eg_kernel<WAVES, 4, TGNN_ACT_LEAKY_RELU> : nnconv32_eg_kernel<WAVES, 4, TGNN_ACT_NONE>;
+    auto kern = sum     ? nnconv32_eg_kernel<WAVES, OCC, TGNN_ACT_NONE, false, true>
+                : shard ? nnconv32_eg_kernel<WAVES, OCC, TGNN_ACT_LEAKY_RELU, true>
+                        : leaky ? nnconv32_eg_kernel<WAVES, OCC, TGNN_ACT_LEAKY_RELU> : nnconv32_eg_kernel<WAVES, OCC, TGNN_ACT_NONE>;
     static LdsOptIn site[4];
     TGNN_CHECK_HIP(opt_in_dynamic_lds(kern, (int)kEgMaxLds, site[sum ? 3 : shard ? 2 : leaky]));
     if (sum) {
@@ -420,15 +425,14 @@
     }
     EgShard sh{};
     if (shard) sh = EgShard{pack->send_row_ptr, pack->send_row_slot, pack->msg, pack->msg_idx, pack->n_msg, pack->sums, pack->counter, pack->group_rows};
-    const int64_t n_tiles = (n_nodes + 15) / 16;
-    constexpr int tiles_per_block = 4;
-    int64_t blocks = (n_tiles + tiles_per_block - 1) / tiles_per_block;
+#ifdef TGNN_ABL_EGRES0
+    constexpr int reserve = 0;
+#else
     constexpr int reserve = 32;
+#endif
     int64_t cap = (int64_t)cus_minus(reserve) * kBlocksPerCu;
     if (const int dbg = g_debug_block_cap[0].load(); dbg > 0) cap = dbg < device_cus() ? dbg : device_cus();
-    if (blocks > cap) blocks = cap;
-    if (blocks >= 8) blocks &= ~7;
-    if (blocks < 1) blocks = 1;
+    const int blocks = nnconv_eg_blocks(n_nodes, cap);
     kern<<<(unsigned)blocks, WAVES * 64, eg_lds_bytes(n_types, WAVES), s>>>(h, tile_grp_ptr, reinterpret_cast<const int2 *>(grp), wimg,
                                                                             n_types, bias, n_nodes, act, out, bn_partial, h_max, root_max,
                                                                             stamp, sh);
@@ -440,6 +444,31 @@
 }
 
 using namespace tgnn;
+
+extern "C" int tgnn_kernel_footprint(int32_t kernel, int32_t n_types, int32_t *out) {
+    TGNN_CHECK_ARG(kernel >= 0 && kernel < kLayerKernels && out && n_types >= 0, "kernel index / null pointer");
+    hipFuncAttributes attr{};
+    int waves = 0, dyn_lds = 0, rc = 0;
+    switch (kernel) {
+    case kLayerNnconvEg:
+        rc = nnconv_eg_func_attributes(&attr, &waves);
+        dyn_lds = (int)eg_lds_bytes(n_types, waves);
+        break;
+    case kLayerMerge: rc = merge_wide_func_attributes(&attr, &waves); break;
+    default: rc = gin32_func_attributes(kernel, &attr, &waves); break;
+    }
+    if (rc != 0) {
+        set_error("tgnn_kernel_footprint: hipFuncGetAttributes failed (%d)", rc);
+        return TGNN_ERR_LAUNCH;
+    }
+    out[0] = waves;
+    out[1] = (waves + kEgSimds - 1) / kEgSimds;
+    out[2] = kLayerFootprints[kernel].vgpr_cap;
+    out[3] = attr.numRegs;
+    out[4] = (int32_t)attr.sharedSizeBytes + dyn_lds;
+    out[5] = attr.maxThreadsPerBlock;
+    return TGNN_OK;
+}
 
 extern "C" int tgnn_nnconv_mean_eg_fwd(const float *h, int64_t ldh, int64_t n_src_rows, const int32_t *tile_grp_ptr,
                                        const int32_t *grp, const float *wtab, int32_t n_types,
diff --git a/tilingnn_amd/csrc/nnconv_eg_plan.h b/tilingnn_amd/csrc/nnconv_eg_plan.h
--- /dev/null
+++ b/tilingnn_amd/csrc/nnconv_eg_plan.h
@@ -0,0 +1,71 @@
+#pragma once
+#include <stdint.h>
+
+namespace tgnn {
+
+constexpr int kEgTileRows = 16;
+constexpr int kEgSimds = 4;
+constexpr int kEgTilesPerBlock = 4;
+constexpr int kEgMaxBlocks = 1024;
+
+constexpr uint32_t nnconv_eg_n_tiles(int64_t n_nodes) { return (uint32_t)((n_nodes + kEgTileRows - 1) / kEgTileRows); }
+
+constexpr int nnconv_eg_blocks(int64_t n_nodes, int64_t cap) {
+    const int64_t n_tiles = (n_nodes + kEgTileRows - 1) / kEgTileRows;
+    int64_t blocks = (n_tiles + kEgTilesPerBlock - 1) / kEgTilesPerBlock;
+    if (blocks > cap) blocks = cap;
+    if (blocks > kEgMaxBlocks) blocks = kEgMaxBlocks;
+    if (blocks >= 8) blocks &= ~int64_t(7);
+    if (blocks < 1) blocks = 1;
+    return (int)blocks;
+}
+
+struct EgTiles {
+    uint32_t t0, t1;
+};
+
+constexpr uint32_t nnconv_eg_swizzled_block(uint32_t nblk, uint32_t block) {
+    return nblk >= 8 && (nblk & 7) == 0 ? (block & 7) * (nblk >> 3) + (block >> 3) : block;
+}
+
+constexpr EgTiles nnconv_eg_slot_share(uint32_t n_tiles, uint32_t nblk, uint32_t block, uint32_t simd) {
+    const uint32_t slot = nnconv_eg_swizzled_block(nblk, block) * kEgSimds + simd, n_slots = nblk * kEgSimds;
+    const uint32_t tq = n_tiles / n_slots, tr = n_tiles % n_slots;
+    return EgTiles{tq * slot + tr * slot / n_slots, tq * (slot + 1) + tr * (slot + 1) / n_slots};
+}
+
+constexpr EgTiles nnconv_eg_wave_share(uint32_t n_tiles, uint32_t nblk, uint32_t block, uint32_t wave, uint32_t waves) {
+    const EgTiles q = nnconv_eg_slot_share(n_tiles, nblk, block, wave & (kEgSimds - 1));
+    const uint32_t subs = waves / kEgSimds, sub = wave / kEgSimds;
+    return EgTiles{q.t0 + (q.t1 - q.t0) * sub / subs, q.t0 + (q.t1 - q.t0) * (sub + 1) / subs};
+}
+
+enum LayerKernel : int {
+    kLayerNnconvEg = 0,
+    kLayerGinAggregate = 1,
+    kLayerGinMlp = 2,
+    kLayerMerge = 3,
+    kLayerKernels = 4,
+};
+
+struct KernelFootprint {
+    int waves_per_block, waves_per_simd, vgpr_cap;
+};
+
+constexpr int kSimdVgprs = 512, kCuLdsBytes = 160 * 1024;
+
+constexpr KernelFootprint kLayerFootprints[kLayerKernels] = {
+    {16, 4, 128},
+    {4, 1, 512},
+    {4, 1, 256},
+    {8, 2, 128},
+};
+
+struct CoResidentPair {
+    LayerKernel a, b;
+};
+constexpr CoResidentPair kCoResidentPairs[] = {{kLayerGinMlp, kLayerMerge}};
+
+constexpr int vgprs_allocated(int vgprs) { return (vgprs + 7) / 8 * 8; }
+
+}
diff --git a/tilingnn_amd/csrc/tgnn_common.h b/tilingnn_amd/csrc/tgnn_common.h
--- a/tilingnn_amd/csrc/tgnn_common.h
+++ b/tilingnn_amd/csrc/tgnn_common.h
@@ -435,6 +435,9 @@
 int launch_nnconv_eg(const float *h, const int32_t *tile_grp_ptr, const int32_t *grp, const float *wimg, int32_t n_types, const float *bias, int64_t n_nodes, int32_t act, float *out,
                      double *bn_partial, int32_t *n_partials_host, hipStream_t s, const unsigned *h_max, const unsigned *root_max,
                      unsigned long long *stamp = nullptr, const EgShardPack *pack = nullptr, const float *sum_root_rows = nullptr);
+int nnconv_eg_func_attributes(hipFuncAttributes *attr, int *waves);
+int gin32_func_attributes(int which, hipFuncAttributes *attr, int *waves);
+int merge_wide_func_attributes(hipFuncAttributes *attr, int *waves);
 void launch_absmax(const float *h, int64_t n_floats, unsigned *max_bits, hipStream_t s);
 void launch_dense_bounds(int n_jobs, const float *const *w, const int64_t *w_n, const float *const *gamma, const float *const *beta,
                          const int *f, unsigned *const *w_max, unsigned *const *a_max, int64_t n_total, hipStream_t s);
```

Measured after the change: 53.60 million nodes/s, median of 6. 1.4% higher.
